# EricSteinberger/PokerRL

Hardware: AMD Instinct MI355X
Metric: CFR+ node-updates/sec on FHP public tree (higher is better)
Workload: dtype f32

## Files before the change

include/pokerrl_hip.h:

```cpp
#ifndef POKERRL_HIP_H
#define POKERRL_HIP_H

#include <stdint.h>

#ifdef __cplusplus
extern "C" {
#endif

#define PRL_MAX_BET_SIZES 96

#define PRL_OK 0
#define PRL_ERR_ARG (-1)
#define PRL_ERR_NO_DEVICE (-2)
#define PRL_ERR_HIP (-3)
#define PRL_ERR_UNSUPPORTED (-4)
#define PRL_ERR_OOM (-5)
#define PRL_ERR_STATE (-6)

typedef struct PrlRules {
    int32_t n_hole_cards;
    int32_t n_ranks;
    int32_t n_suits;
    int32_t n_cards;
    int32_t range_size;
// ... 86 lines not shown
int32_t prl_tree_info(const prl_tree_t* tree, int32_t* out_info );

enum {
    PRL_TF_KIND = 0,
    PRL_TF_ACTOR = 1,
    PRL_TF_PARENT = 2,
    PRL_TF_CHILD_IDX = 3,
    PRL_TF_ACTION = 4,
    PRL_TF_ACTED_LAST = 5,
    PRL_TF_ROUND = 6,
    PRL_TF_BOARD_ID = 7,
    PRL_TF_MAIN_POT = 8,
    PRL_TF_DEPTH = 9,
    PRL_TF_N_CHILDREN = 10,
    PRL_TF_FIRST_COL = 11,
    PRL_TF_SUBTREE_SIZE = 12,
    PRL_TF_CHILD_START = 13,
    PRL_TF_CHILD_LIST = 14,
    PRL_TF_COL_ACTION = 15,
    PRL_TF_COL_NODE = 16,
    PRL_TF_LEVEL_START = 17,
    PRL_TF_LEVEL_NODES = 18
};
int32_t prl_tree_get(const prl_tree_t* tree, int32_t field, int32_t* out);
int32_t prl_tree_get_boards(const prl_tree_t* tree, int8_t* out_rows);

#define PRL_OBS_VANILLA 0
#define PRL_OBS_HISTORY 1
#define PRL_OBS_FLAT_HU_LIMIT 2
int32_t prl_tree_obs_hist_len(const prl_tree_t* tree, const int32_t* node_idx, int32_t n, int32_t* out_hist_len);
int32_t prl_tree_observations_device(const prl_tree_t* tree, int32_t kind, int32_t invert, const int32_t* node_idx, const int64_t* row_offset,
                                     int32_t n, const int32_t* flat_offsets, int32_t row_dim, int64_t n_rows, float* d_out, uint8_t* d_legal,
                                     int32_t n_actions);
int32_t prl_tree_obs_stats(const prl_tree_t* tree, double* out);


int32_t prl_env_reset_host(const PrlGame* game, PrlEnvState* state);
int32_t prl_env_step_host(const PrlGame* game, PrlEnvState* state, int32_t action_int, PrlStepInfo* out_info);
int32_t prl_env_step_processed_host(const PrlGame* game, PrlEnvState* state, int32_t type, int32_t amount, PrlStepInfo* out_info);
int32_t prl_env_apply_action_host(const PrlGame* game, PrlEnvState* state, int32_t action_int, int32_t is_processed, int32_t type, int32_t amount,
                                  PrlStepInfo* out_info);
int32_t prl_env_legal_actions_host(const PrlGame* game, const PrlEnvState* state, int32_t* out_actions, int32_t* out_n);
int32_t prl_env_fraction_of_pot_raise_host(const PrlEnvState* state, double fraction, int32_t seat, int32_t* out_total);

typedef struct prl_envbatch prl_envbatch_t;
#define PRL_EB_N_COLS 13
enum {
    PRL_EB_ROUND = 0, PRL_EB_MAIN_POT = 1, PRL_EB_BET0 = 2, PRL_EB_BET1 = 3, PRL_EB_STACK0 = 4, PRL_EB_STACK1 = 5,
    PRL_EB_FLAGS = 6,
    PRL_EB_SEATS = 7,
    PRL_EB_N_ACTIONS_EP = 8, PRL_EB_N_RAISES_ROUND = 9, PRL_EB_LAST_ACTION_TYPE = 10, PRL_EB_LAST_ACTION_AMOUNT = 11, PRL_EB_LAST_ACTION_SEAT = 12
};
int32_t prl_envbatch_create(const PrlGame* game, int32_t n_envs, prl_envbatch_t** out_batch);
void prl_envbatch_destroy(prl_envbatch_t* batch);
int32_t prl_envbatch_reset(prl_envbatch_t* batch, const uint8_t* mask);
int32_t prl_envbatch_step(prl_envbatch_t* batch, const int32_t* actions, const int32_t* amounts, int32_t* out_info4);
int32_t prl_envbatch_step_device(prl_envbatch_t* batch, const int32_t* d_actions, const int32_t* d_amounts, int32_t* d_info4);
int32_t prl_envbatch_legal_masks(prl_envbatch_t* batch, uint32_t* out_mask4, int32_t* out_count);
int32_t prl_envbatch_active(prl_envbatch_t* batch, int32_t* out_idx, int32_t* out_count);
int32_t prl_envbatch_get_state(prl_envbatch_t* batch, int32_t* out_cols);
int32_t prl_envbatch_state_device(prl_envbatch_t* batch, void** out_d_cols, void** out_hip_stream);
int32_t prl_envbatch_random_rollout(prl_envbatch_t* batch, int32_t n_steps, uint32_t seed, uint64_t* out_stats3, float* out_device_ms);
int32_t prl_envbatch_random_steps(prl_envbatch_t* batch, int32_t n_launches, uint32_t seed, uint64_t* out_stats3, float* out_device_ms);
int32_t prl_env_random_rollout_host(const PrlGame* game, int32_t n_envs, int32_t n_steps, uint32_t seed, uint64_t* out_stats3);
int32_t prl_envbatch_create_with_cards(const PrlGame* game, const PrlRules* rules, int32_t n_envs, uint64_t deck_seed, double reward_scalar,
                                       prl_envbatch_t** out_batch);
int32_t prl_envbatch_obs_dim(prl_envbatch_t* batch, int32_t* out_dim);
int32_t prl_envbatch_reset_full(prl_envbatch_t* batch, const uint8_t* mask, float* out_obs );
int32_t prl_envbatch_set_cards(prl_envbatch_t* batch, const int8_t* cards);
int32_t prl_envbatch_get_cards(prl_envbatch_t* batch, int8_t* out_cards);
int32_t prl_envbatch_observe(prl_envbatch_t* batch, float* out_obs);
int32_t prl_envbatch_step_full(prl_envbatch_t* batch, const int32_t* actions, const int32_t* amounts, float* out_obs, double* out_reward2,
                               uint8_t* out_done, int32_t* out_info4);
int32_t prl_envbatch_step_full_device(prl_envbatch_t* batch, const int32_t* d_actions, const int32_t* d_amounts, float* d_obs, double* d_reward2,
                                      uint8_t* d_done, int32_t* d_info4);
int32_t prl_envbatch_random_rollout_full(prl_envbatch_t* batch, int32_t n_steps, uint32_t seed, uint64_t* out_stats4, float* out_device_ms);
int32_t prl_envbatch_random_steps_full(prl_envbatch_t* batch, int32_t n_launches, uint32_t seed, uint64_t* out_stats3, float* out_device_ms);
int32_t prl_envbatch_last_outputs(prl_envbatch_t* batch, float* out_obs, double* out_reward2, uint8_t* out_done);
int32_t prl_env_random_rollout_full_host(const PrlGame* game, const PrlRules* rules, int32_t n_envs, int32_t n_steps, uint32_t seed, uint64_t deck_seed,
                                         double reward_scalar, uint64_t* out_stats4);

typedef struct prl_solver prl_solver_t;

enum { PRL_VARIANT_VANILLA = 0, PRL_VARIANT_PLUS = 1, PRL_VARIANT_LINEAR = 2 };

int32_t prl_solver_create(const prl_tree_t* tree, int32_t variant, int32_t delay, prl_solver_t** out_solver);
enum { PRL_ENGINE_AUTO = 0, PRL_ENGINE_LEVELS = 1, PRL_ENGINE_FUSED = 2 };
int32_t prl_solver_create_ex(const prl_tree_t* tree, int32_t variant, int32_t delay, int32_t engine, prl_solver_t** out_solver);
enum { PRL_SOLVER_AVG_F32 = 1 };
int32_t prl_solver_create_opts(const prl_tree_t* tree, int32_t variant, int32_t delay, int32_t engine, int32_t flags, prl_solver_t** out_solver);
enum { PRL_SYMMETRIZE_SUBSET = 2 };
int32_t prl_solver_create_weighted(const prl_tree_t* tree, int32_t variant, int32_t delay, int32_t flags, const int32_t* board_mult, int32_t symmetrize,
                                   prl_solver_t** out_solver);
int32_t prl_solver_create_placed(const prl_tree_t* tree, int32_t variant, int32_t delay, int32_t engine, int32_t flags, int32_t n_candidates,
                                 int32_t probe_iters, float* out_ms, int32_t* out_chosen, prl_solver_t** out_solver);
int32_t prl_solver_create_weighted_placed(const prl_tree_t* tree, int32_t variant, int32_t delay, int32_t flags, const int32_t* board_mult, int32_t symmetrize,
                                          int32_t n_candidates, int32_t probe_iters, float* out_ms, int32_t* out_chosen, prl_solver_t** out_solver);
typedef int32_t (*prl_exchange_fn)(void* user, const void* local_dev, void* gathered_dev, uint64_t bytes_per_rank);
int32_t prl_solver_create_sharded(const prl_tree_t* local_tree, int32_t variant, int32_t delay, int32_t world_size, int32_t rank,
                                  prl_exchange_fn exchange, void* user, prl_solver_t** out_solver);
int32_t prl_solver_create_sharded_ragged(const prl_tree_t* local_tree, int32_t variant, int32_t delay, int32_t world_size, int32_t rank,
                                         int64_t shard_boards, int64_t total_boards, prl_exchange_fn exchange, void* user,
                                         prl_solver_t** out_solver);
int32_t prl_rccl_unique_id(void* out_id128);
int32_t prl_rccl_info(char* out, int32_t n);
int32_t prl_solver_create_sharded_rccl(const prl_tree_t* local_tree, int32_t variant, int32_t delay, int32_t world_size, int32_t rank,
                                       const void* unique_id128, int64_t shard_boards, int64_t total_boards, prl_solver_t** out_solver);
int32_t prl_solver_state_size(prl_solver_t* solver, uint64_t* out_bytes);
int32_t prl_solver_save_state(prl_solver_t* solver, void* out_blob, uint64_t bytes);
int32_t prl_solver_load_state(prl_solver_t* solver, const void* blob, uint64_t bytes);
int32_t prl_solver_get_stream(prl_solver_t* solver, void** out_hip_stream);
int32_t prl_solver_set_exchange_async(prl_solver_t* solver, int32_t stream_ordered);
int32_t prl_chance_sum_host(const float* board_values, int32_t n_boards, int32_t R, int32_t world_size, float* out);
int32_t prl_chance_sum_host_ragged(const float* board_values, int32_t n_boards, int32_t R, int32_t world_size, int32_t shard_boards, float* out);
void prl_solver_destroy(prl_solver_t* solver);
int32_t prl_solver_reset(prl_solver_t* solver);
int32_t prl_solver_iteration(prl_solver_t* solver);
int32_t prl_solver_iterations(prl_solver_t* solver, int32_t n);
int32_t prl_solver_iterations_many(prl_solver_t** solvers, int32_t n_solvers, int32_t n);
int32_t prl_solver_eval_avg(prl_solver_t* solver, float* out_expl2);
int32_t prl_solver_fill_uniform(prl_solver_t* solver);
int32_t prl_solver_set_strategy(prl_solver_t* solver, const void* strategy_cols, int32_t is_f64);
int32_t prl_solver_set_strategy_mixed(prl_solver_t* solver, const void* strategy_cols, int32_t is_f64, const uint8_t* node_is_f64);
int32_t prl_solver_update_reach(prl_solver_t* solver);
int32_t prl_solver_compute_ev(prl_solver_t* solver);
int32_t prl_solver_exploitability(prl_solver_t* solver, float* out_expl2);
int32_t prl_solver_sync(prl_solver_t* solver);
int32_t prl_solver_time_iterations(prl_solver_t* solver, int32_t n, float* out_ms);
int32_t prl_solver_time_iterations_ex(prl_solver_t* solver, int32_t n, float* out_ms, float* out_pass_ms, int32_t* out_n_pass);

int32_t prl_solver_time_evaluations(prl_solver_t* solver, int32_t n, float* out_ms, float* out_pass_ms, int32_t* out_n_pass);

enum {
    PRL_SF_REACH = 0,
    PRL_SF_EV = 1,
    PRL_SF_EV_BR = 2,
    PRL_SF_STRATEGY = 3,
    PRL_SF_STRAT_F64 = 4,
    PRL_SF_REGRET = 5,
    PRL_SF_AVG = 6,
    PRL_SF_AVG_F64 = 7,
    PRL_SF_AVG_SUM = 8,
    PRL_SF_BR_IDX = 9,
    PRL_SF_EXPL_HISTORY = 10,
    PRL_SF_ITER = 11,
    PRL_SF_CONSTANTS = 12,
    PRL_SF_BYTES_ALLOCATED = 13,
    PRL_SF_ENGINE = 14,
    PRL_SF_GRAPH_REPLAY = 15,
    PRL_SF_EXCHANGES = 17,
    PRL_SF_VMM_RANGES = 18,
    PRL_SF_AVG_PAIRS = 19,
    PRL_SF_AVG_SPLIT_PAIRS = 20,
    PRL_SF_EXPLICIT_STRATEGY = 16
};
int32_t prl_solver_get(prl_solver_t* solver, int32_t field, void* out);
int32_t prl_solver_set_strategy_device(prl_solver_t* solver, const prl_tree_t* tree, const float* d_probs, int32_t n_actions);
int32_t prl_solver_get_cols(prl_solver_t* solver, int32_t field, int64_t col_begin, int64_t n_cols, void* out);

int32_t prl_lbr_checkdown_equity(const PrlRules* rules, const int8_t* board_dealt, int32_t n_dealt, const int8_t* lbr_hand,
                                 const float* ranges, int32_t n_q, float* out_wp);
int32_t prl_lbr_checkdown_equity_batch(const PrlRules* rules, int32_t n_req, const int8_t* boards_dealt , const int32_t* n_dealt,
                                       const int8_t* lbr_hands , const float* ranges ,
                                       const int32_t* n_q, int32_t q_stride, float* out_wp );

int32_t prl_lbr_batch_run(const PrlGame* lbr_game, const PrlGame* agent_game, const PrlRules* rules, int32_t n_envs, int32_t agent_seat,
                          int32_t check_to_round, int32_t agent_kind, uint32_t agent_seed, uint32_t episode_base, double reward_scalar,
                          double ev_normalizer, const int8_t* cards, float* out_winnings, uint64_t* out_stats4, float* out_device_ms);
int32_t prl_lbr_batch_last_info(double* out8);

int32_t prl_h2h_batch_run(const PrlGame* game, const PrlRules* rules, int32_t n_envs, int32_t ref_seat, int32_t ref_kind, uint32_t ref_seed,
                          int32_t opp_kind, uint32_t opp_seed, uint32_t episode_base, double reward_scalar, double ev_normalizer,
                          const int8_t* cards, float* out_winnings, uint64_t* out_stats2, float* out_device_ms);

typedef struct PrlPolicyTable prl_policy_table_t;
prl_policy_table_t* prl_policy_table_create(const uint64_t* keys, const int32_t* rows, uint32_t capacity, const float* probs, int32_t n_rows,
                                            int32_t n_actions, int32_t range_size, uint32_t key_seed);
void prl_policy_table_destroy(prl_policy_table_t* table);
int32_t prl_policy_table_probe(const prl_policy_table_t* table, int32_t n, const uint32_t* key_lo, const uint32_t* key_hi, const int32_t* action,
                               const int32_t* hand, int32_t* out_row, float* out_prob);

int32_t prl_policy_table_from_solver(prl_solver_t* solver, const prl_tree_t* tree, uint32_t key_seed, prl_policy_table_t** out_table);
int32_t prl_policy_table_info(const prl_policy_table_t* table, int64_t* out6);
int32_t prl_policy_table_export_keys(const prl_policy_table_t* table, uint64_t* out_keys, int32_t* out_rows);
int32_t prl_policy_table_get_rows(const prl_policy_table_t* table, int32_t row_begin, int32_t n_rows, float* out);
int32_t prl_suit_canon_boards(const int8_t* boards, int32_t n, int32_t k, int32_t n_suits, int8_t* out_boards, int32_t* out_perm);

int32_t prl_lbr_batch_run_table(const PrlGame* lbr_game, const PrlGame* agent_game, const PrlRules* rules, int32_t n_envs, int32_t agent_seat,
                                int32_t check_to_round, const prl_policy_table_t* table, uint32_t agent_seed, uint32_t episode_base, double reward_scalar,
                                double ev_normalizer, const int8_t* cards, float* out_winnings, uint64_t* out_stats4, float* out_device_ms);

int32_t prl_h2h_batch_run_tables(const PrlGame* game, const PrlRules* rules, int32_t n_envs, int32_t ref_seat, int32_t ref_kind, uint32_t ref_seed,
                                 const prl_policy_table_t* ref_table, int32_t opp_kind, uint32_t opp_seed, const prl_policy_table_t* opp_table,
                                 uint32_t episode_base, double reward_scalar, double ev_normalizer, const int8_t* cards, float* out_winnings,
                                 uint64_t* out_stats2, float* out_device_ms);

int32_t prl_deal_decks(int32_t n_hands, int32_t n_cards_in_deck, int32_t n_deal, uint64_t seed, uint64_t first_hand, int8_t* out_cards);

#ifdef __cplusplus
}
#endif
#endif
```

pokerrl_amd/_native.py:

```python
import ctypes
import os

import numpy as np

_HERE = os.path.dirname(os.path.abspath(__file__))
EXCHANGE_FN = ctypes.CFUNCTYPE(ctypes.c_int32, ctypes.c_void_p, ctypes.c_void_p, ctypes.c_void_p, ctypes.c_uint64)
LIB_PATH = os.environ.get("POKERRL_AMD_LIB", os.path.join(_HERE, "lib", "libpokerrl_hip.so"))

PRL_MAX_BET_SIZES = 96


class NativeError(RuntimeError):
    status = None


ERR_ARG, ERR_NO_DEVICE, ERR_HIP, ERR_UNSUPPORTED, ERR_OOM, ERR_STATE = -1, -2, -3, -4, -5, -6


class PrlRules(ctypes.Structure):
    _fields_ = [
        ("n_hole_cards", ctypes.c_int32), ("n_ranks", ctypes.c_int32), ("n_suits", ctypes.c_int32),
        ("n_cards", ctypes.c_int32), ("range_size", ctypes.c_int32), ("n_rounds", ctypes.c_int32),
        ("board_cards_in_round", ctypes.c_int32 * 4), ("n_board_cards", ctypes.c_int32),
        ("btn_first_postflop", ctypes.c_int32), ("rank_rule", ctypes.c_int32),
# ... 373 lines not shown
        assert c.shape == (self.n_envs, self.n_deal)
        check(self._L.prl_envbatch_set_cards(self._h, _ptr(c)), self._L)

    def get_cards(self):
        c = np.empty((self.n_envs, self.n_deal), np.int8)
        check(self._L.prl_envbatch_get_cards(self._h, _ptr(c)), self._L)
        return c

    def observe(self):
        o = np.empty((self.n_envs, self.obs_dim), np.float32)
        check(self._L.prl_envbatch_observe(self._h, _ptr(o)), self._L)
        return o

    def step_full(self, actions, amounts=None):
        a = np.ascontiguousarray(actions, dtype=np.int32)
        b = None if amounts is None else np.ascontiguousarray(amounts, dtype=np.int32)
        obs, rew = np.empty((self.n_envs, self.obs_dim), np.float32), np.empty((self.n_envs, 2), np.float64)
        done, info = np.empty(self.n_envs, np.uint8), np.empty((4, self.n_envs), np.int32)
        check(self._L.prl_envbatch_step_full(self._h, _ptr(a), None if b is None else _ptr(b), _ptr(obs), _ptr(rew), _ptr(done), _ptr(info)), self._L)
        return obs, rew, done, info

    def last_outputs(self):
        obs, rew, done = np.empty((self.n_envs, self.obs_dim), np.float32), np.empty((self.n_envs, 2), np.float64), np.empty(self.n_envs, np.uint8)
        self._L.prl_envbatch_last_outputs.argtypes = [ctypes.c_void_p] * 4
        self._L.prl_envbatch_last_outputs.restype = ctypes.c_int32
        check(self._L.prl_envbatch_last_outputs(self._h, _ptr(obs), _ptr(rew), _ptr(done)), self._L)
        return obs, rew, done

    def random_steps_full(self, n_launches, seed):
        st, ms = np.zeros(3, np.uint64), ctypes.c_float()
        self._L.prl_envbatch_random_steps_full.argtypes = [ctypes.c_void_p, ctypes.c_int32, ctypes.c_uint32, ctypes.c_void_p, ctypes.c_void_p]
        self._L.prl_envbatch_random_steps_full.restype = ctypes.c_int32
        check(self._L.prl_envbatch_random_steps_full(self._h, int(n_launches), int(seed) & 0xFFFFFFFF, _ptr(st), ctypes.byref(ms)), self._L)
        return int(st[0]), int(st[1]), int(st[2]), float(ms.value)

    def random_rollout_full(self, n_steps, seed):
        st, ms = np.zeros(4, np.uint64), ctypes.c_float()
        check(self._L.prl_envbatch_random_rollout_full(self._h, int(n_steps), int(seed) & 0xFFFFFFFF, _ptr(st), ctypes.byref(ms)), self._L)
        return int(st[0]), int(st[1]), int(st[2]), int(st[3]), float(ms.value)

    def __del__(self):
        try:
            if self._h:
                self._L.prl_envbatch_destroy(self._h)
                self._h = None
        except Exception:
            pass


def env_random_rollout_full_host(game, rules, n_envs, n_steps, seed, deck_seed=0, reward_scalar=1.0, _lib=None):
    L = _lib or lib()
    st = np.zeros(4, np.uint64)
    L.prl_env_random_rollout_full_host.argtypes = [ctypes.POINTER(PrlGame), ctypes.POINTER(PrlRules), ctypes.c_int32, ctypes.c_int32, ctypes.c_uint32,
                                                   ctypes.c_uint64, ctypes.c_double, ctypes.c_void_p]
    L.prl_env_random_rollout_full_host.restype = ctypes.c_int32
    check(L.prl_env_random_rollout_full_host(ctypes.byref(game), ctypes.byref(rules), int(n_envs), int(n_steps), int(seed) & 0xFFFFFFFF, int(deck_seed),
                                             float(reward_scalar), _ptr(st)), L)
    return tuple(int(x) for x in st)


def env_random_rollout_host(game, n_envs, n_steps, seed, _lib=None):
    L = _lib or lib()
    st = np.zeros(3, np.uint64)
    check(L.prl_env_random_rollout_host(ctypes.byref(game), int(n_envs), int(n_steps), int(seed) & 0xFFFFFFFF, _ptr(st)), L)
    return int(st[0]), int(st[1]), int(st[2])


class NativeTree:

    def __init__(self, game, rules, boards_1d, _lib=None, stop_at_round=None):
        boards = np.ascontiguousarray(boards_1d, dtype=np.int8)
        assert boards.ndim == 2
        self._L = _lib or lib()
        self._h = ctypes.c_void_p()
        self._game, self._rules = game, rules
        self.is_partial = stop_at_round is not None
        self._L.prl_tree_build_partial.argtypes = [ctypes.POINTER(PrlGame), ctypes.POINTER(PrlRules), ctypes.c_void_p, ctypes.c_int32, ctypes.c_int32,
                                                   ctypes.c_int32, ctypes.POINTER(ctypes.c_void_p)]
        self._L.prl_tree_build_partial.restype = ctypes.c_int32
        check(self._L.prl_tree_build_partial(ctypes.byref(game), ctypes.byref(rules), _ptr(boards), boards.shape[0], boards.shape[1],
                                             -1 if stop_at_round is None else int(stop_at_round), ctypes.byref(self._h)), self._L)
        info = np.zeros(TI_COUNT, dtype=np.int32)
        check(self._L.prl_tree_info(self._h, _ptr(info)), self._L)
        self.info = info
        self.n_nodes, self.n_cols = int(info[TI_N_NODES]), int(info[TI_N_COLS])
        self.n_boards, self.board_len = int(info[TI_N_BOARDS]), int(info[TI_BOARD_LEN])
        self.n_levels, self.range_size = int(info[TI_N_LEVELS]), int(info[TI_RANGE_SIZE])
        self.n_decision, self.n_terminal = int(info[TI_N_DECISION]), int(info[TI_N_TERMINAL])
        self.boards = boards
        rows = np.empty((self.n_boards, self.board_len), np.int8)
        self._L.prl_tree_get_boards.argtypes = [ctypes.c_void_p, ctypes.c_void_p]
        self._L.prl_tree_get_boards.restype = ctypes.c_int32
        check(self._L.prl_tree_get_boards(self._h, _ptr(rows)), self._L)
        self.board_rows = rows
        self._cache = {}

    @classmethod
    def for_game(cls, game_cls, stack, bet_sizes, boards_1d, _lib=None):
        args = game_cls.ARGS_CLS(n_seats=2, starting_stack_sizes_list=[stack, stack], bet_sizes_list_as_frac_of_pot=bet_sizes)
        return cls(game_cls.native_game(args), game_cls.native_rules(), boards_1d, _lib=_lib)

    @property
    def handle(self):
        return self._h

    def field(self, name):
        if name not in self._cache:
            n = {"child_start": self.n_nodes + 1, "child_list": max(self.n_nodes - 1, 0), "col_action": self.n_cols,
                 "col_node": self.n_cols, "level_start": self.n_levels + 1}.get(name, self.n_nodes)
            out = np.empty(n, dtype=np.int32)
            check(self._L.prl_tree_get(self._h, TREE_FIELDS[name], _ptr(out)), self._L)
            self._cache[name] = out
        return self._cache[name]

    def obs_hist_len(self, node_idx):
        idx = np.ascontiguousarray(node_idx, dtype=np.int32)
        out = np.empty(len(idx), np.int32)
        self._L.prl_tree_obs_hist_len.argtypes = [ctypes.c_void_p, ctypes.c_void_p, ctypes.c_int32, ctypes.c_void_p]
        self._L.prl_tree_obs_hist_len.restype = ctypes.c_int32
        check(self._L.prl_tree_obs_hist_len(self._h, _ptr(idx), len(idx), _ptr(out)), self._L)
        return out

    def observations_device(self, kind, invert, node_idx, row_offset, flat_offsets, row_dim, n_rows, d_out, d_legal, n_actions):
        idx = np.ascontiguousarray(node_idx, dtype=np.int32)
        off = np.ascontiguousarray(row_offset, dtype=np.int64)
        assert len(off) == len(idx)
        fo = None if flat_offsets is None else np.ascontiguousarray(flat_offsets, dtype=np.int32)
        L = self._L
        L.prl_tree_observations_device.argtypes = [ctypes.c_void_p, ctypes.c_int32, ctypes.c_int32, ctypes.c_void_p, ctypes.c_void_p, ctypes.c_int32,
                                                   ctypes.c_void_p, ctypes.c_int32, ctypes.c_int64, ctypes.c_void_p, ctypes.c_void_p, ctypes.c_int32]
        L.prl_tree_observations_device.restype = ctypes.c_int32
        check(L.prl_tree_observations_device(self._h, int(kind), 1 if invert else 0, _ptr(idx), _ptr(off), len(idx), None if fo is None else _ptr(fo),
                                              int(row_dim), int(n_rows), ctypes.c_void_p(int(d_out)), ctypes.c_void_p(int(d_legal or 0)), int(n_actions)), L)

    def obs_stats(self):
        out = np.zeros(4, np.float64)
        self._L.prl_tree_obs_stats.argtypes = [ctypes.c_void_p, ctypes.c_void_p]
        self._L.prl_tree_obs_stats.restype = ctypes.c_int32
        check(self._L.prl_tree_obs_stats(self._h, _ptr(out)), self._L)
        return dict(state_bytes=int(out[0]), states_ms=float(out[1]), obs_ms=float(out[2]), obs_bytes=int(out[3]))

    def __del__(self):
        try:
            if self._h:
                self._L.prl_tree_destroy(self._h)
                self._h = None
        except Exception:
            pass


OBS_VANILLA, OBS_HISTORY, OBS_FLAT_HU_LIMIT = 0, 1, 2

SF = dict(reach=0, ev=1, ev_br=2, strategy=3, strat_f64=4, regret=5, avg=6, avg_f64=7, avg_sum=8, br_idx=9,
          expl_history=10, iter=11, constants=12, bytes_allocated=13, engine=14, graph_replay=15, explicit_strategy=16, exchanges=17, vmm_ranges=18, avg_pairs=19, avg_split_pairs=20)
VARIANTS = {"vanilla": 0, "plus": 1, "linear": 2}
ENGINES = {"auto": 0, "levels": 1, "fused": 2}


class NativeSolver:

    def __init__(self, tree, variant, delay=0, engine="auto", _lib=None, shard=None, avg_dtype="f64", place=None, probe_iters=4, board_mult=None,
                 symmetrize=False):
        self._L = _lib or tree._L
        self.placement_ms, self.placement_chosen = None, None
        if _lib is None and self._L is lib():
            require_device()
        self.tree = tree
        self._h = ctypes.c_void_p()
        v = VARIANTS[variant] if isinstance(variant, str) else int(variant)
        e = ENGINES[engine] if isinstance(engine, str) else int(engine)
        self._exchange_cb = None
        if board_mult is not None and shard is not None:
            raise ValueError("weighted boards (board_mult=): one GPU -- not with shard=")
        if symmetrize and board_mult is None:
            raise ValueError("symmetrize= goes with board_mult= (suit-class representatives and their orbit sizes)")
        if shard is not None and isinstance(shard[0], str):
            assert shard[0] == "rccl"
            world, rank, uid = shard[1:4]
            uid = (ctypes.c_char * 128).from_buffer_copy(bytes(uid))
            sb, tb = (int(shard[4]), int(shard[5])) if len(shard) == 6 else (0, 0)
            self._L.prl_solver_create_sharded_rccl.argtypes = [ctypes.c_void_p, ctypes.c_int32, ctypes.c_int32, ctypes.c_int32, ctypes.c_int32, ctypes.c_void_p,
                                                               ctypes.c_int64, ctypes.c_int64, ctypes.POINTER(ctypes.c_void_p)]
            self._L.prl_solver_create_sharded_rccl.restype = ctypes.c_int32
            check(self._L.prl_solver_create_sharded_rccl(tree.handle, v, int(delay), int(world), int(rank), ctypes.cast(uid, ctypes.c_void_p), sb, tb,
                                                         ctypes.byref(self._h)), self._L)
            shard = None
        elif shard is not None:
            world, rank, exchange = shard[:3]

            def _cb(_user, local_ptr, gathered_ptr, nbytes):
                try:
                    exchange(int(local_ptr or 0), int(gathered_ptr or 0), int(nbytes))
                    return 0
                except Exception:
                    import traceback
                    traceback.print_exc()
                    return 1

            self._exchange_cb = EXCHANGE_FN(_cb)
            if len(shard) == 5:
                check(self._L.prl_solver_create_sharded_ragged(tree.handle, v, int(delay), int(world), int(rank), int(shard[3]), int(shard[4]),
                                                               self._exchange_cb, None, ctypes.byref(self._h)), self._L)
            else:
                check(self._L.prl_solver_create_sharded(tree.handle, v, int(delay), int(world), int(rank), self._exchange_cb, None,
                                                        ctypes.byref(self._h)), self._L)
        elif board_mult is not None:
            m = np.ascontiguousarray(board_mult, np.int32)
            assert m.shape == (tree.n_boards,), "one multiplicity per listed board"
            sym = 2 if symmetrize == "subset" else (1 if symmetrize else 0)
            if place is not None:
                n = int(place)
                ms, chosen = (ctypes.c_float * n)(), ctypes.c_int32(0)
                self._L.prl_solver_create_weighted_placed.argtypes = [ctypes.c_void_p, ctypes.c_int32, ctypes.c_int32, ctypes.c_int32, ctypes.c_void_p, ctypes.c_int32,
                                                                      ctypes.c_int32, ctypes.c_int32, ctypes.POINTER(ctypes.c_float), ctypes.POINTER(ctypes.c_int32),
                                                                      ctypes.POINTER(ctypes.c_void_p)]
                self._L.prl_solver_create_weighted_placed.restype = ctypes.c_int32
                check(self._L.prl_solver_create_weighted_placed(tree.handle, v, int(delay), 1 if avg_dtype == "f32" else 0, _ptr(m), sym, n, int(probe_iters), ms,
                                                                ctypes.byref(chosen), ctypes.byref(self._h)), self._L)
                self.placement_ms, self.placement_chosen = [float(x) for x in ms], int(chosen.value)
            else:
                check(self._L.prl_solver_create_weighted(tree.handle, v, int(delay), 1 if avg_dtype == "f32" else 0, _ptr(m), sym, ctypes.byref(self._h)), self._L)
        elif not self._h and place is not None:
            n = int(place)
            ms = (ctypes.c_float * n)()
            chosen = ctypes.c_int32(0)
            self._L.prl_solver_create_placed.argtypes = [ctypes.c_void_p, ctypes.c_int32, ctypes.c_int32, ctypes.c_int32, ctypes.c_int32, ctypes.c_int32,
                                                         ctypes.c_int32, ctypes.POINTER(ctypes.c_float), ctypes.POINTER(ctypes.c_int32),
                                                         ctypes.POINTER(ctypes.c_void_p)]
            self._L.prl_solver_create_placed.restype = ctypes.c_int32
            check(self._L.prl_solver_create_placed(tree.handle, v, int(delay), e, 1 if avg_dtype == "f32" else 0, n, int(probe_iters), ms,
                                                   ctypes.byref(chosen), ctypes.byref(self._h)), self._L)
            self.placement_ms = [float(x) for x in ms]
            self.placement_chosen = int(chosen.value)
        elif not self._h:
            if avg_dtype == "f32":
                self._L.prl_solver_create_opts.argtypes = [ctypes.c_void_p, ctypes.c_int32, ctypes.c_int32, ctypes.c_int32, ctypes.c_int32, ctypes.POINTER(ctypes.c_void_p)]
                self._L.prl_solver_create_opts.restype = ctypes.c_int32
                check(self._L.prl_solver_create_opts(tree.handle, v, int(delay), e, 1, ctypes.byref(self._h)), self._L)
            else:
                assert avg_dtype == "f64"
                check(self._L.prl_solver_create_ex(tree.handle, v, int(delay), e, ctypes.byref(self._h)), self._L)
        if shard is not None and hasattr(shard[2], "bind_stream"):
            sp = ctypes.c_void_p()
            check(self._L.prl_solver_get_stream(self._h, ctypes.byref(sp)), self._L)
            if shard[2].bind_stream(sp.value or 0):
                check(self._L.prl_solver_set_exchange_async(self._h, 1), self._L)
        self.n_nodes, self.n_cols, self.R = tree.n_nodes, tree.n_cols, tree.range_size
        eng = np.zeros(1, np.int32)
        self._call("prl_solver_get", SF["engine"], _ptr(eng))
        self.engine = {1: "levels", 2: "fused"}[int(eng[0])]

    def __del__(self):
        try:
            if self._h:
                self._L.prl_solver_destroy(self._h)
                self._h = None
        except Exception:
            pass

    def _call(self, name, *args):
        check(getattr(self._L, name)(self._h, *args), self._L)

    def reset(self):
        self._call("prl_solver_reset")

    def iteration(self):
        self._call("prl_solver_iteration")

    def iterations(self, n):
        self._call("prl_solver_iterations", int(n))

    def fill_uniform(self):
        self._call("prl_solver_fill_uniform")

    def set_strategy(self, strategy_cols):
        a = np.ascontiguousarray(strategy_cols)
        if a.dtype not in (np.float32, np.float64):
            a = a.astype(np.float32)
        assert a.shape == (self.n_cols, self.R), (a.shape, (self.n_cols, self.R))
        self._call("prl_solver_set_strategy", _ptr(a), int(a.dtype == np.float64))

    def set_strategy_device(self, device_ptr, n_actions):
        self._L.prl_solver_set_strategy_device.argtypes = [ctypes.c_void_p, ctypes.c_void_p, ctypes.c_void_p, ctypes.c_int32]
        self._L.prl_solver_set_strategy_device.restype = ctypes.c_int32
        self._call("prl_solver_set_strategy_device", self.tree.handle, ctypes.c_void_p(int(device_ptr)), int(n_actions))

    def set_strategy_mixed(self, strategy_cols_f64, node_is_f64):
        a = np.ascontiguousarray(strategy_cols_f64, dtype=np.float64)
        f = np.ascontiguousarray(node_is_f64, dtype=np.uint8)
        assert a.shape == (self.n_cols, self.R)
        self._L.prl_solver_set_strategy_mixed.argtypes = [ctypes.c_void_p, ctypes.c_void_p, ctypes.c_int32, ctypes.c_void_p]
        self._L.prl_solver_set_strategy_mixed.restype = ctypes.c_int32
        self._call("prl_solver_set_strategy_mixed", _ptr(a), 1, _ptr(f))

    def update_reach(self):
        self._call("prl_solver_update_reach")

    def compute_ev(self):
        self._call("prl_solver_compute_ev")

    def sync(self):
        self._call("prl_solver_sync")

    def time_iterations(self, n):
        ms = ctypes.c_float()
        self._call("prl_solver_time_iterations", int(n), ctypes.byref(ms))
        return float(ms.value)

    def save_state(self):
        n = ctypes.c_uint64()
        self._call("prl_solver_state_size", ctypes.byref(n))
        blob = np.zeros(int(n.value), np.uint8)
        self._call("prl_solver_save_state", _ptr(blob), int(n.value))
        return blob

    def load_state(self, blob):
        blob = np.ascontiguousarray(blob, dtype=np.uint8)
        self._call("prl_solver_load_state", _ptr(blob), int(blob.shape[0]))

    @property
    def graph_replay(self):
        v = np.zeros(1, np.int32)
        self._call("prl_solver_get", SF["graph_replay"], _ptr(v))
        return bool(v[0])

    def time_iterations_ex(self, n):
        ms, pms, cnt = ctypes.c_float(), ctypes.c_float(), ctypes.c_int32()
        self._call("prl_solver_time_iterations_ex", int(n), ctypes.byref(ms), ctypes.byref(pms), ctypes.byref(cnt))
        return float(ms.value), float(pms.value), int(cnt.value)

    def time_evaluations(self, n):
        ms, pms, cnt = ctypes.c_float(), ctypes.c_float(), ctypes.c_int32()
        self._call("prl_solver_time_evaluations", int(n), ctypes.byref(ms), ctypes.byref(pms), ctypes.byref(cnt))
        return float(ms.value), float(pms.value), int(cnt.value)

    @staticmethod
    def iterations_many(solvers, n):
        if not solvers:
            return
        L = solvers[0]._L
        arr = (ctypes.c_void_p * len(solvers))(*[s._h for s in solvers])
        check(L.prl_solver_iterations_many(arr, len(solvers), int(n)), L)

    def exploitability(self):
        out = np.zeros(2, np.float32)
        self._call("prl_solver_exploitability", _ptr(out))
        return out

    def eval_avg(self):
        out = np.zeros(2, np.float32)
        self._call("prl_solver_eval_avg", _ptr(out))
        return out

    @property
    def iter(self):
        out = np.zeros(1, np.int32)
        self._call("prl_solver_get", SF["iter"], _ptr(out))
        return int(out[0])

    def get_cols(self, name, col_begin, n_cols):
        out = np.zeros((int(n_cols), self.R), np.float64 if name == "avg" else np.float32)
        self._L.prl_solver_get_cols.argtypes = [ctypes.c_void_p, ctypes.c_int32, ctypes.c_int64, ctypes.c_int64, ctypes.c_void_p]
        self._L.prl_solver_get_cols.restype = ctypes.c_int32
        self._call("prl_solver_get_cols", SF[name], int(col_begin), int(n_cols), _ptr(out))
        return out

    def sha256_of(self, name, cols_per_piece=65536):
        import hashlib
        h = hashlib.sha256()
        for c0 in range(0, self.n_cols, cols_per_piece):
            a = self.get_cols(name, c0, min(cols_per_piece, self.n_cols - c0))
            h.update(np.ascontiguousarray(a + a.dtype.type(0)).tobytes())
        return h.hexdigest()

    def sha256_of_many(self, names, cols_per_piece=32768):
        import hashlib
        import queue
        import threading
        hs = {n: hashlib.sha256() for n in names}
        qs = {n: queue.Queue(maxsize=3) for n in names}

        def work(n):
            while True:
                a = qs[n].get()
                if a is None:
                    return
                hs[n].update(np.ascontiguousarray(a + a.dtype.type(0)).tobytes())

        th = [threading.Thread(target=work, args=(n,), daemon=True) for n in names]
        for t in th:
            t.start()
        try:
            for c0 in range(0, self.n_cols, cols_per_piece):
                for n in names:
                    qs[n].put(self.get_cols(n, c0, min(cols_per_piece, self.n_cols - c0)))
        finally:
            for n in names:
                qs[n].put(None)
            for t in th:
                t.join()
        return {n: h.hexdigest() for n, h in hs.items()}

    def get(self, name):
        n, c, R = self.n_nodes, self.n_cols, self.R
        shape, dtype = {
            "reach": ((n, 2, R), np.float32), "ev": ((n, 2, R), np.float32), "ev_br": ((n, 2, R), np.float32),
            "strategy": ((c, R), np.float64), "strat_f64": ((n,), np.uint8), "regret": ((c, R), np.float32),
            "avg": ((c, R), np.float64), "avg_f64": ((n,), np.uint8), "avg_sum": ((c, R), np.float32),
            "br_idx": ((n, R), np.int32), "constants": ((2,), np.float32), "bytes_allocated": ((1,), np.int64),
            "explicit_strategy": ((1,), np.int32), "exchanges": ((1,), np.int64), "vmm_ranges": ((2,), np.int64),
            "avg_pairs": ((1,), np.int64), "avg_split_pairs": ((1,), np.int64),
        }.get(name, (None, None))
        if name == "expl_history":
            shape, dtype = (self.iter + 1, 2), np.float32
        out = np.zeros(shape, dtype)
        self._call("prl_solver_get", SF[name], _ptr(out))
        return out
```

pokerrl_amd/csrc/prl_fhp.h:

```cpp
#pragma once
#include "prl_defs.h"
#include "prl_solver_types.h"
#include "prl_tree.h"

enum { PRL_SRC_REGRET = 0, PRL_SRC_UNIFORM64 = 1, PRL_SRC_ARR64 = 2, PRL_SRC_ARR32 = 3,
       PRL_SRC_STRAT32 = 4 ,
       PRL_SRC_AVGF32 = 5  };
enum { PRL_FHP_UPDATE0 = 0, PRL_FHP_UPDATE1 = 1, PRL_FHP_EVAL = 2, PRL_FHP_UPDATE0_EVAL = 3, PRL_FHP_UPDATE0_BR = 4, PRL_FHP_UPDATE1_EVAL1 = 5,
       PRL_FHP_EVAL0 = 6 };
constexpr bool prl_fhp_runs_seat(int mode, int p) {
    return mode == PRL_FHP_EVAL || mode == PRL_FHP_UPDATE0_EVAL ? true
         : (mode == PRL_FHP_UPDATE1 || mode == PRL_FHP_UPDATE1_EVAL1) ? p == 1 : p == 0;
}
constexpr bool prl_fhp_updates(int mode, int p) {
    return p == 0 ? (mode == PRL_FHP_UPDATE0 || mode == PRL_FHP_UPDATE0_EVAL || mode == PRL_FHP_UPDATE0_BR)
                  : (mode == PRL_FHP_UPDATE1 || mode == PRL_FHP_UPDATE1_EVAL1);
}
constexpr bool prl_fhp_with_br(int mode) { return mode >= PRL_FHP_EVAL; }
constexpr int prl_fhp_out_width(int mode) {
    return mode == PRL_FHP_UPDATE1_EVAL1 ? 3
         : (prl_fhp_runs_seat(mode, 0) && prl_fhp_runs_seat(mode, 1) ? 2 : 1) * (prl_fhp_with_br(mode) ? 2 : 1);
}

#define PRL_FHP_MAX_NODES 40
// ... 12 lines not shown
    static constexpr int K(int n) { constexpr int t[N_NODES] = {0, 0, 3, 0, 2, 3, 0, 2, 3}; return t[n]; }
    static constexpr int A(int n) { constexpr int t[N_NODES] = {1, 0, -1, 1, -1, -1, 0, -1, -1}; return t[n]; }
    static constexpr int C(int n) { constexpr int t[N_NODES] = {2, 2, 0, 2, 0, 0, 2, 0, 0}; return t[n]; }
};
struct PrlFhpSpec21 {
    static constexpr int N_NODES = 21;
    static constexpr int K(int n) { constexpr int t[N_NODES] = {0, 0, 3, 0, 2, 3, 0, 2, 3, 0, 2, 3, 0, 2, 3, 0, 2, 3, 0, 2, 3}; return t[n]; }
    static constexpr int A(int n) { constexpr int t[N_NODES] = {1, 0, -1, 1, -1, -1, 0, -1, -1, 1, -1, -1, 0, -1, -1, 1, -1, -1, 0, -1, -1}; return t[n]; }
    static constexpr int C(int n) { constexpr int t[N_NODES] = {2, 2, 0, 3, 0, 0, 3, 0, 0, 2, 0, 0, 3, 0, 0, 3, 0, 0, 2, 0, 0}; return t[n]; }
};

struct PrlFhpSpec27 {
    static constexpr int N_NODES = 27;
    static constexpr int K(int n) { constexpr int t[N_NODES] = {0, 0, 3, 0, 2, 3, 0, 2, 3, 0, 2, 3, 0, 2, 3, 0, 2, 3, 0, 2, 3, 0, 2, 3, 0, 2, 3}; return t[n]; }
    static constexpr int A(int n) { constexpr int t[N_NODES] = {1, 0, -1, 1, -1, -1, 0, -1, -1, 1, -1, -1, 0, -1, -1, 0, -1, -1, 1, -1, -1, 0, -1, -1, 1, -1, -1}; return t[n]; }
    static constexpr int C(int n) { constexpr int t[N_NODES] = {2, 2, 0, 3, 0, 0, 3, 0, 0, 3, 0, 0, 2, 0, 0, 3, 0, 0, 3, 0, 0, 3, 0, 0, 2, 0, 0}; return t[n]; }
};
struct PrlFhpSpec33 {
    static constexpr int N_NODES = 33;
    static constexpr int K(int n) { constexpr int t[N_NODES] = {0, 0, 3, 0, 2, 3, 0, 2, 3, 0, 2, 3, 0, 2, 3, 0, 2, 3, 0, 2, 3, 0, 2, 3, 0, 2, 3, 0, 2, 3, 0, 2, 3}; return t[n]; }
    static constexpr int A(int n) { constexpr int t[N_NODES] = {1, 0, -1, 1, -1, -1, 0, -1, -1, 1, -1, -1, 0, -1, -1, 1, -1, -1, 0, -1, -1, 1, -1, -1, 0, -1, -1, 1, -1, -1, 0, -1, -1}; return t[n]; }
    static constexpr int C(int n) { constexpr int t[N_NODES] = {2, 2, 0, 3, 0, 0, 3, 0, 0, 3, 0, 0, 3, 0, 0, 2, 0, 0, 3, 0, 0, 3, 0, 0, 3, 0, 0, 3, 0, 0, 2, 0, 0}; return t[n]; }
};
struct PrlFhpSpec15B2 {
    static constexpr int N_NODES = 15;
    static constexpr int K(int n) { constexpr int t[N_NODES] = {0, 0, 3, 0, 2, 3, 0, 2, 3, 0, 2, 3, 0, 2, 3}; return t[n]; }
    static constexpr int A(int n) { constexpr int t[N_NODES] = {1, 0, -1, 1, -1, -1, 1, -1, -1, 0, -1, -1, 0, -1, -1}; return t[n]; }
    static constexpr int C(int n) { constexpr int t[N_NODES] = {3, 3, 0, 2, 0, 0, 2, 0, 0, 2, 0, 0, 2, 0, 0}; return t[n]; }
};
struct PrlFhpSpec21B2 {
    static constexpr int N_NODES = 21;
    static constexpr int K(int n) { constexpr int t[N_NODES] = {0, 0, 3, 0, 2, 3, 0, 2, 3, 0, 2, 3, 0, 2, 3, 0, 2, 3, 0, 2, 3}; return t[n]; }
    static constexpr int A(int n) { constexpr int t[N_NODES] = {1, 0, -1, 1, -1, -1, 0, -1, -1, 1, -1, -1, 0, -1, -1, 1, -1, -1, 0, -1, -1}; return t[n]; }
    static constexpr int C(int n) { constexpr int t[N_NODES] = {3, 3, 0, 3, 0, 0, 2, 0, 0, 2, 0, 0, 3, 0, 0, 2, 0, 0, 2, 0, 0}; return t[n]; }
};
struct PrlFhpSpec33B2 {
    static constexpr int N_NODES = 33;
    static constexpr int K(int n) { constexpr int t[N_NODES] = {0, 0, 3, 0, 2, 3, 0, 2, 3, 0, 2, 3, 0, 2, 3, 0, 2, 3, 0, 2, 3, 0, 2, 3, 0, 2, 3, 0, 2, 3, 0, 2, 3}; return t[n]; }
    static constexpr int A(int n) { constexpr int t[N_NODES] = {1, 0, -1, 1, -1, -1, 0, -1, -1, 1, -1, -1, 0, -1, -1, 1, -1, -1, 0, -1, -1, 1, -1, -1, 0, -1, -1, 1, -1, -1, 0, -1, -1}; return t[n]; }
    static constexpr int C(int n) { constexpr int t[N_NODES] = {3, 3, 0, 4, 0, 0, 3, 0, 0, 2, 0, 0, 2, 0, 0, 2, 0, 0, 4, 0, 0, 3, 0, 0, 2, 0, 0, 2, 0, 0, 2, 0, 0}; return t[n]; }
};
template <class S>
struct PrlFhpDerive {
    static constexpr int N_NODES = S::N_NODES;
    static constexpr int kind(int n) { return S::K(n); }
    static constexpr int actor(int n) { return S::A(n); }
    static constexpr int nch(int n) { return S::C(n); }
    static constexpr int subtree_size(int n) {
        int size = 1;
        for (int i = 0, c = n + 1; i < nch(n); ++i) { const int t = subtree_size(c); size += t; c += t; }
        return size;
    }
    static constexpr int child(int n, int i) {
        if (i >= nch(n)) return -1;
        int c = n + 1;
        for (int k = 0; k < i; ++k) c += subtree_size(c);
        return c;
    }
    static constexpr int parent(int n) {
        for (int p = n - 1; p >= 0; --p)
            for (int i = 0; i < nch(p); ++i)
                if (child(p, i) == n) return p;
        return -1;
    }
    static constexpr int count_kind(int k, int below) { int c = 0; for (int m = 0; m < below; ++m) c += kind(m) == k; return c; }
    static constexpr int N_DEC = count_kind(PRL_NODE_DECISION, N_NODES);
    static constexpr int N_SHOW = count_kind(PRL_NODE_TERM_SHOWDOWN, N_NODES);
    static constexpr int N_FOLD = count_kind(PRL_NODE_TERM_FOLD, N_NODES);
    static constexpr int col0(int n) {
        if (kind(n) != PRL_NODE_DECISION) return -1;
        int c = 0;
        for (int m = 0; m < n; ++m) c += kind(m) == PRL_NODE_DECISION ? nch(m) : 0;
        return c;
    }
    static constexpr int n_cols_() { int c = 0; for (int m = 0; m < N_NODES; ++m) c += kind(m) == PRL_NODE_DECISION ? nch(m) : 0; return c; }
    static constexpr int N_COLS = n_cols_();
    static constexpr int max_a_() { int a = 0; for (int m = 0; m < N_NODES; ++m) a = kind(m) == PRL_NODE_DECISION && nch(m) > a ? nch(m) : a; return a; }
    static constexpr int MAX_A = max_a_();
    static constexpr int folder(int n) { return kind(n) == PRL_NODE_TERM_FOLD ? actor(parent(n)) : -1; }
    static constexpr int term_slot(int n) {
        return kind(n) == PRL_NODE_TERM_SHOWDOWN ? count_kind(PRL_NODE_TERM_SHOWDOWN, n)
             : kind(n) == PRL_NODE_TERM_FOLD ? N_SHOW + count_kind(PRL_NODE_TERM_FOLD, n) : -1;
    }
    static constexpr int col_node(int col) {
        for (int m = 0; m < N_NODES; ++m)
            if (kind(m) == PRL_NODE_DECISION && col0(m) <= col && col < col0(m) + nch(m)) return m;
        return -1;
    }
    static constexpr int col_actor(int col) { return actor(col_node(col)); }
    static constexpr int dec_node(int j) {
        for (int m = 0, k = 0; m < N_NODES; ++m)
            if (kind(m) == PRL_NODE_DECISION && k++ == j) return m;
        return -1;
    }
};

struct PrlFhpShapeDesc {
    int32_t n_nodes, n_cols, n_dec;
    int32_t kind[PRL_FHP_MAX_NODES], actor[PRL_FHP_MAX_NODES], nch[PRL_FHP_MAX_NODES], parent[PRL_FHP_MAX_NODES], col0[PRL_FHP_MAX_NODES],
        folder[PRL_FHP_MAX_NODES];
    int32_t dec_nch[PRL_FHP_MAX_DEC], dec_col0[PRL_FHP_MAX_DEC];
};
template <class D>
inline PrlFhpShapeDesc prl_fhp_describe() {
    PrlFhpShapeDesc d = {};
    d.n_nodes = D::N_NODES; d.n_cols = D::N_COLS; d.n_dec = D::N_DEC;
    static_assert(D::N_NODES <= PRL_FHP_MAX_NODES && D::N_DEC <= PRL_FHP_MAX_DEC, "enlarge PRL_FHP_MAX_*");
    static_assert(D::MAX_A <= PRL_FHP_MAX_ACTIONS, "a decision node with more actions than the readers of dec_nch hold (PRL_FHP_MAX_ACTIONS)");
    for (int n = 0; n < D::N_NODES; ++n) {
        d.kind[n] = D::kind(n); d.actor[n] = D::actor(n); d.nch[n] = D::nch(n); d.parent[n] = D::parent(n); d.col0[n] = D::col0(n);
        d.folder[n] = D::folder(n);
    }
    for (int j = 0; j < D::N_DEC; ++j) { d.dec_nch[j] = D::nch(D::dec_node(j)); d.dec_col0[j] = D::col0(D::dec_node(j)); }
    return d;
}
enum { PRL_FHP_SHAPE_15 = 0, PRL_FHP_SHAPE_9 = 1, PRL_FHP_SHAPE_21 = 2, PRL_FHP_N_SHAPES = 3 };
const PrlFhpShapeDesc& prl_fhp_shape_desc(int shape_id);

#define PRL_FHP_NP 1088
enum { PRL_FHP_AVG_NORMAL = 0, PRL_FHP_AVG_DEFERRED = 1, PRL_FHP_AVG_CATCH_UP = 2 };
struct PrlFhpParams {
    int32_t n_boards, R;
    int32_t np;
    int32_t variant, iter;
    int32_t max_grid;
    int32_t shape;
    int32_t n_cols_board, n_dec;
    int32_t dec_nch[PRL_FHP_MAX_DEC], dec_col0[PRL_FHP_MAX_DEC];
    float chance_prob, eq_const;
    float pot[PRL_FHP_MAX_NODES];
    const float* chance_reach;
    const float* board_w;
    float* regret;
    double* avg;
    float* avg32;
    int32_t avg_mode;
    double m_old, m_new;
    int32_t avg_pair, avg_pair_b;
    double m_old_prev, m_new_prev;
    float* avg_sum;
    int32_t avgsum_mask, avgsum_iter[2];
    int32_t block_sum;
    int32_t exp;
    int32_t no_steady;
    const double* strat_arr;
    float* board_out;
    const int16_t* plan_pp;
    const uint32_t* plan_clx;
    unsigned long long* timing;
};

int prl_fhp_match_shape(const PrlFlatTree& t, int* chance_node, int* first_board_node, int* col_base, float* pots );

int prl_launch_fhp_pass(const PrlFhpParams& prm, int mode, int src0, int src1, void* stream);
bool prl_fhp_avg_split_supported(int shape_id);
void prl_launch_fhp_strategy_from_regret(const PrlFhpParams& prm, double* out_region, void* stream);
void prl_launch_fhp_avg_from_sum(const PrlFhpParams& prm, void* stream);
void prl_launch_fhp_symmetrize(const float* in, int n_vec, int R, const int32_t* class_of, const int32_t* class_start, const int32_t* class_hands, float* out, void* stream);
void prl_launch_fhp_expand(const PrlFhpParams& prm, const void* region, int elem, int b0, int nb, const void* fill_by_col, const void* blocked_src,
                           void* dst, void* stream);
void prl_launch_fhp_compact(const PrlFhpParams& prm, const void* src, int elem, int b0, int nb, void* region, void* blocked_dst, void* stream);
#define PRL_FHP_NBLOCKED (1326 - 1081)
void prl_launch_fhp_chance_sum(const float* d_board_vals, int n_boards, int W, float* d_scratch, float* d_dest, void* stream);
int prl_fhp_units_at_level(int n_boards, int level);
void prl_launch_fhp_chance_partial(const float* d_board_vals, int n_boards, int level, int W, float* d_scratch, float* d_units, void* stream);
void prl_launch_fhp_chance_partial_from_blocks(const float* d_blocks, int n_blk, int level, int W, float* d_units, void* stream);
void prl_launch_fhp_chance_finish(const float* d_units, int n_units, int level, int W, float* d_scratch, float* d_dest, void* stream);
void prl_launch_fhp_compact_gathered(const float* d_in, int world, int n_which, int n_units, int W, float* d_out, void* stream);
```

pokerrl_amd/csrc/prl_fhp_kernels.hip:

```cpp
#include <type_traits>

#include "prl_device.h"
#include "prl_fhp.h"
#include "prl_kernels.h"


#if defined(PRL_EMU)
#define FHP_LB(t, w)
#else
#define FHP_LB(t, w) __launch_bounds__(t, w)
#endif

#define FHP_THREADS 768
#define FHP_SLOTS 2
#define FHP_LAUNCH_BOUNDS FHP_LB(768, 3)
#define FHP_AVG_SPLIT 1
#define FHP_SPEC PrlFhpSpec15
namespace fhp_shape15 {
#include "prl_fhp_pass.inc"
}
#undef FHP_SPEC
#define FHP_SPEC PrlFhpSpec9
namespace fhp_shape9 {
#include "prl_fhp_pass.inc"
}
#undef FHP_SPEC
#if !defined(PRL_FHP_NO_SHAPE21)
#undef FHP_AVG_SPLIT
#define FHP_AVG_SPLIT 0
#define FHP_SPEC PrlFhpSpec21
namespace fhp_shape21 {
#include "prl_fhp_pass.inc"
}
#undef FHP_SPEC
#endif
#undef FHP_THREADS
#undef FHP_SLOTS
#undef FHP_LAUNCH_BOUNDS
#undef FHP_AVG_SPLIT

bool prl_fhp_avg_split_supported(int shape_id) { return shape_id == PRL_FHP_SHAPE_15 || shape_id == PRL_FHP_SHAPE_9; }

const PrlFhpShapeDesc& prl_fhp_shape_desc(int shape_id) {
    static_assert(PrlFhpDerive<PrlFhpSpec15>::MAX_A <= PRL_FHP_BOARD_MAX_ACTIONS && PrlFhpDerive<PrlFhpSpec9>::MAX_A <= PRL_FHP_BOARD_MAX_ACTIONS &&
                      PrlFhpDerive<PrlFhpSpec21>::MAX_A <= PRL_FHP_BOARD_MAX_ACTIONS,
                  "the board pass and the readers of PrlFhpParams::dec_nch hold PRL_FHP_BOARD_MAX_ACTIONS actions per node");
    static const PrlFhpShapeDesc d[PRL_FHP_N_SHAPES] = {prl_fhp_describe<PrlFhpDerive<PrlFhpSpec15>>(), prl_fhp_describe<PrlFhpDerive<PrlFhpSpec9>>(),
                                                        prl_fhp_describe<PrlFhpDerive<PrlFhpSpec21>>()};
    return d[shape_id];
}

bool prl_fhp_shape_compiled(int shape_id) {
#if !defined(PRL_FHP_NO_SHAPE21)
    return shape_id >= 0 && shape_id < PRL_FHP_N_SHAPES;
#else
    return shape_id == PRL_FHP_SHAPE_15 || shape_id == PRL_FHP_SHAPE_9;
#endif
}

PRL_GLOBAL void prl_k_fhp_symmetrize(const float* in, int n_vec, int R, const int32_t* class_of, const int32_t* class_start, const int32_t* class_hands, float* out) {
    const int i = (int)(prl_bid() * prl_nthreads() + prl_tid());
    if (i >= n_vec * R) return;
    const int v = i / R, h = i - v * R, k = class_of[h];
    const int a = class_start[k], b = class_start[k + 1];
    float s = in[(size_t)v * R + class_hands[a]];
    for (int j = a + 1; j < b; ++j) s = s + in[(size_t)v * R + class_hands[j]];
    out[i] = s / (float)(b - a);
}
void prl_launch_fhp_symmetrize(const float* in, int n_vec, int R, const int32_t* class_of, const int32_t* class_start, const int32_t* class_hands, float* out, void* stream) {
    const int n = n_vec * R;
    PRL_LAUNCH(prl_k_fhp_symmetrize, (n + 255) / 256, 256, 0, stream, in, n_vec, R, class_of, class_start, class_hands, out);
}

int prl_launch_fhp_pass(const PrlFhpParams& prm, int mode, int src0, int src1, void* stream) {
    switch (prm.shape) {
        case PRL_FHP_SHAPE_15: return fhp_shape15::launch_pass(prm, mode, src0, src1, stream);
        case PRL_FHP_SHAPE_9: return fhp_shape9::launch_pass(prm, mode, src0, src1, stream);
#if !defined(PRL_FHP_NO_SHAPE21)
        case PRL_FHP_SHAPE_21: return fhp_shape21::launch_pass(prm, mode, src0, src1, stream);
#endif
        default: return PRL_ERR_UNSUPPORTED;
    }
}

PRL_GLOBAL void prl_k_fhp_strategy_from_regret(PrlFhpParams prm, double* out_region) {
    const size_t per_board = (size_t)prm.n_dec * prm.np;
    const size_t total = (size_t)prm.n_boards * per_board;
    for (size_t t = (size_t)prl_bid() * prl_nthreads() + prl_tid(); t < total; t += (size_t)prl_nblocks() * prl_nthreads()) {
        const size_t b = t / per_board;
        const int j = (int)((t % per_board) / prm.np);
        const size_t q = t % prm.np;
        const int A = prm.dec_nch[j], col0 = prm.dec_col0[j];
        const size_t base = (b * prm.n_cols_board + col0) * (size_t)prm.np + q;
        float tt[PRL_FHP_BOARD_MAX_ACTIONS];
        float sum = 0.f;
        for (int i = 0; i < A; ++i) {
            float r = prm.regret[base + (size_t)i * prm.np];
            tt[i] = prm.variant == PRL_CFR_PLUS ? r : (r > 0.f ? r : 0.f);
            sum = sum + tt[i];
        }
        const float unif = (float)(1.0 / (double)A);
        for (int i = 0; i < A; ++i) out_region[base + (size_t)i * prm.np] = (double)(sum > 0.f ? tt[i] / sum : unif);
    }
}

PRL_GLOBAL void prl_k_fhp_avg_from_sum(PrlFhpParams prm) {
    const size_t per_board = (size_t)prm.n_dec * prm.np;
    const size_t total = (size_t)prm.n_boards * per_board;
    for (size_t t = (size_t)prl_bid() * prl_nthreads() + prl_tid(); t < total; t += (size_t)prl_nblocks() * prl_nthreads()) {
        const size_t b = t / per_board;
        const int j = (int)((t % per_board) / prm.np);
        const size_t q = t % prm.np;
        const int A = prm.dec_nch[j], col0 = prm.dec_col0[j];
        const size_t base = (b * prm.n_cols_board + col0) * (size_t)prm.np + q;
        float as[PRL_FHP_BOARD_MAX_ACTIONS];
        for (int i = 0; i < A; ++i) as[i] = prm.avg_sum[base + (size_t)i * prm.np];
        float sum = as[0];
        for (int i = 1; i < A; ++i) sum = sum + as[i];
        for (int i = 0; i < A; ++i) prm.avg[base + (size_t)i * prm.np] = sum == 0.f ? 1.0 / (double)A : (double)(as[i] / sum);
    }
}

template <class E>
PRL_GLOBAL void prl_k_fhp_expand(PrlFhpParams prm, const E* region, int b0, int nb, const E* fill_by_col, const E* blocked_src, E* dst) {
    const int ncb = prm.n_cols_board, R = prm.R, NL = R - PRL_FHP_NBLOCKED;
    const size_t total = (size_t)nb * ncb * R;
    for (size_t t = (size_t)prl_bid() * prl_nthreads() + prl_tid(); t < total; t += (size_t)prl_nblocks() * prl_nthreads()) {
        const int q = (int)(t % R);
        const size_t bj = t / R;
        const int j = (int)(bj % ncb);
        const size_t b = (size_t)b0 + bj / ncb;
        const int h = prm.plan_pp[b * PRL_PP_STRIDE + q];
        E v;
        if (q < NL) v = region[(b * ncb + j) * (size_t)prm.np + q];
        else if (blocked_src) v = blocked_src[(b * ncb + j) * (size_t)PRL_FHP_NBLOCKED + (q - NL)];
        else v = fill_by_col ? fill_by_col[j] : (E)0;
        dst[bj * R + h] = v;
    }
}
template <class E>
PRL_GLOBAL void prl_k_fhp_compact(PrlFhpParams prm, const E* src, int b0, int nb, E* region, E* blocked_dst) {
    const int ncb = prm.n_cols_board, R = prm.R, NL = R - PRL_FHP_NBLOCKED, NPX = prm.np + PRL_FHP_NBLOCKED;
    const size_t total = (size_t)nb * ncb * NPX;
    for (size_t t = (size_t)prl_bid() * prl_nthreads() + prl_tid(); t < total; t += (size_t)prl_nblocks() * prl_nthreads()) {
        const int q = (int)(t % NPX);
        const size_t bj = t / NPX;
        const int j = (int)(bj % ncb);
        const size_t b = (size_t)b0 + bj / ncb;
        const int16_t* sh = prm.plan_pp + b * PRL_PP_STRIDE;
        if (q < prm.np) region[(b * ncb + j) * (size_t)prm.np + q] = q < NL ? src[bj * R + sh[q]] : (E)0;
        else if (blocked_dst) blocked_dst[(b * ncb + j) * (size_t)PRL_FHP_NBLOCKED + (q - prm.np)] = src[bj * R + sh[NL + (q - prm.np)]];
    }
}

struct alignas(8) PrlF2 { float x, y; };
PRL_GLOBAL void prl_k_fhp_sum_level(const float* __restrict__ in, int n_in, int fan, int R2, float* __restrict__ out) {
    const int n_out = (n_in + fan - 1) / fan;
    const int R2h = R2 / 2;
    const size_t total = (size_t)n_out * R2h;
    for (size_t t = (size_t)prl_bid() * prl_nthreads() + prl_tid(); t < total; t += (size_t)prl_nblocks() * prl_nthreads()) {
        const int o = (int)(t / R2h);
        const int x = 2 * (int)(t % R2h);
        const int lo = o * fan, hi = lo + fan < n_in ? lo + fan : n_in;
        PrlF2 s = *(const PrlF2*)(in + (size_t)lo * R2 + x);
        for (int i = lo + 1; i < hi; ++i) {
            const PrlF2 v = *(const PrlF2*)(in + (size_t)i * R2 + x);
            s.x = s.x + v.x;
            s.y = s.y + v.y;
        }
        *(PrlF2*)(out + (size_t)o * R2 + x) = s;
    }
}

static inline int fhp_grid_for(size_t items, int block) {
    size_t g = (items + block - 1) / block;
    if (g < 1) g = 1;
    if (g > 16384) g = 16384;
    return (int)g;
}

void prl_launch_fhp_strategy_from_regret(const PrlFhpParams& prm, double* out_region, void* stream) {
    if (prm.n_boards <= 0) return;
    size_t items = (size_t)prm.n_boards * prm.n_dec * prm.np;
    PRL_LAUNCH(prl_k_fhp_strategy_from_regret, fhp_grid_for(items, 256), 256, 0, stream, prm, out_region);
}

void prl_launch_fhp_avg_from_sum(const PrlFhpParams& prm, void* stream) {
    if (prm.n_boards <= 0) return;
    size_t items = (size_t)prm.n_boards * prm.n_dec * prm.np;
    PRL_LAUNCH(prl_k_fhp_avg_from_sum, fhp_grid_for(items, 256), 256, 0, stream, prm);
}

void prl_launch_fhp_expand(const PrlFhpParams& prm, const void* region, int elem, int b0, int nb, const void* fill_by_col, const void* blocked_src,
                           void* dst, void* stream) {
    if (nb <= 0) return;
    const size_t items = (size_t)nb * prm.n_cols_board * prm.R;
    if (elem == 4) PRL_LAUNCH(prl_k_fhp_expand<float>, fhp_grid_for(items, 256), 256, 0, stream, prm, (const float*)region, b0, nb, (const float*)fill_by_col, (const float*)blocked_src, (float*)dst);
    else PRL_LAUNCH(prl_k_fhp_expand<double>, fhp_grid_for(items, 256), 256, 0, stream, prm, (const double*)region, b0, nb, (const double*)fill_by_col, (const double*)blocked_src, (double*)dst);
}

void prl_launch_fhp_compact(const PrlFhpParams& prm, const void* src, int elem, int b0, int nb, void* region, void* blocked_dst, void* stream) {
    if (nb <= 0) return;
    const size_t items = (size_t)nb * prm.n_cols_board * (prm.np + PRL_FHP_NBLOCKED);
    if (elem == 4) PRL_LAUNCH(prl_k_fhp_compact<float>, fhp_grid_for(items, 256), 256, 0, stream, prm, (const float*)src, b0, nb, (float*)region, (float*)blocked_dst);
    else PRL_LAUNCH(prl_k_fhp_compact<double>, fhp_grid_for(items, 256), 256, 0, stream, prm, (const double*)src, b0, nb, (double*)region, (double*)blocked_dst);
}

void prl_launch_fhp_chance_sum(const float* d_board_vals, int n_boards, int W, float* d_scratch, float* d_dest, void* stream) {
    prl_launch_fhp_chance_finish(d_board_vals, n_boards, 0, W, d_scratch, d_dest, stream);
}

int prl_fhp_units_at_level(int n_boards, int level) {
    int n = n_boards;
    for (int l = 0; l < level; ++l) n = (n + PRL_CHANCE_BLOCK - 1) / PRL_CHANCE_BLOCK;
    return n;
}

void prl_launch_fhp_chance_partial(const float* d_board_vals, int n_boards, int level, int W, float* d_scratch, float* d_units, void* stream) {
    const int R2 = W;
    if (level == 0) {
        PRL_LAUNCH(prl_k_fhp_sum_level, fhp_grid_for((size_t)n_boards * R2 / 2, 256), 256, 0, stream, d_board_vals, n_boards, 1, R2, d_units);
        return;
    }
    const int n_blk = (n_boards + PRL_CHANCE_BLOCK - 1) / PRL_CHANCE_BLOCK;
    float* blk = level == 1 ? d_units : d_scratch;
    PRL_LAUNCH(prl_k_fhp_sum_level, fhp_grid_for((size_t)n_blk * R2 / 2, 256), 256, 0, stream, d_board_vals, n_boards, PRL_CHANCE_BLOCK, R2, blk);
    if (level == 1) return;
    const int n_grp = (n_blk + PRL_CHANCE_BLOCK - 1) / PRL_CHANCE_BLOCK;
    PRL_LAUNCH(prl_k_fhp_sum_level, fhp_grid_for((size_t)n_grp * R2 / 2, 256), 256, 0, stream, (const float*)blk, n_blk, PRL_CHANCE_BLOCK, R2, d_units);
}

void prl_launch_fhp_chance_partial_from_blocks(const float* d_blocks, int n_blk, int level, int W, float* d_units, void* stream) {
// ... 39 lines not shown
```

pokerrl_amd/csrc/prl_fhp_pass.inc:

```
#ifndef FHP_NPAD
#define FHP_NPAD 1088
#define FHP_NLIVE 1081
#define FHP_NCARDS 52
#define FHP_R 1326
#define FHP_NP PRL_FHP_NP
#define FHP_NSHOW (PrlFhpShape::N_SHOW)
#define FHP_NFOLD (PrlFhpShape::N_FOLD)
#define FHP_NVEC (PrlFhpShape::N_SHOW + PrlFhpShape::N_FOLD)
#endif
typedef PrlFhpDerive<FHP_SPEC> PrlFhpShape;
#if defined(FHP_EXPERIMENT)
#define FHP_EXP(c, bit) (((c).prm->exp & (bit)) != 0)
#define FHP_AVG_PIPELINED(c) true
#define FHP_TERMINAL_CACHE(c) true
#else
#define FHP_EXP(c, bit) false
#define FHP_AVG_PIPELINED(c) true
#define FHP_TERMINAL_CACHE(c) true
#endif
static_assert(PrlFhpShape::subtree_size(0) == PrlFhpShape::N_NODES, "the spec is one DFS pre-order tree");
static_assert(FHP_NP == FHP_NPAD && FHP_NP == PRL_PP_NPAD && FHP_R == PRL_PP_R && FHP_SLOTS == 2, "sorted storage: a column holds the padded sorted domain, a lane two positions");

#include "prl_fhp_div.inc"
struct FhpV { FhpF v; };
// ... 31 lines not shown
#else
    if constexpr (FHP_SLOTS == 2 && sizeof(T) == 4) {
        typedef float v2 __attribute__((ext_vector_type(2)));
        v2 v; v.x = in[0]; v.y = in[1];
        __builtin_nontemporal_store(v, (v2*)p);
    } else if constexpr (FHP_SLOTS == 2 && sizeof(T) == 8) {
        typedef double d2 __attribute__((ext_vector_type(2)));
        d2 v; v.x = in[0]; v.y = in[1];
        __builtin_nontemporal_store(v, (d2*)p);
    } else { for (int k = 0; k < FHP_SLOTS; ++k) __builtin_nontemporal_store(in[k], p + k); }
#endif
}
template <class T>
PRL_DEV PRL_INLINE void fhp_gload_nt(const T* p, T (&out)[FHP_SLOTS]) {
#if defined(PRL_EMU)
    fhp_gload(p, out);
#else
    if constexpr (FHP_SLOTS == 2 && sizeof(T) == 8) {
        typedef double d2 __attribute__((ext_vector_type(2)));
        const d2 v = __builtin_nontemporal_load((const d2*)p);
        out[0] = v.x; out[1] = v.y;
    } else if constexpr (FHP_SLOTS == 2 && sizeof(T) == 4) {
        typedef float v2 __attribute__((ext_vector_type(2)));
        const v2 v = __builtin_nontemporal_load((const v2*)p);
        out[0] = v.x; out[1] = v.y;
    } else { for (int k = 0; k < FHP_SLOTS; ++k) out[k] = __builtin_nontemporal_load(p + k); }
#endif
}
PRL_DEV PRL_INLINE void fhp_gstore(float* p, const FhpF& in) {
    float t[FHP_SLOTS];
    for (int k = 0; k < FHP_SLOTS; ++k) t[k] = in[k];
    fhp_gstore(p, t);
}

PRL_DEV PRL_INLINE FhpF fhp_lds_load2(const float* v, int p0) { return *(const FhpF*)(v + p0); }
PRL_DEV PRL_INLINE void fhp_lds_store2(float* v, int p0, const FhpF& x) { *(FhpF*)(v + p0) = x; }

#define FHP_NPAIRS (FHP_NVEC / 2)
constexpr int fhp_y_base(int u) { return u < 2 * FHP_NPAIRS ? (u >> 1) * (2 * FHP_NPAD) + (u & 1) : 2 * FHP_NPAIRS * FHP_NPAD; }
constexpr int fhp_y_step(int u) { return u < 2 * FHP_NPAIRS ? 2 : 1; }
constexpr int fhp_term_node(int slot) {
    for (int n = 0; n < PrlFhpShape::N_NODES; ++n)
        if (PrlFhpShape::kind(n) != PRL_NODE_DECISION && PrlFhpShape::term_slot(n) == slot) return n;
    return -1;
}
constexpr int fhp_yord(int slot) {
    int u = 0;
    for (int n = 0; n < fhp_term_node(slot); ++n) u += PrlFhpShape::kind(n) != PRL_NODE_DECISION;
    return u;
}
constexpr unsigned fhp_show_mask() {
    unsigned m = 0;
    for (int s = 0; s < PrlFhpShape::N_SHOW; ++s) m |= 1u << fhp_yord(s);
    return m;
}
#if defined(PRL_EMU)
struct FhpQ { float e[4]; float& operator[](int k) { return e[k]; } const float& operator[](int k) const { return e[k]; } };
#else
typedef float FhpQ __attribute__((ext_vector_type(4)));
#endif

#ifdef PRL_FHP_TIMING
#define FHP_TICK(c, i) do { const long long t_ = __builtin_readcyclecounter(); (c).t_acc[i] += t_ - (c).t_prev; (c).t_prev = t_; } while (0)
#ifdef PRL_FHP_TIMING_BARRIERS
#define FHP_SYNC(c, id) do { const long long a_ = clock64(); prl_sync_lds(); if ((prl_tid() & 63) == 0) atomicAdd((c).prm->timing + 8 + 12 * (id) + (prl_tid() >> 6), (unsigned long long)(clock64() - a_)); } while (0)
#else
#define FHP_SYNC(c, id) prl_sync_lds()
#endif
#else
#define FHP_TICK(c, i) do { } while (0)
#define FHP_SYNC(c, id) prl_sync_lds()
#endif

struct FhpLds {
    float* y;
    float* K;
    float* Tc;
    float* Tt;
    float* pf_rg;
    uint32_t* pf_clx;
    uint32_t* pf_pp;
    float* acc;
};
PRL_DEV PRL_INLINE int fhp_lead(const void* p) { return (int)(((size_t)p >> 2) & 3); }
#define FHP_PF_ROWS(words) ((((words) + 3 + 3) / 4 + 63) / 64)
#define FHP_PF_AREA(words) (FHP_PF_ROWS(words) * 256)
#define FHP_PP_WORDS (PRL_PP_STRIDE / 2)
#define FHP_ACC_WORDS (4 * FHP_R)
constexpr bool fhp_run_starts(int seat, int j) { return PrlFhpShape::col_actor(j) == seat && (j == 0 || PrlFhpShape::col_actor(j - 1) != seat); }
constexpr int fhp_n_runs(int seat) { int n = 0; for (int j = 0; j < PrlFhpShape::N_COLS; ++j) n += fhp_run_starts(seat, j); return n; }
constexpr int fhp_run_col0(int seat, int r) {
    for (int j = 0, n = 0; j < PrlFhpShape::N_COLS; ++j)
        if (fhp_run_starts(seat, j) && n++ == r) return j;
    return PrlFhpShape::N_COLS;
}
constexpr int fhp_run_cols(int seat, int r) {
    int n = 0;
    for (int j = fhp_run_col0(seat, r); j < PrlFhpShape::N_COLS && PrlFhpShape::col_actor(j) == seat; ++j) ++n;
    return n;
}
constexpr int fhp_run_rows(int seat, int r) { return FHP_PF_ROWS(fhp_run_cols(seat, r) * FHP_NP); }
constexpr int fhp_run_row0(int seat, int r) { int s = 0; for (int i = 0; i < r; ++i) s += fhp_run_rows(seat, i); return s; }
constexpr int fhp_seat_rows(int seat) { return fhp_run_row0(seat, fhp_n_runs(seat)); }
constexpr int fhp_col_run(int j) {
    const int seat = PrlFhpShape::col_actor(j);
    for (int r = 0; r < fhp_n_runs(seat); ++r)
        if (fhp_run_col0(seat, r) <= j && j < fhp_run_col0(seat, r) + fhp_run_cols(seat, r)) return r;
    return -1;
}
constexpr int FHP_PF_RG_ROWS = fhp_seat_rows(0) > fhp_seat_rows(1) ? fhp_seat_rows(0) : fhp_seat_rows(1);
#define FHP_PF_RG_WORDS (FHP_PF_RG_ROWS * 256)
#define FHP_LDS_WORK_BYTES ((FHP_NVEC * FHP_NPAD + 2 * FHP_NSHOW * FHP_NPAD + FHP_NFOLD * 64 + 16 + FHP_ACC_WORDS) * 4)
#define FHP_LDS_BYTES_WITH_RG (FHP_LDS_WORK_BYTES + (FHP_PF_RG_WORDS + FHP_PF_AREA(PRL_CLX_WORDS) + FHP_PF_AREA(FHP_PP_WORDS)) * 4)
#define FHP_RG_IN_LDS (FHP_LDS_BYTES_WITH_RG <= 160 * 1024)
#define FHP_LDS_BYTES (FHP_RG_IN_LDS ? FHP_LDS_BYTES_WITH_RG : FHP_LDS_BYTES_WITH_RG - FHP_PF_RG_WORDS * 4)

PRL_DEV PRL_INLINE FhpLds fhp_lds() {
    FhpLds L;
    float* f = (float*)prl_smem();
    L.y = f; f += FHP_NVEC * FHP_NPAD;
    L.K = f; f += 2 * FHP_NSHOW * FHP_NPAD;
    L.Tc = f; f += FHP_NFOLD * 64;
    L.Tt = f; f += 16;
    L.acc = f; f += FHP_ACC_WORDS;
    L.pf_rg = f; f += FHP_RG_IN_LDS ? FHP_PF_RG_WORDS : 0;
    L.pf_clx = (uint32_t*)f; f += FHP_PF_AREA(PRL_CLX_WORDS);
    L.pf_pp = (uint32_t*)f; f += FHP_PF_AREA(FHP_PP_WORDS);
    return L;
}

constexpr int FHP_STEADY_PAIR0 = 16;
constexpr int fhp_kind_code(int k) { return k == 1 ? 0 : k == 5 ? 1 : 2; }
constexpr int fhp_steady_pair(int ka, int kb) { return ka == kb ? ka : FHP_STEADY_PAIR0 + 4 * fhp_kind_code(ka) + fhp_kind_code(kb); }
constexpr int fhp_code_kind(int c) { return c == 0 ? 1 : c == 1 ? 5 : 6; }
constexpr int fhp_set_kind(int steady, int set) {
    return steady < FHP_STEADY_PAIR0 ? steady : fhp_code_kind(set == 0 ? (steady - FHP_STEADY_PAIR0) / 4 : (steady - FHP_STEADY_PAIR0) % 4);
}
constexpr bool fhp_steady_plus(int steady) { return steady == 1 || steady == 4 || steady == 5 || steady == 6 || steady >= FHP_STEADY_PAIR0; }
constexpr int fhp_avg_set(int n) {
    int cols[2] = {0, 0};
    for (int a = PrlFhpShape::MAX_A; a >= 1; --a)
        for (int m = 0; m < PrlFhpShape::N_NODES; ++m)
            if (PrlFhpShape::kind(m) == PRL_NODE_DECISION && PrlFhpShape::actor(m) == PrlFhpShape::actor(n) && PrlFhpShape::nch(m) == a) {
                const int set = cols[1] <= cols[0] ? 1 : 0;
                if (m == n) return set;
                cols[set] += a;
            }
    return 0;
}
constexpr bool fhp_may_load_avg(int steady, int n) {
    if (steady == 0) return true;
    const int k = fhp_set_kind(steady, fhp_avg_set(n));
    return k == 1 || k == 4 || k == 6;
}
template <int STEADY>
struct FhpCtxT {
    static constexpr int steady = STEADY;
    static constexpr bool own_after_b(int src_opp) { return src_opp == PRL_SRC_REGRET && !fhp_steady_plus(STEADY); }
    PRL_DEV PRL_INLINE int variant() const {
        if constexpr (fhp_steady_plus(STEADY)) return PRL_CFR_PLUS;
        else if constexpr (STEADY == 2) return PRL_CFR_LINEAR;
        else if constexpr (STEADY == 3) return PRL_CFR_VANILLA;
        else return variant_;
    }
    PRL_DEV PRL_INLINE bool first_iteration() const { if constexpr (STEADY != 0) return false; else return iter == 0; }
    template <int NODE>
    PRL_DEV PRL_INLINE int avg_mode() const {
        constexpr int set = fhp_avg_set(NODE);
        if constexpr (STEADY == 0) return (set == 0 ? prm->avg_pair : prm->avg_pair_b) == PRL_FHP_AVG_DEFERRED ? 0 : prm->avg_mode;
        else return fhp_may_load_avg(STEADY, NODE) ? 2 : 0;
    }
    template <int NODE>
    PRL_DEV PRL_INLINE bool avg_catch_up() const {
        constexpr int set = fhp_avg_set(NODE);
        if constexpr (STEADY == 0) return (set == 0 ? prm->avg_pair : prm->avg_pair_b) == PRL_FHP_AVG_CATCH_UP;
        else return fhp_set_kind(STEADY, set) == 6;
    }
    PRL_DEV PRL_INLINE int avgsum_mask() const { if constexpr (fhp_steady_plus(STEADY)) return 0; else return prm->avgsum_mask; }
    PRL_DEV PRL_INLINE bool avg32() const { if constexpr (STEADY == 4) return true; else if constexpr (STEADY != 0) return false; else return prm->avg32 != nullptr; }
    FhpLds L;
    int wave;
    uint32_t pf_lds;
    uint32_t rec0, rec1;
    int p0;
    int gsm1[FHP_SLOTS];
    int gem1[FHP_SLOTS];
    bool live[FHP_SLOTS];
    int c1[FHP_SLOTS], c2[FHP_SLOTS];
    int sh[FHP_SLOTS];
    bool active;
    bool valid;
    float eq_const;
    int variant_, iter;
    const PrlFhpParams* prm;
    size_t cofs;
    FhpF nr0, nr1;
    float nw;
    double av_old[PrlFhpShape::N_COLS][FHP_SLOTS];
    bool fast;
#ifdef PRL_FHP_TIMING
    long long t_prev, t_acc[6];
#endif
};

constexpr bool fhp_src_f32_block(int src) { return src == PRL_SRC_REGRET || src == PRL_SRC_STRAT32; }
constexpr bool fhp_src_in_lds(int src) { return FHP_RG_IN_LDS && fhp_src_f32_block(src); }
template <int SRC> struct FhpScalar { typedef float type; };
template <> struct FhpScalar<PRL_SRC_UNIFORM64> { typedef double type; };
template <> struct FhpScalar<PRL_SRC_ARR64> { typedef double type; };
template <> struct FhpScalar<PRL_SRC_AVGF32> { typedef double type; };

PRL_DEV PRL_INLINE float fhp_mul_reach(float s, float r) { return s * r; }
PRL_DEV PRL_INLINE float fhp_mul_reach(double s, float r) { return (float)(s * (double)r); }

struct FhpRegs {
    float rg[PrlFhpShape::N_COLS][FHP_SLOTS];
    double sa[PrlFhpShape::N_COLS][FHP_SLOTS];
};

template <int SRC, int A, class S, class C>
PRL_DEV PRL_INLINE void fhp_node_strategy(const C& c, const FhpRegs& R, int col0, S (&s)[3][FHP_SLOTS]) {
    if constexpr (SRC == PRL_SRC_REGRET) {
        float t[3][FHP_SLOTS], sum[FHP_SLOTS], q[3][FHP_SLOTS];
        for (int k = 0; k < FHP_SLOTS; ++k) {
            for (int i = 0; i < A; ++i) {
                float r = R.rg[col0 + i][k];
                t[i][k] = c.variant() == PRL_CFR_PLUS ? r : (r > 0.f ? r : 0.f);
            }
            sum[k] = 0.f;
            for (int i = 0; i < A; ++i) sum[k] = sum[k] + t[i][k];
        }
        fhp_regret_match<A>(t, sum, q, c.fast);
        for (int i = 0; i < A; ++i)
            for (int k = 0; k < FHP_SLOTS; ++k) s[i][k] = (S)q[i][k];
        return;
    }
    for (int k = 0; k < FHP_SLOTS; ++k) {
        if (SRC == PRL_SRC_UNIFORM64) {
            for (int i = 0; i < A; ++i) s[i][k] = (S)(1.0 / (double)A);
        } else if (SRC == PRL_SRC_STRAT32) {
            for (int i = 0; i < A; ++i) s[i][k] = (S)R.rg[col0 + i][k];
        } else if (SRC == PRL_SRC_ARR64 || SRC == PRL_SRC_AVGF32) {
            for (int i = 0; i < A; ++i) s[i][k] = (S)R.sa[col0 + i][k];
        } else {
            for (int i = 0; i < A; ++i) s[i][k] = (S)(float)R.sa[col0 + i][k];
        }
    }
}

struct FhpAvgPre { float v[PrlFhpShape::N_COLS][FHP_SLOTS]; };

template <int Q, int S0, int S1, int NODE>
struct FhpDown {
    template <class C>
    static PRL_DEV PRL_INLINE void run(C& c, const FhpRegs& R, const FhpAvgPre& AP, const FhpV& rq, FhpF& yv) {
        constexpr int kind = PrlFhpShape::kind(NODE);
        if constexpr (kind != PRL_NODE_DECISION) {
            constexpr int u = fhp_yord(PrlFhpShape::term_slot(NODE)), ub = fhp_y_base(u);
            if constexpr (fhp_y_step(u) == 1) fhp_lds_store2(c.L.y + ub, c.p0, rq.v);
            else if constexpr ((u & 1) == 0) yv = rq.v;
            else {
                FhpQ q;
                q[0] = yv[0]; q[1] = rq.v[0]; q[2] = yv[1]; q[3] = rq.v[1];
                *(FhpQ*)(c.L.y + (u >> 1) * (2 * FHP_NPAD) + 2 * c.p0) = q;
            }
        } else {
            constexpr int a = PrlFhpShape::actor(NODE);
            constexpr int A = PrlFhpShape::nch(NODE);
            if constexpr (a == Q) {
                constexpr int SRC = Q == 0 ? S0 : S1;
                constexpr int col0_q = PrlFhpShape::col0(NODE);
                typedef typename FhpScalar<SRC>::type S;
                S s[3][FHP_SLOTS];
                fhp_node_strategy<SRC, A, S>(c, R, col0_q, s);
                if (SRC == PRL_SRC_REGRET && (c.avgsum_mask() & (1 << Q))) {
                    constexpr int col0 = PrlFhpShape::col0(NODE);
                    const int it = c.prm->avgsum_iter[Q];
                    for (int i = 0; i < A; ++i) {
                        float as[FHP_SLOTS];
                        for (int k = 0; k < FHP_SLOTS; ++k) {
                            float contrib = (float)s[i][k] * rq.v[k];
                            if (c.variant() == PRL_CFR_LINEAR) contrib = contrib * (float)(it + 1);
                            as[k] = it > 0 ? AP.v[col0 + i][k] + contrib : contrib;
                        }
                        fhp_gstore(c.prm->avg_sum + c.cofs + (size_t)(col0 + i) * FHP_NP, as);
                    }
                }
                FhpV cr;
                for (int k = 0; k < FHP_SLOTS; ++k) cr.v[k] = fhp_mul_reach(s[0][k], rq.v[k]);
                FhpDown<Q, S0, S1, PrlFhpShape::child(NODE, 0)>::run(c, R, AP, cr, yv);
                for (int k = 0; k < FHP_SLOTS; ++k) cr.v[k] = fhp_mul_reach(s[1][k], rq.v[k]);
                FhpDown<Q, S0, S1, PrlFhpShape::child(NODE, 1)>::run(c, R, AP, cr, yv);
                if constexpr (A > 2) {
                    for (int k = 0; k < FHP_SLOTS; ++k) cr.v[k] = fhp_mul_reach(s[2][k], rq.v[k]);
                    FhpDown<Q, S0, S1, PrlFhpShape::child(NODE, 2)>::run(c, R, AP, cr, yv);
                }
            } else {
                FhpDown<Q, S0, S1, PrlFhpShape::child(NODE, 0)>::run(c, R, AP, rq, yv);
                FhpDown<Q, S0, S1, PrlFhpShape::child(NODE, 1)>::run(c, R, AP, rq, yv);
                if constexpr (A > 2) FhpDown<Q, S0, S1, PrlFhpShape::child(NODE, 2)>::run(c, R, AP, rq, yv);
            }
        }
    }
};

template <class C, class F>
PRL_DEV PRL_INLINE void fhp_scan_phases(C& c, F&& between_c_and_d) {
    const FhpLds& L = c.L;
    const int tid = (int)prl_tid(), wave = tid >> 6, lane = tid & 63, n_waves = FHP_THREADS / 64;
    static_assert(FHP_THREADS == PRL_CLX_SLOTS * 16, "one lane per record");
    {
        float kc[3][FHP_NSHOW];
        int qpos[3];
        const uint32_t ent[3] = {c.rec0 & 0xFFFFu, c.rec0 >> 16, c.rec1 & 0xFFFFu};
        const int lane_a = (int)((c.rec1 >> 16) & 15u), lane_b = (int)((c.rec1 >> 20) & 15u), card = (int)(c.rec1 >> 24);
        const int row_base = lane & 48;
        bool head[3], tail[3], lower[3], ok[3];
#pragma unroll
        for (int k = 0; k < 3; ++k) {
            qpos[k] = (int)(ent[k] & 0x7FFu);
            head[k] = (ent[k] & PRL_CLX_HEAD) != 0;
            tail[k] = (ent[k] & PRL_CLX_TAIL) != 0;
            lower[k] = (ent[k] & PRL_CLX_LOWER) != 0;
            ok[k] = (ent[k] & PRL_CLX_VALID) != 0;
        }
        float l[3][FHP_NVEC];
#pragma unroll
        for (int j = 0; j < FHP_NPAIRS; ++j)
#pragma unroll
            for (int k = 0; k < 3; ++k) {
                const FhpF t = *(const FhpF*)(L.y + j * (2 * FHP_NPAD) + 2 * qpos[k]);
                l[k][2 * j] = t[0];
                l[k][2 * j + 1] = t[1];
            }
        if constexpr (FHP_NVEC % 2 == 1) {
#pragma unroll
            for (int k = 0; k < 3; ++k) l[k][FHP_NVEC - 1] = L.y[2 * FHP_NPAIRS * FHP_NPAD + qpos[k]];
        }
        float carry[FHP_NVEC];
#pragma unroll
        for (int v = 0; v < FHP_NVEC; ++v) {
            l[1][v] = l[0][v] + l[1][v];
            l[2][v] = l[1][v] + l[2][v];
            carry[v] = l[2][v];
        }
#pragma unroll
        for (int v = 0; v < FHP_NVEC; ++v) carry[v] = prl_row16_scan(carry[v]);
#pragma unroll
        for (int v = 0; v < FHP_NVEC; ++v) carry[v] = prl_dpp_row_shr<1>(carry[v]);
        if ((lane & 15) == 15 && card < 64) {
            fhp_static_for<0, FHP_NFOLD>([&](auto V) __attribute__((always_inline)) {
                constexpr int v = decltype(V)::value, u = fhp_yord(FHP_NSHOW + v);
                L.Tc[v * 64 + card] = carry[u] + l[0][u];
            });
        }
        fhp_static_for<0, FHP_NSHOW>([&](auto V) __attribute__((always_inline)) {
            constexpr int v = decltype(V)::value, u = fhp_yord(v);
            const float qi0 = carry[u] + l[0][u], qi1 = carry[u] + l[1][u], qi2 = carry[u] + l[2][u];
            const float qe0 = prl_dpp_row_shr<1>(qi2);
            const float tot = prl_dpp_row_share<15>(qi0);
            const float out_a = head[2] ? qi1 : (head[1] ? qi0 : qe0);
            const float out_b = tail[0] ? qi0 : (tail[1] ? qi1 : qi2);
            const float ra = prl_shfl(out_a, row_base + lane_a);
            const float rb = prl_shfl(out_b, row_base + lane_b);
            const float a0 = head[0] ? qe0 : ra, a1 = head[1] ? qi0 : a0, a2 = head[2] ? qi1 : a1;
            const float b2 = tail[2] ? qi2 : rb, b1 = tail[1] ? qi1 : b2, b0 = tail[0] ? qi0 : b1;
            kc[0][v] = a0 - (tot - b0);
            kc[1][v] = a1 - (tot - b1);
            kc[2][v] = a2 - (tot - b2);
        });
#pragma unroll
        for (int k = 0; k < 3; ++k) {
            const int kp = ok[k] ? qpos[k] + (lower[k] ? 0 : FHP_NSHOW * FHP_NPAD) : FHP_NPAD - 2 - (lane & 3);
#pragma unroll
            for (int v = 0; v < FHP_NSHOW; ++v) L.K[v * FHP_NPAD + kp] = kc[k][v];
        }
    }
    FHP_SYNC(c, 2);
    FHP_TICK(c, 2);
    between_c_and_d();
    constexpr int NCH = FHP_NPAD / 64, LAST = NCH - 1, LAST_LANES = FHP_NLIVE - 64 * LAST;
    static_assert(LAST_LANES > 0 && LAST_LANES <= 64 - 7, "the last chunk ends with the unused / trash / zero slots");
    auto range_prefix = [&](auto ST, const int v) __attribute__((always_inline)) {
        constexpr int st = decltype(ST)::value;
        float* y = L.y + (st == 2 ? (v >> 1) * (2 * FHP_NPAD) + (v & 1) : 2 * FHP_NPAIRS * FHP_NPAD) + st * lane;
        float incl[NCH];
#pragma unroll
        for (int k = 0; k < NCH; ++k) incl[k] = y[st * 64 * k];
        incl[LAST] = lane < LAST_LANES ? incl[LAST] : 0.f;
        prl_wave_scan_canonical_n(incl);
        float carry = 0.f;
        constexpr unsigned SHOW = fhp_show_mask();
        const bool show = ((SHOW >> v) & 1u) != 0u;
        if (show) {
#pragma unroll
            for (int k = 0; k < LAST; ++k) {
                y[st * 64 * k] = carry + incl[k];
                carry = carry + prl_readlane(incl[k], 63);
            }
        } else {
#pragma unroll
            for (int k = 0; k < LAST; ++k) carry = carry + prl_readlane(incl[k], 63);
        }
        const float pj = carry + incl[LAST];
        if (show && lane < LAST_LANES) y[st * 64 * LAST] = pj;
        if (lane == LAST_LANES - 1) L.Tt[v] = pj;
    };
    for (int v = wave; v < FHP_NVEC; v += n_waves) {
        if (v < 2 * FHP_NPAIRS) range_prefix(std::integral_constant<int, 2>(), v);
        else range_prefix(std::integral_constant<int, 1>(), v);
    }
    prl_dma_wait();
    FHP_SYNC(c, 3);
}

constexpr bool fhp_is_dec_of(int P, int n) { return PrlFhpShape::kind(n) == PRL_NODE_DECISION && PrlFhpShape::actor(n) == P; }
constexpr bool fhp_completes_before(int a, int b) {
    if (a > b) return a < b + PrlFhpShape::subtree_size(b);
    return !(b < a + PrlFhpShape::subtree_size(a));
}
constexpr int fhp_completion_rank(int steady, int P, int n) {
    int r = 0;
    for (int m = 0; m < PrlFhpShape::N_NODES; ++m)
        if (m != n && fhp_is_dec_of(P, m) && fhp_may_load_avg(steady, m) && fhp_completes_before(m, n)) ++r;
    return r;
}
constexpr int fhp_node_of_rank(int steady, int P, int r) {
    for (int m = 0; m < PrlFhpShape::N_NODES; ++m)
        if (fhp_is_dec_of(P, m) && fhp_may_load_avg(steady, m) && fhp_completion_rank(steady, P, m) == r) return m;
    return -1;
}
template <int NODE, class C>
PRL_DEV PRL_INLINE void fhp_request_old_average(C& c) {
    if constexpr (NODE >= 0) {
        constexpr int col0 = PrlFhpShape::col0(NODE);
        if (c.template avg_mode<NODE>() == 2)
#pragma unroll
        for (int i = 0; i < PrlFhpShape::nch(NODE); ++i)
        {
            if (c.avg32()) {
                float f[FHP_SLOTS];
                fhp_gload_nt(c.prm->avg32 + c.cofs + (size_t)(col0 + i) * FHP_NP, f);
                for (int k = 0; k < FHP_SLOTS; ++k) c.av_old[col0 + i][k] = (double)f[k];
            } else fhp_gload_nt(c.prm->avg + c.cofs + (size_t)(col0 + i) * FHP_NP, c.av_old[col0 + i]);
        }
    }
}

template <int MODE, int P, int S0, int S1, int NODE, int TC = 0>
struct FhpUp {
    template <class C>
    static PRL_DEV PRL_INLINE void run(C& c, FhpRegs& R, FhpV& ev, FhpV& br) {
        constexpr int kind = PrlFhpShape::kind(NODE);
        const FhpLds& L = c.L;
        if constexpr (kind != PRL_NODE_DECISION) {
            constexpr int slot = PrlFhpShape::term_slot(NODE);
            constexpr int yu = fhp_yord(slot), yb = fhp_y_base(yu), ys = fhp_y_step(yu);
            if constexpr (TC == 2) {
                FhpF ek;
                if constexpr (kind == PRL_NODE_TERM_SHOWDOWN) ek = fhp_lds_load2(L.K + slot * FHP_NPAD, c.p0);
                else { ek[0] = L.y[yb + ys * c.p0]; ek[1] = L.y[yb + ys * (c.p0 + 1)]; }
                ev.v = ek;
                br.v = ek;
                return;
            }
            const float pot = c.prm->pot[NODE];
            const float T = L.Tt[yu];
            FhpF e;
            if constexpr (kind == PRL_NODE_TERM_SHOWDOWN) {
                const float* Pm = L.y + yb;
                FhpF p_gs, p_ge;
                for (int k = 0; k < FHP_SLOTS; ++k) {
                    p_gs[k] = Pm[ys * c.gsm1[k]];
                    p_ge[k] = Pm[ys * c.gem1[k]];
                }
                const FhpF kk = fhp_lds_load2(L.K + slot * FHP_NPAD, c.p0) + fhp_lds_load2(L.K + (FHP_NSHOW + slot) * FHP_NPAD, c.p0);
                const FhpF G = p_gs - (T - p_ge);
                e = G - kk;
            } else {
                const float* Tc = L.Tc + (slot - FHP_NSHOW) * 64;
                FhpF t1, t2;
                for (int k = 0; k < FHP_SLOTS; ++k) {
                    t1[k] = Tc[c.c1[k]];
                    t2[k] = Tc[c.c2[k]];
                }
                FhpF yv;
                if constexpr (ys == 2) {
                    const FhpQ q = *(const FhpQ*)(L.y + (yb & ~1) + 2 * c.p0);
                    yv[0] = q[yb & 1]; yv[1] = q[2 + (yb & 1)];
                } else { yv[0] = L.y[yb + ys * c.p0]; yv[1] = L.y[yb + ys * (c.p0 + 1)]; }
                const FhpF m = t1 + t2;
                e = T - (m - yv);
            }
            e = e * c.eq_const;
            constexpr bool p_folded = kind == PRL_NODE_TERM_FOLD && PrlFhpShape::folder(NODE) == P;
            if constexpr (p_folded) e = -e;
            e = (e * pot) * 0.5f;
            for (int k = 0; k < FHP_SLOTS; ++k) {
                const float ek = c.live[k] ? e[k] : 0.f;
                ev.v[k] = ek;
                br.v[k] = ek;
            }
            if constexpr (TC == 1) {
                if constexpr (kind == PRL_NODE_TERM_SHOWDOWN) fhp_lds_store2(L.K + slot * FHP_NPAD, c.p0, ev.v);
                else { L.y[yb + ys * c.p0] = ev.v[0]; L.y[yb + ys * (c.p0 + 1)] = ev.v[1]; }
            }
        } else {
            constexpr int a = PrlFhpShape::actor(NODE);
            constexpr int A = PrlFhpShape::nch(NODE);
            constexpr int col0 = PrlFhpShape::col0(NODE);
            constexpr bool UPD = a == P && prl_fhp_updates(MODE, P);
            if constexpr (UPD) {
                if (!FHP_AVG_PIPELINED(c)) fhp_request_old_average<NODE>(c);
            }
            FhpV ce[3], cb[3];
            FhpUp<MODE, P, S0, S1, PrlFhpShape::child(NODE, 0), TC>::run(c, R, ce[0], cb[0]);
            FhpUp<MODE, P, S0, S1, PrlFhpShape::child(NODE, 1), TC>::run(c, R, ce[1], cb[1]);
            if constexpr (A > 2) FhpUp<MODE, P, S0, S1, PrlFhpShape::child(NODE, 2), TC>::run(c, R, ce[2], cb[2]);
            if constexpr (a == P) {
                constexpr int SRC = P == 0 ? S0 : S1;
                typedef typename FhpScalar<SRC>::type S;
                S s[3][FHP_SLOTS];
                fhp_node_strategy<SRC, A, S>(c, R, col0, s);
                if constexpr (sizeof(S) == sizeof(float)) {
                    FhpF sv[3];
                    for (int i = 0; i < A; ++i)
                        for (int k = 0; k < FHP_SLOTS; ++k) sv[i][k] = (float)s[i][k];
                    FhpF acc = sv[0] * ce[0].v;
                    for (int i = 1; i < A; ++i) acc = acc + sv[i] * ce[i].v;
                    ev.v = acc;
                } else {
                    for (int k = 0; k < FHP_SLOTS; ++k) {
                        S acc = s[0][k] * (S)ce[0].v[k];
                        for (int i = 1; i < A; ++i) acc = acc + s[i][k] * (S)ce[i].v[k];
                        ev.v[k] = (float)acc;
                    }
                }
                for (int k = 0; k < FHP_SLOTS; ++k) {
                    float mx = cb[0].v[k];
                    for (int i = 1; i < A; ++i) mx = cb[i].v[k] > mx ? cb[i].v[k] : mx;
                    br.v[k] = mx;
                }
                if constexpr (UPD) {
                    float rn[3][FHP_SLOTS];
                    for (int i = 0; i < A; ++i) {
                        const FhpF d = ce[i].v - ev.v;
                        FhpF rv = d;
                        if (!c.first_iteration()) {
                            FhpF old;
                            for (int k = 0; k < FHP_SLOTS; ++k) old[k] = SRC == PRL_SRC_REGRET ? R.rg[col0 + i][k] : 0.f;
                            rv = c.variant() == PRL_CFR_LINEAR ? ((float)(c.iter + 1) * d) + old : d + old;
                        }
                        for (int k = 0; k < FHP_SLOTS; ++k) {
                            float r = rv[k];
                            if (c.variant() == PRL_CFR_PLUS) r = r > 0.f ? r : 0.f;
                            rn[i][k] = r;
                        }
                        fhp_gstore_nt(c.prm->regret + c.cofs + (size_t)(col0 + i) * FHP_NP, rn[i]);
                    }
                    constexpr bool KEEP = MODE == PRL_FHP_UPDATE1_EVAL1;
                    const int avg_mode = c.template avg_mode<NODE>();
                    if (KEEP || avg_mode) {
                        float t[3][FHP_SLOTS], sum[FHP_SLOTS];
                        for (int k = 0; k < FHP_SLOTS; ++k) {
                            sum[k] = 0.f;
                            for (int i = 0; i < A; ++i) {
                                t[i][k] = c.variant() == PRL_CFR_PLUS ? rn[i][k] : (rn[i][k] > 0.f ? rn[i][k] : 0.f);
                                sum[k] = sum[k] + t[i][k];
                            }
                        }
                        float qn[3][FHP_SLOTS];
#if !defined(FHP_DIV_FAST) || defined(FHP_NEWSTRAT_GENERIC)
                        fhp_regret_match<A>(t, sum, qn, false);
#else
                        fhp_regret_match<A>(t, sum, qn, prl_ballot(!fhp_node_in_box<A>(t, sum)) == 0ull);
#endif
                        for (int i = 0; i < A; ++i) {
                            double an[FHP_SLOTS];
                            for (int k = 0; k < FHP_SLOTS; ++k) {
                                const float sn = qn[i][k];
                                if (KEEP) R.rg[col0 + i][k] = sn;
                                double ao = c.av_old[col0 + i][k];
                                if constexpr (SRC == PRL_SRC_REGRET) {
                                    if (c.template avg_catch_up<NODE>()) ao = c.prm->m_old_prev * ao + c.prm->m_new_prev * (double)s[i][k];
                                }
                                an[k] = avg_mode == 2 ? c.prm->m_old * ao + c.prm->m_new * (double)sn : (double)sn;
                            }
                            if (avg_mode) {
                                if (c.avg32()) {
                                    float af[FHP_SLOTS];
                                    for (int k = 0; k < FHP_SLOTS; ++k) af[k] = (float)an[k];
                                    fhp_gstore_nt(c.prm->avg32 + c.cofs + (size_t)(col0 + i) * FHP_NP, af);
                                } else fhp_gstore_nt(c.prm->avg + c.cofs + (size_t)(col0 + i) * FHP_NP, an);
                            }
                        }
                    }
                    if constexpr (fhp_may_load_avg(C::steady, NODE)) {
                        if (FHP_AVG_PIPELINED(c)) fhp_request_old_average<fhp_node_of_rank(C::steady, P, fhp_completion_rank(C::steady, P, NODE) + 2)>(c);
                    }
                }
            } else {
                FhpF acc = ce[0].v, accb = cb[0].v;
                for (int i = 1; i < A; ++i) { acc = acc + ce[i].v; accb = accb + cb[i].v; }
                ev.v = acc;
                br.v = accb;
            }
        }
    }
};

struct FhpSrc { const float* rg; const uint32_t* clx; const int16_t* pp; };
PRL_DEV PRL_INLINE FhpSrc fhp_sources(const PrlFhpParams& prm, int b) {
    FhpSrc s;
    s.rg = prm.regret + (size_t)b * PrlFhpShape::N_COLS * FHP_NP;
    s.clx = prm.plan_clx + (size_t)b * PRL_CLX_WORDS;
    s.pp = prm.plan_pp + (size_t)b * PRL_PP_STRIDE;
    return s;
}

template <int ROWS, int START>
PRL_DEV PRL_INLINE void fhp_prefetch_segment(const void* g, uint32_t lds_addr, int wave, uint32_t lane_off) {
    constexpr int n_waves = FHP_THREADS / 64;
    const int lead = fhp_lead(g);
    int r = wave - START;
    if (r < 0) r += n_waves;
    const char* gw = (const char*)g - 4 * lead + r * 1024;
    const uint32_t lw = lds_addr + (uint32_t)r * 1024u;
#pragma unroll
    for (int i = 0; i * n_waves < ROWS; ++i)
        if ((i + 1) * n_waves <= ROWS || r + i * n_waves < ROWS) prl_lds_dma_x4_a(gw + i * n_waves * 1024, lane_off, lw + (uint32_t)(i * n_waves * 1024));
}

template <bool RG, int SEAT, class C>
PRL_DEV PRL_INLINE void fhp_prefetch(const C& c, int b) {
    const PrlFhpParams& prm = *c.prm;
    constexpr int n_waves = FHP_THREADS / 64;
    const uint32_t lane_off = ((uint32_t)prl_tid() & 63u) * 16u;
    const int wave = c.wave;
    const FhpSrc src = fhp_sources(prm, b);
    constexpr int R_RG = RG ? fhp_seat_rows(SEAT) : 0, R_CLX = FHP_PF_ROWS(PRL_CLX_WORDS), R_PP = FHP_PF_ROWS(FHP_PP_WORDS);
    const uint32_t a0 = c.pf_lds;
    constexpr uint32_t O_CLX = (FHP_RG_IN_LDS ? FHP_PF_RG_WORDS : 0) * 4u, O_PP = O_CLX + FHP_PF_AREA(PRL_CLX_WORDS) * 4u;
    if constexpr (RG) {
        fhp_static_for<0, fhp_n_runs(SEAT)>([&](auto Rn) __attribute__((always_inline)) {
            constexpr int r = decltype(Rn)::value, rows = fhp_run_rows(SEAT, r), row0 = fhp_run_row0(SEAT, r), col0 = fhp_run_col0(SEAT, r);
            fhp_prefetch_segment<rows, row0 % n_waves>(src.rg + (size_t)col0 * FHP_NP, a0 + (uint32_t)row0 * 1024u, wave, lane_off);
        });
    }
    fhp_prefetch_segment<R_CLX, R_RG % n_waves>(src.clx, a0 + O_CLX, wave, lane_off);
    fhp_prefetch_segment<R_PP, (R_RG + R_CLX) % n_waves>(src.pp, a0 + O_PP, wave, lane_off);
}

template <int MODE, int P, int S0, int S1, bool FIRST, class C>
PRL_DEV PRL_INLINE void fhp_seat(C& c, FhpRegs& R, const FhpV& r_opp, FhpV& ev, FhpV& br, int next_b) {
    if (c.active) {
        FhpAvgPre AP;
        if ((P == 0 ? S1 : S0) == PRL_SRC_REGRET && (c.avgsum_mask() & (1 << (1 - P))) && c.prm->avgsum_iter[1 - P] > 0) {
            fhp_for_cols<0>([&](auto J) __attribute__((always_inline)) {
                constexpr int j = decltype(J)::value;
                if constexpr (PrlFhpShape::col_actor(j) == 1 - P) fhp_gload(c.prm->avg_sum + c.cofs + (size_t)j * FHP_NP, AP.v[j]);
            });
        }
        FhpF yv;
        FhpDown<1 - P, S0, S1, 0>::run(c, R, AP, r_opp, yv);
    }
    FHP_SYNC(c, 1);
    if (FIRST && next_b >= 0) fhp_prefetch<fhp_src_in_lds(P == 0 ? S1 : S0), 1 - P>(c, next_b);
    if constexpr (FIRST && fhp_src_f32_block(P == 0 ? S0 : S1) && C::own_after_b(P == 0 ? S1 : S0)) {
        if (c.active) {
            fhp_for_cols<0>([&](auto J) __attribute__((always_inline)) {
                constexpr int j = decltype(J)::value;
                if constexpr (PrlFhpShape::col_actor(j) == P) fhp_gload(c.prm->regret + c.cofs + (size_t)j * FHP_NP, R.rg[j]);
            });
        }
    }
    FHP_TICK(c, 1);
    fhp_scan_phases(c, [&]() {});
    if (FIRST && next_b >= 0 && c.active) {
        const FhpSrc nsrc = fhp_sources(*c.prm, next_b);
        const uint32_t s2 = (c.L.pf_pp + fhp_lead(nsrc.pp))[prl_tid()];
#pragma unroll
        for (int k = 0; k < FHP_SLOTS; ++k) {
            const int sh = (int)((s2 >> (16 * k)) & 0xFFFFu);
            c.nr0[k] = c.prm->chance_reach[sh];
            c.nr1[k] = c.prm->chance_reach[c.prm->R + sh];
        }
    }
    if (FIRST && next_b >= 0) c.nw = c.prm->board_w[next_b];
    FHP_TICK(c, 3);
    if (c.active) {
        if constexpr (prl_fhp_updates(MODE, P)) {
            if (FHP_AVG_PIPELINED(c)) {
                fhp_request_old_average<fhp_node_of_rank(C::steady, P, 0)>(c);
                fhp_request_old_average<fhp_node_of_rank(C::steady, P, 1)>(c);
            }
        }
        if constexpr (MODE == PRL_FHP_UPDATE1_EVAL1) {
            if (FHP_TERMINAL_CACHE(c)) FhpUp<MODE, P, S0, S1, 0, 1>::run(c, R, ev, br);
            else FhpUp<MODE, P, S0, S1, 0>::run(c, R, ev, br);
        } else {
            FhpUp<MODE, P, S0, S1, 0>::run(c, R, ev, br);
        }
    }
    FHP_TICK(c, 4);
}

template <int MODE, int S0, int S1, int STEADY>
FHP_LAUNCH_BOUNDS PRL_GLOBAL void prl_k_fhp_pass(PrlFhpParams prm) {
    constexpr int PF_SEAT = prl_fhp_runs_seat(MODE, 0) ? 1 : 0;
    constexpr bool RG = fhp_src_in_lds(PF_SEAT == 0 ? S0 : S1);
    constexpr bool OWN_AFTER_B = FhpCtxT<STEADY>::own_after_b(PF_SEAT == 0 ? S0 : S1);
    FhpCtxT<STEADY> c;
    c.L = fhp_lds();
    c.prm = &prm;
    c.eq_const = prm.eq_const;
    for (int k = 0; k < FHP_SLOTS; ++k) { c.nr0[k] = 0.f; c.nr1[k] = 0.f; }
    c.nw = 0.f;
    c.variant_ = prm.variant;
    c.iter = prm.iter;
    const int tid = (int)prl_tid();
    c.wave = prl_wave_uniform(tid >> 6);
    c.pf_lds = prl_lds_addr(c.L.pf_rg);
    int per_wg = (prm.n_boards + (int)prl_nblocks() - 1) / (int)prl_nblocks();
    if (prm.block_sum) per_wg = (per_wg + PRL_CHANCE_BLOCK - 1) / PRL_CHANCE_BLOCK * PRL_CHANCE_BLOCK;
    int b = (int)prl_bid() * per_wg;
    const int b_begin = b, b_end = b + per_wg < prm.n_boards ? b + per_wg : prm.n_boards, b_step = 1;
    if (b < b_end) fhp_prefetch<RG, PF_SEAT>(c, b);
    static_assert(PRL_CLX_ZERO_POS == FHP_NPAD - 1, "entries past the end of a card list read the always-zero slot");
    if (tid < FHP_NVEC) c.L.y[fhp_y_base(tid) + fhp_y_step(tid) * (FHP_NPAD - 1)] = 0.f;
    if (tid < FHP_NFOLD * 64) c.L.Tc[tid] = 0.f;
    static_assert(FHP_THREADS * FHP_SLOTS >= FHP_R && FHP_NLIVE < FHP_NPAD - 6, "a lane owns two adjacent positions; trash and zero slots follow the live ones");
    c.p0 = tid * FHP_SLOTS;
    c.active = c.p0 < FHP_NLIVE;
    c.valid = c.p0 < prm.R;
    constexpr int NV = prl_fhp_out_width(MODE);
    auto flush_block = [&](int blk) __attribute__((always_inline)) {
        if (c.valid) {
            float* o = (prm.board_out + (size_t)blk * NV * prm.R) + c.p0;
#pragma unroll
            for (int v = 0; v < NV; ++v) fhp_gstore(o + (size_t)v * prm.R, fhp_lds_load2(c.L.acc + v * FHP_R, c.p0));
        }
    };
#ifdef PRL_FHP_TIMING
    for (int i = 0; i < 6; ++i) c.t_acc[i] = 0;
    c.t_prev = __builtin_readcyclecounter();
#endif
    prl_dma_wait();
    if (b < b_end) {
        prl_sync_lds();
        if (c.active) {
            const uint32_t s2 = (c.L.pf_pp + fhp_lead(fhp_sources(prm, prl_opaque_scalar(b)).pp))[tid];
#pragma unroll
            for (int k = 0; k < FHP_SLOTS; ++k) {
                const int sh = (int)((s2 >> (16 * k)) & 0xFFFFu);
                c.nr0[k] = prm.chance_reach[sh];
                c.nr1[k] = prm.chance_reach[prm.R + sh];
            }
        }
        c.nw = prm.board_w[b];
        for (int k = 0; k < FHP_SLOTS; ++k) {
            float a = c.nr0[k], b2 = c.nr1[k];
            prl_use(a); prl_use(b2);
            c.nr0[k] = a; c.nr1[k] = b2;
        }
        prl_use(c.nw);
    }
    for (int b_iv = b; b_iv < b_end; b_iv += b_step) {
        const int b = prl_opaque_scalar(b_iv);
        c.cofs = (size_t)b * (PrlFhpShape::N_COLS * FHP_NP) + (size_t)c.p0;
        FHP_SYNC(c, 0);
        if (prm.block_sum && b_iv > b_begin && b % PRL_CHANCE_BLOCK == 0) flush_block(b / PRL_CHANCE_BLOCK - 1);
        FhpRegs R;
        FhpV r0, r1;
        const FhpSrc src = fhp_sources(prm, b);
        {
            const uint32_t* lclx = c.L.pf_clx + fhp_lead(src.clx);
            c.rec0 = lclx[2 * tid];
            c.rec1 = lclx[2 * tid + 1];
        }
        const uint32_t* lpp = c.L.pf_pp + fhp_lead(src.pp);
        if (c.valid) {
            const uint32_t s2 = lpp[tid];
            c.sh[0] = (int)(s2 & 0xFFFFu);
            c.sh[1] = (int)(s2 >> 16);
        }
        for (int k = 0; k < FHP_SLOTS; ++k) { r0.v[k] = 0.f; r1.v[k] = 0.f; c.live[k] = false; }
        if (c.active) {
            const uint32_t g2 = lpp[PRL_PP_OFF_GM1 / 2 + tid], e2 = lpp[PRL_PP_OFF_EM1 / 2 + tid], c2 = lpp[PRL_PP_OFF_CC / 2 + tid];
            const float* lrg = c.L.pf_rg + fhp_lead(src.rg);
#pragma unroll
            for (int k = 0; k < FHP_SLOTS; ++k) {
                const bool live = c.p0 + k < FHP_NLIVE;
                c.live[k] = live;
                c.gsm1[k] = (int)((g2 >> (16 * k)) & 0xFFFFu);
                c.gem1[k] = (int)((e2 >> (16 * k)) & 0xFFFFu);
                const uint32_t cc = (c2 >> (16 * k)) & 0xFFFFu;
                c.c1[k] = (int)(cc & 0xFFu);
                c.c2[k] = (int)(cc >> 8);
                const float w = live ? c.nw : 0.f;
                r0.v[k] = c.nr0[k] * w;
                r1.v[k] = c.nr1[k] * w;
            }
            auto request = [&](auto J) __attribute__((always_inline)) {
                constexpr int j = decltype(J)::value;
                constexpr int sj = PrlFhpShape::col_actor(j) == 0 ? S0 : S1;
                constexpr bool from_pf = fhp_src_in_lds(sj) && PrlFhpShape::col_actor(j) == PF_SEAT;
                const size_t col = c.cofs + (size_t)j * FHP_NP;
                if constexpr (sj == PRL_SRC_ARR64 || sj == PRL_SRC_ARR32) fhp_gload(prm.strat_arr + col, R.sa[j]);
                if constexpr (sj == PRL_SRC_AVGF32) {
                    float f[FHP_SLOTS];
                    fhp_gload(prm.avg32 + col, f);
                    for (int k = 0; k < FHP_SLOTS; ++k) R.sa[j][k] = (double)f[k];
                }
                if constexpr (fhp_src_f32_block(sj) && !from_pf && (PrlFhpShape::col_actor(j) == PF_SEAT || !OWN_AFTER_B)) fhp_gload(prm.regret + col, R.rg[j]);
            };
            fhp_for_cols<0>([&](auto J) __attribute__((always_inline)) { if constexpr (PrlFhpShape::col_actor(decltype(J)::value) == PF_SEAT) request(J); });
            fhp_for_cols<0>([&](auto J) __attribute__((always_inline)) { if constexpr (PrlFhpShape::col_actor(decltype(J)::value) != PF_SEAT) request(J); });
            fhp_for_cols<0>([&](auto J) __attribute__((always_inline)) {
                constexpr int j = decltype(J)::value;
                constexpr int sj = PrlFhpShape::col_actor(j) == 0 ? S0 : S1;
                constexpr bool from_pf = fhp_src_in_lds(sj) && PrlFhpShape::col_actor(j) == PF_SEAT;
                if constexpr (from_pf) {
                    constexpr int r = fhp_col_run(j), word0 = fhp_run_row0(PF_SEAT, r) * 256 + (j - fhp_run_col0(PF_SEAT, r)) * FHP_NP;
                    const FhpF v = fhp_lds_load2(lrg + word0, c.p0);
#pragma unroll
                    for (int k = 0; k < FHP_SLOTS; ++k) R.rg[j][k] = v[k];
                }
            });
#if !defined(FHP_DIV_FAST)
            c.fast = false;
#else
#error "FHP_DIV_FAST (measured and rejected in round 2): its board-start box looks at every regret column, and since round 5 the own columns are requested after phase B"
            {
                FhpBox box = fhp_box_empty();
                fhp_for_cols<0>([&](auto J) __attribute__((always_inline)) {
                    constexpr int j = decltype(J)::value;
                    constexpr int sj = PrlFhpShape::col_actor(j) == 0 ? S0 : S1;
                    if constexpr (sj == PRL_SRC_REGRET)
                        for (int k = 0; k < FHP_SLOTS; ++k) {
                            const float r = R.rg[j][k];
                            fhp_box_add(box, c.variant() == PRL_CFR_PLUS ? r : (r > 0.f ? r : 0.f));
                        }
                });
                c.fast = prl_ballot(!fhp_box_ok(box)) == 0ull;
#if defined(FHP_EXPERIMENT)
                c.fast = c.fast && FHP_EXP(c, 2);
#endif
#ifdef PRL_FHP_TIMING
                if (b % 64 == 0 && (tid & 63) == 0) { atomicAdd(c.prm->timing + 6, (unsigned long long)(c.fast ? 1 : 0)); atomicAdd(c.prm->timing + 7, 1ull); }
#endif
            }
#endif
        }
        FHP_TICK(c, 0);
        const int next_b = b_iv + b_step < b_end ? prl_opaque_scalar(b_iv + b_step) : -1;
        FhpV ev0, ev1, br0, br1;
        for (int k = 0; k < FHP_SLOTS; ++k) { ev0.v[k] = 0.f; ev1.v[k] = 0.f; br0.v[k] = 0.f; br1.v[k] = 0.f; }
        if constexpr (!prl_fhp_runs_seat(MODE, 0)) {
            fhp_seat<MODE, 1, S0, S1, true>(c, R, r0, ev1, br1, next_b);
            if constexpr (MODE == PRL_FHP_UPDATE1_EVAL1) {
                if (c.active) {
                    if (FHP_TERMINAL_CACHE(c)) FhpUp<PRL_FHP_EVAL, 1, S0, PRL_SRC_STRAT32, 0, 2>::run(c, R, br0, br1);
                    else FhpUp<PRL_FHP_EVAL, 1, S0, PRL_SRC_STRAT32, 0>::run(c, R, br0, br1);
                }
            }
        } else {
            fhp_seat<MODE, 0, S0, S1, true>(c, R, r1, ev0, br0, next_b);
            if constexpr (prl_fhp_runs_seat(MODE, 1)) {
                FHP_SYNC(c, 4);
                fhp_seat<MODE, 1, S0, S1, false>(c, R, r0, ev1, br1, -1);
            }
        }
        if (c.valid) {
            constexpr bool BOTH = prl_fhp_runs_seat(MODE, 0) && prl_fhp_runs_seat(MODE, 1);
            constexpr int SEAT = prl_fhp_runs_seat(MODE, 0) ? 0 : 1;
            FhpF row[NV];
            if constexpr (BOTH) {
                row[0] = ev0.v; row[1] = ev1.v;
                if constexpr (prl_fhp_with_br(MODE)) { row[2] = br0.v; row[3] = br1.v; }
            } else if constexpr (MODE == PRL_FHP_UPDATE1_EVAL1) {
                row[0] = ev1.v; row[1] = br0.v; row[2] = br1.v;
            } else {
                row[0] = SEAT == 0 ? ev0.v : ev1.v;
                if constexpr (prl_fhp_with_br(MODE)) row[1] = SEAT == 0 ? br0.v : br1.v;
            }
            if (prm.block_sum) {
                const bool first = b % PRL_CHANCE_BLOCK == 0;
#pragma unroll
                for (int k = 0; k < FHP_SLOTS; ++k) {
                    float* a = c.L.acc + c.sh[k];
#pragma unroll
                    for (int v = 0; v < NV; ++v) {
                        const float x = c.live[k] ? row[v][k] : 0.f;
                        a[v * FHP_R] = first ? x : a[v * FHP_R] + x;
                    }
                }
            } else {
                float* o = prm.board_out + (size_t)b * NV * prm.R;
#pragma unroll
                for (int k = 0; k < FHP_SLOTS; ++k)
#pragma unroll
                    for (int v = 0; v < NV; ++v) o[(size_t)v * prm.R + c.sh[k]] = c.live[k] ? row[v][k] : 0.f;
            }
        }
        FHP_TICK(c, 5);
    }
    if (prm.block_sum && b_begin < b_end) {
        prl_sync_lds();
        flush_block((b_end - 1) / PRL_CHANCE_BLOCK);
    }
#ifdef PRL_FHP_TIMING
    if (tid == 0) for (int i = 0; i < 6; ++i) atomicAdd(prm.timing + i, (unsigned long long)c.t_acc[i]);
#endif
}

template <int MODE, int S0, int S1, int STEADY = 0>
static void fhp_launch_t(const PrlFhpParams& prm, int grid, void* stream) {
    PRL_LAUNCH((prl_k_fhp_pass<MODE, S0, S1, STEADY>), grid, FHP_THREADS, FHP_LDS_BYTES, stream, prm);
}

template <int MODE, int STEADY>
static void fhp_launch_split_t(const PrlFhpParams& prm, int grid, void* stream) {
    if constexpr (FHP_AVG_SPLIT) fhp_launch_t<MODE, PRL_SRC_REGRET, PRL_SRC_REGRET, STEADY>(prm, grid, stream);
    else fhp_launch_t<MODE, PRL_SRC_REGRET, PRL_SRC_REGRET>(prm, grid, stream);
}

int launch_pass(const PrlFhpParams& prm, int mode, int src0, int src1, void* stream) {
    if (prm.n_boards <= 0) return PRL_OK;
    if (prm.R != FHP_R) return PRL_ERR_UNSUPPORTED;
    if (((prm.avgsum_mask & 1) && src0 != PRL_SRC_REGRET) || ((prm.avgsum_mask & 2) && src1 != PRL_SRC_REGRET)) return PRL_ERR_UNSUPPORTED;
    static_assert(FHP_NVEC <= 16 && FHP_LDS_BYTES <= 160 * 1024, "terminal vectors + prefetch area of this shape must fit the CU's LDS");
    int grid = prm.n_boards < prm.max_grid ? prm.n_boards : prm.max_grid;
    const int key = mode * 100 + src0 * 10 + src1;
    auto kind_of = [](int pair) { return pair == PRL_FHP_AVG_DEFERRED ? 5 : pair == PRL_FHP_AVG_CATCH_UP ? 6 : 1; };
    const int steady = prm.no_steady || prm.iter == 0 ? 0
                       : (prm.variant == PRL_CFR_PLUS && prm.avg_mode == 2 && prm.avgsum_mask == 0)
                           ? (prm.avg32 ? 4 : fhp_steady_pair(kind_of(prm.avg_pair), kind_of(prm.avg_pair_b)))
                       : (prm.variant == PRL_CFR_LINEAR && prm.avg_mode == 0) ? 2
                       : (prm.variant == PRL_CFR_VANILLA && prm.avg_mode == 0) ? 3 : 0;
    switch (key) {
        case PRL_FHP_UPDATE0 * 100 + PRL_SRC_UNIFORM64 * 10 + PRL_SRC_UNIFORM64: fhp_launch_t<PRL_FHP_UPDATE0, PRL_SRC_UNIFORM64, PRL_SRC_UNIFORM64>(prm, grid, stream); break;
        case PRL_FHP_UPDATE1 * 100 + PRL_SRC_REGRET * 10 + PRL_SRC_UNIFORM64: fhp_launch_t<PRL_FHP_UPDATE1, PRL_SRC_REGRET, PRL_SRC_UNIFORM64>(prm, grid, stream); break;
        case PRL_FHP_UPDATE0 * 100 + PRL_SRC_REGRET * 10 + PRL_SRC_REGRET: fhp_launch_t<PRL_FHP_UPDATE0, PRL_SRC_REGRET, PRL_SRC_REGRET>(prm, grid, stream); break;
        case PRL_FHP_UPDATE1 * 100 + PRL_SRC_REGRET * 10 + PRL_SRC_REGRET: fhp_launch_t<PRL_FHP_UPDATE1, PRL_SRC_REGRET, PRL_SRC_REGRET>(prm, grid, stream); break;
        case PRL_FHP_UPDATE0_EVAL * 100 + PRL_SRC_REGRET * 10 + PRL_SRC_REGRET: fhp_launch_t<PRL_FHP_UPDATE0_EVAL, PRL_SRC_REGRET, PRL_SRC_REGRET>(prm, grid, stream); break;
        case PRL_FHP_UPDATE0_BR * 100 + PRL_SRC_REGRET * 10 + PRL_SRC_REGRET:
            if (steady == 1) fhp_launch_t<PRL_FHP_UPDATE0_BR, PRL_SRC_REGRET, PRL_SRC_REGRET, 1>(prm, grid, stream);
            else if (steady == 4) fhp_launch_t<PRL_FHP_UPDATE0_BR, PRL_SRC_REGRET, PRL_SRC_REGRET, 4>(prm, grid, stream);
            else if (steady == 5) fhp_launch_t<PRL_FHP_UPDATE0_BR, PRL_SRC_REGRET, PRL_SRC_REGRET, 5>(prm, grid, stream);
            else if (steady == 6) fhp_launch_t<PRL_FHP_UPDATE0_BR, PRL_SRC_REGRET, PRL_SRC_REGRET, 6>(prm, grid, stream);
            else if (steady == fhp_steady_pair(5, 1)) fhp_launch_split_t<PRL_FHP_UPDATE0_BR, fhp_steady_pair(5, 1)>(prm, grid, stream);
            else if (steady == fhp_steady_pair(6, 5)) fhp_launch_split_t<PRL_FHP_UPDATE0_BR, fhp_steady_pair(6, 5)>(prm, grid, stream);
            else if (steady == fhp_steady_pair(5, 6)) fhp_launch_split_t<PRL_FHP_UPDATE0_BR, fhp_steady_pair(5, 6)>(prm, grid, stream);
            else if (steady == fhp_steady_pair(6, 1)) fhp_launch_split_t<PRL_FHP_UPDATE0_BR, fhp_steady_pair(6, 1)>(prm, grid, stream);
            else if (steady == fhp_steady_pair(1, 6)) fhp_launch_split_t<PRL_FHP_UPDATE0_BR, fhp_steady_pair(1, 6)>(prm, grid, stream);
            else if (steady == 2) fhp_launch_t<PRL_FHP_UPDATE0_BR, PRL_SRC_REGRET, PRL_SRC_REGRET, 2>(prm, grid, stream);
            else if (steady == 3) fhp_launch_t<PRL_FHP_UPDATE0_BR, PRL_SRC_REGRET, PRL_SRC_REGRET, 3>(prm, grid, stream);
            else fhp_launch_t<PRL_FHP_UPDATE0_BR, PRL_SRC_REGRET, PRL_SRC_REGRET>(prm, grid, stream);
            break;
        case PRL_FHP_UPDATE1_EVAL1 * 100 + PRL_SRC_REGRET * 10 + PRL_SRC_REGRET:
            if (steady == 1) fhp_launch_t<PRL_FHP_UPDATE1_EVAL1, PRL_SRC_REGRET, PRL_SRC_REGRET, 1>(prm, grid, stream);
            else if (steady == 4) fhp_launch_t<PRL_FHP_UPDATE1_EVAL1, PRL_SRC_REGRET, PRL_SRC_REGRET, 4>(prm, grid, stream);
            else if (steady == 5) fhp_launch_t<PRL_FHP_UPDATE1_EVAL1, PRL_SRC_REGRET, PRL_SRC_REGRET, 5>(prm, grid, stream);
            else if (steady == 6) fhp_launch_t<PRL_FHP_UPDATE1_EVAL1, PRL_SRC_REGRET, PRL_SRC_REGRET, 6>(prm, grid, stream);
            else if (steady == fhp_steady_pair(5, 1)) fhp_launch_split_t<PRL_FHP_UPDATE1_EVAL1, fhp_steady_pair(5, 1)>(prm, grid, stream);
            else if (steady == fhp_steady_pair(6, 5)) fhp_launch_split_t<PRL_FHP_UPDATE1_EVAL1, fhp_steady_pair(6, 5)>(prm, grid, stream);
            else if (steady == fhp_steady_pair(5, 6)) fhp_launch_split_t<PRL_FHP_UPDATE1_EVAL1, fhp_steady_pair(5, 6)>(prm, grid, stream);
            else if (steady == fhp_steady_pair(6, 1)) fhp_launch_split_t<PRL_FHP_UPDATE1_EVAL1, fhp_steady_pair(6, 1)>(prm, grid, stream);
            else if (steady == fhp_steady_pair(1, 6)) fhp_launch_split_t<PRL_FHP_UPDATE1_EVAL1, fhp_steady_pair(1, 6)>(prm, grid, stream);
            else if (steady == 2) fhp_launch_t<PRL_FHP_UPDATE1_EVAL1, PRL_SRC_REGRET, PRL_SRC_REGRET, 2>(prm, grid, stream);
            else if (steady == 3) fhp_launch_t<PRL_FHP_UPDATE1_EVAL1, PRL_SRC_REGRET, PRL_SRC_REGRET, 3>(prm, grid, stream);
            else fhp_launch_t<PRL_FHP_UPDATE1_EVAL1, PRL_SRC_REGRET, PRL_SRC_REGRET>(prm, grid, stream);
            break;
        case PRL_FHP_EVAL0 * 100 + PRL_SRC_REGRET * 10 + PRL_SRC_REGRET: fhp_launch_t<PRL_FHP_EVAL0, PRL_SRC_REGRET, PRL_SRC_REGRET>(prm, grid, stream); break;
        case PRL_FHP_EVAL * 100 + PRL_SRC_UNIFORM64 * 10 + PRL_SRC_UNIFORM64: fhp_launch_t<PRL_FHP_EVAL, PRL_SRC_UNIFORM64, PRL_SRC_UNIFORM64>(prm, grid, stream); break;
        case PRL_FHP_EVAL * 100 + PRL_SRC_REGRET * 10 + PRL_SRC_REGRET: fhp_launch_t<PRL_FHP_EVAL, PRL_SRC_REGRET, PRL_SRC_REGRET>(prm, grid, stream); break;
        case PRL_FHP_EVAL * 100 + PRL_SRC_ARR64 * 10 + PRL_SRC_ARR64: fhp_launch_t<PRL_FHP_EVAL, PRL_SRC_ARR64, PRL_SRC_ARR64>(prm, grid, stream); break;
        case PRL_FHP_EVAL * 100 + PRL_SRC_STRAT32 * 10 + PRL_SRC_STRAT32: fhp_launch_t<PRL_FHP_EVAL, PRL_SRC_STRAT32, PRL_SRC_STRAT32>(prm, grid, stream); break;
        case PRL_FHP_EVAL * 100 + PRL_SRC_AVGF32 * 10 + PRL_SRC_AVGF32: fhp_launch_t<PRL_FHP_EVAL, PRL_SRC_AVGF32, PRL_SRC_AVGF32>(prm, grid, stream); break;
        case PRL_FHP_EVAL * 100 + PRL_SRC_ARR32 * 10 + PRL_SRC_ARR32: fhp_launch_t<PRL_FHP_EVAL, PRL_SRC_ARR32, PRL_SRC_ARR32>(prm, grid, stream); break;
        default: return PRL_ERR_UNSUPPORTED;
    }
    return PRL_OK;
}
```

pokerrl_amd/csrc/prl_solver.hip:

```cpp
#include <math.h>
#include <stdlib.h>
#include <string.h>
#if !defined(PRL_EMU)
#include <dlfcn.h>
#include <rccl/rccl.h>
#endif

#include <algorithm>
#include <string>
#include <unordered_map>
#include <vector>

#include "prl_cards.h"
#include "prl_device.h"
#include "prl_fhp.h"
#include "prl_host.h"
#include "prl_kernels.h"
#include "prl_policy.h"
#include "prl_rt.h"
#include "prl_solver_types.h"
#include "prl_st.h"

#define PRL_NODE_LEAF 4

struct prl_solver {
    PrlFlatTree ft;
    PrlDevTree T{};
    PrlDevState S{};
    PrlDevState Seval{};
    bool eval_ready = false;
    hipStream_t stream = nullptr;
    std::vector<void*> allocs;
    std::vector<void*> vmm;
    int32_t* d_term_nodes = nullptr;
    int n_term = 0;
    int32_t* d_nodes_p[2] = {nullptr, nullptr};
    int n_nodes_p[2] = {0, 0};
    int32_t* d_col_node = nullptr;
    int variant = PRL_CFR_PLUS, delay = 0, iter = 0;
    bool ev_valid = false;
    bool root_reach_set[2] = {false, false};
    float* expl_copy_dst = nullptr;
    float* d_expl_hist = nullptr;
    int hist_cap = 0;
    size_t bytes_allocated = 0;
    int full_nodes = 0, full_cols = 0, R = 0;
    bool fused = false;
    int world = 1, rank = 0, xlevel = 0, n_units = 0;
    int n_units_all = 0;
    uint64_t fingerprint = 0;
    prl_exchange_fn exchange = nullptr;
    bool exchange_async = false;
    bool block_sum = true;
    void* exchange_user = nullptr;
    float *d_xlocal = nullptr, *d_xgather = nullptr;
    bool have_half = false;
    float* d_board_out = nullptr;
    float* d_row_sum = nullptr;
    const float* d_board_w = nullptr;
    bool symmetrize = false;
    float* d_row_sym = nullptr;
    const int32_t *d_sym_class_of = nullptr, *d_sym_class_start = nullptr, *d_sym_class_hands = nullptr;
    float* d_half = nullptr;
    PrlIterDev* d_ip = nullptr;
    const int32_t* d_level_start = nullptr;
    bool small_tree = false;
    void* levels_graph_exec = nullptr;
    bool graphs_off = false;
    int avg_pending[2] = {-1, -1};
    bool time_passes = false;
    std::vector<hipEvent_t> pass_events;
    bool expl_pending = false;
    PrlFhpParams fp{};
    int chance_trunk = -1;
    float* d_sum_scratch = nullptr;
    double* d_user_strategy = nullptr;
    float* d_user_strategy32 = nullptr;
    int user_strategy_f64 = -1;
    int src[2] = {PRL_SRC_UNIFORM64, PRL_SRC_UNIFORM64};
    bool board_avg_f64 = false;
    bool board_avg_stale = false;
    bool avg_deferred = false;
    float* d_regret = nullptr;
    double* d_avg = nullptr;
    float* d_avg32 = nullptr;
    bool avg_f32 = false;
    long long n_exchanges = 0;
    long long n_avg_pairs = 0;
    long long n_avg_split_pairs = 0;
    void* rccl_comm = nullptr;
    bool streets = false;
    PrlStPlanHost st;
    PrlStParams sp{};
    struct StLevelDev { PrlStInst* inst = nullptr; } st_dev[PRL_ST_MAX_GROUPS];
    struct StStreetDev { float* leaf_reach = nullptr; float* val = nullptr; } st_str[PRL_ST_MAX_LEVELS + 1];
    PrlFlatTree chain_ft;
    PrlDevTree Tc{};
    float* d_chain_ev = nullptr;
    PrlStChainTerm* d_chain_terms = nullptr;
    PrlStChainBundle* d_chain_bundles = nullptr;
    hipStream_t chain_stream = nullptr;
    hipEvent_t chain_fork = nullptr, chain_join = nullptr;
    std::vector<int32_t> chain_level_start;
    int n_chain_term = 0, n_chain_bundles = 0, n_chain = 0;
    PrlStChainDev chain_dev{};
    int32_t* d_trunk_leaves = nullptr;
    int n_trunk_leaves = 1;
    std::vector<int32_t> col_dfs;
    std::vector<int32_t> col_int;
    bool sorted = false;
    int col_base = 0, ncb = 0;
    size_t board_ofs = 0, col_elems = 0;
    double blk_avg[PRL_FHP_BOARD_MAX_ACTIONS + 1] = {};
    float* d_user_blocked32 = nullptr;
    double* d_user_blocked64 = nullptr;
    char* d_stage = nullptr;
    int stage_boards = 0;
    double* d_fill = nullptr;
};

namespace {

#if !defined(PRL_EMU)
struct PrlVmmRange { void* va; size_t size, chunk; std::vector<hipMemGenericAllocationHandle_t> handles; };
static void* vmm_alloc_shuffled(size_t bytes, size_t chunk, PrlVmmRange* out) {
    int dev = 0;
    if (hipGetDevice(&dev) != hipSuccess) return nullptr;
    hipMemAllocationProp prop = {};
    prop.type = hipMemAllocationTypePinned;
    prop.location.type = hipMemLocationTypeDevice;
    prop.location.id = dev;
    size_t gran = 0;
    if (hipMemGetAllocationGranularity(&gran, &prop, hipMemAllocationGranularityRecommended) != hipSuccess || gran == 0) return nullptr;
    chunk = (chunk + gran - 1) / gran * gran;
    const size_t n = (bytes + chunk - 1) / chunk, size = n * chunk;
    void* va = nullptr;
    if (hipMemAddressReserve(&va, size, chunk, nullptr, 0) != hipSuccess) return nullptr;
    out->va = va; out->size = size; out->chunk = chunk;
    std::vector<size_t> slot(n);
    for (size_t i = 0; i < n; ++i) slot[i] = i;
    unsigned long long x = 0x9E3779B97F4A7C15ull;
    for (size_t i = n; i > 1; --i) { x = x * 6364136223846793005ull + 1442695040888963407ull; std::swap(slot[i - 1], slot[(size_t)((x >> 33) % i)]); }
    bool ok = true;
    for (size_t i = 0; i < n && ok; ++i) {
        hipMemGenericAllocationHandle_t h;
        if (hipMemCreate(&h, chunk, &prop, 0) != hipSuccess) { ok = false; break; }
        out->handles.push_back(h);
        if (hipMemMap((char*)va + slot[i] * chunk, chunk, 0, h, 0) != hipSuccess) ok = false;
    }
    hipMemAccessDesc acc = {};
    acc.location = prop.location;
    acc.flags = hipMemAccessFlagsProtReadWrite;
    if (ok && hipMemSetAccess(va, size, &acc, 1) != hipSuccess) ok = false;
    if (!ok) {
        (void)hipGetLastError();
        (void)hipMemUnmap(va, size);
        for (auto h : out->handles) (void)hipMemRelease(h);
        (void)hipMemAddressFree(va, size);
        out->handles.clear();
        return nullptr;
    }
    return va;
}
static void vmm_free(PrlVmmRange& r) {
    (void)hipMemUnmap(r.va, r.size);
    for (auto h : r.handles) (void)hipMemRelease(h);
    (void)hipMemAddressFree(r.va, r.size);
}
#endif

#if !defined(PRL_EMU)
struct PrlRcclApi {
    ncclResult_t (*GetUniqueId)(ncclUniqueId*) = nullptr;
    ncclResult_t (*CommInitRank)(ncclComm_t*, int, ncclUniqueId, int) = nullptr;
    ncclResult_t (*AllGather)(const void*, void*, size_t, ncclDataType_t, ncclComm_t, hipStream_t) = nullptr;
    ncclResult_t (*CommDestroy)(ncclComm_t) = nullptr;
    const char* (*GetErrorString)(ncclResult_t) = nullptr;
    bool ok = false;
    std::string why, path;
};
static const PrlRcclApi& prl_rccl_api() {
    static PrlRcclApi api = [] {
        PrlRcclApi a;
        void* h = nullptr;
        const char* forced = getenv("PRL_RCCL_LIB");
        if (forced && *forced) {
            h = dlopen(forced, RTLD_NOW | RTLD_GLOBAL);
            if (!h) {
                const char* de = dlerror();
                a.why = std::string("PRL_RCCL_LIB=") + forced + ": " + (de ? de : "dlopen failed");
                return a;
            }
        }
        if (!h) h = dlopen("librccl.so", RTLD_NOW | RTLD_NOLOAD);
        if (!h) h = dlopen("librccl.so.1", RTLD_NOW | RTLD_NOLOAD);
        if (!h) h = dlopen("librccl.so.1", RTLD_NOW | RTLD_GLOBAL);
        if (!h) h = dlopen("/opt/rocm/lib/librccl.so.1", RTLD_NOW | RTLD_GLOBAL);
        if (!h) { a.why = "librccl.so / librccl.so.1 not found (already loaded, on the loader's path, or /opt/rocm/lib); set PRL_RCCL_LIB=<path to librccl.so>"; return a; }
        a.GetUniqueId = (decltype(a.GetUniqueId))dlsym(h, "ncclGetUniqueId");
        a.CommInitRank = (decltype(a.CommInitRank))dlsym(h, "ncclCommInitRank");
        a.AllGather = (decltype(a.AllGather))dlsym(h, "ncclAllGather");
        a.CommDestroy = (decltype(a.CommDestroy))dlsym(h, "ncclCommDestroy");
        a.GetErrorString = (decltype(a.GetErrorString))dlsym(h, "ncclGetErrorString");
        a.ok = a.GetUniqueId && a.CommInitRank && a.AllGather && a.CommDestroy && a.GetErrorString;
        if (!a.ok) a.why = "the RCCL library bound lacks ncclGetUniqueId / ncclCommInitRank / ncclAllGather / ncclCommDestroy / ncclGetErrorString";
        {
            Dl_info di;
            if (a.GetUniqueId && dladdr((void*)a.GetUniqueId, &di) && di.dli_fname) a.path = di.dli_fname;
        }
        return a;
    }();
    return api;
}
static int32_t prl_rccl_exchange(void* user, const void* local_dev, void* gathered_dev, uint64_t bytes_per_rank) {
    prl_solver* s = (prl_solver*)user;
    const ncclResult_t r = prl_rccl_api().AllGather(local_dev, gathered_dev, (size_t)bytes_per_rank, ncclInt8, (ncclComm_t)s->rccl_comm, s->stream);
    if (r != ncclSuccess) { prl_set_error(std::string("ncclAllGather: ") + prl_rccl_api().GetErrorString(r)); return 1; }
    return 0;
}
#endif

template <class T>
int dev_alloc(prl_solver* s, T** p, size_t count, bool plain = false) {
    void* q = nullptr;
    size_t bytes = (count ? count : 1) * sizeof(T);
#if !defined(PRL_EMU)
    static const long vmm_env = getenv("PRL_VMM_SHUFFLE_MB") ? atol(getenv("PRL_VMM_SHUFFLE_MB")) : -1;
    const long vmm_mb = vmm_env >= 0 ? vmm_env : (s->world > 1 ? 2 : 0);
    if (!plain && vmm_mb > 0 && bytes >= ((size_t)32 << 20)) {
        PrlVmmRange* r = new PrlVmmRange();
        q = vmm_alloc_shuffled(bytes + 4096, (size_t)vmm_mb << 20, r);
        if (q) {
            s->vmm.push_back(r);
            s->bytes_allocated += bytes;
            *p = (T*)q;
            return PRL_OK;
        }
        delete r;
    }
#endif
    hipError_t e = hipMalloc(&q, bytes + 4096);
    if (e != hipSuccess) {
// ... 186 lines not shown
                p.avgsum_iter[q] = s->avg_pending[q];
                s->avg_pending[q] = -1;
                s->board_avg_f64 = true;
                s->board_avg_stale = true;
            }
    }
    const int NG = s->st.n_groups, R = p.R, NL0 = s->n_trunk_leaves;
    const int width = prl_fhp_out_width(mode);
    auto level_params = [&](int g) {
        PrlStParams q = p;
        const PrlStLevelHost& H = s->st.group[g];
        q.n_inst = H.n_inst; q.col_base = H.col_base; q.inst = s->st_dev[g].inst;
        q.parent_reach = H.street == 0 ? st.reach : s->st_str[H.street - 1].leaf_reach;
        q.leaf_reach = s->st_str[H.street].leaf_reach;
        q.child_val = s->st_str[H.street + 1].val;
        q.child_w = width;
        q.val = s->st_str[H.street].val;
#ifdef PRL_ST_TIMING
        if (H.last == (getenv("PRL_ST_TIMING_INNER") != nullptr)) q.timing = nullptr;
#else
        q.timing = nullptr;
#endif
        return q;
    };
    auto side_by_side = [&](int g0, int g1, auto&& launch) -> int {
        for (int g = g0; g < g1; ++g) {
            const int e = launch(g, s->stream);
            if (e) return e;
        }
        return PRL_OK;
    };
    auto street_end = [&](int g0) { int g1 = g0; while (g1 < NG && s->st.group[g1].street == s->st.group[g0].street) ++g1; return g1; };
    for (int g0 = 0; g0 < NG;) {
        const int g1 = street_end(g0);
        if (!s->st.group[g0].last) {
            const int e = side_by_side(g0, g1, [&](int g, hipStream_t on) { return prl_launch_st_down(s->st.group[g].spec, level_params(g), src0, src1, on); });
            if (e) { if (e != PRL_ERR_HIP) prl_set_error("street engine: unsupported strategy-source combination"); return e; }
        }
        g0 = g1;
    }
    if (s->n_chain) {
        PrlStChainIo io = {};
        for (int v = 0; v <= PRL_ST_MAX_LEVELS; ++v) {
            io.src[v] = v == 0 ? st.reach : s->st_str[v - 1].leaf_reach;
            io.val[v] = s->st_str[v].val;
        }
        if (s->chain_stream) {
            PRL_HIP_TRY(hipEventRecord(s->chain_fork, s->stream));
            PRL_HIP_TRY(hipStreamWaitEvent(s->chain_stream, s->chain_fork, 0));
        }
        prl_launch_st_chain_eval(s->Tc, s->d_chain_terms, s->d_chain_bundles, s->n_chain_bundles, io, s->chain_dev, s->d_chain_ev, s->chain_level_start.data(), mode,
                                 s->chain_stream ? s->chain_stream : s->stream);
        if (s->chain_stream) PRL_HIP_TRY(hipEventRecord(s->chain_join, s->chain_stream));
    }
    bool chain_joined = !(s->n_chain && s->chain_stream);
    for (int g1 = NG; g1 > 0;) {
        int g0 = g1 - 1;
        while (g0 > 0 && s->st.group[g0 - 1].street == s->st.group[g1 - 1].street) --g0;
        if (s->st.group[g0].last) {
            for (int g = g1 - 1; g >= g0; --g) {
                hipEvent_t ev0 = nullptr, ev1 = nullptr;
                const bool timed = s->time_passes;
                if (timed) {
                    PRL_HIP_TRY(hipEventCreate(&ev0));
                    PRL_HIP_TRY(hipEventCreate(&ev1));
                    PRL_HIP_TRY(hipEventRecord(ev0, s->stream));
                }
                const int e = prl_launch_st_pass(s->st.group[g].spec, true, level_params(g), mode, src0, src1, s->stream);
                if (e) { prl_set_error("street engine: unsupported pass mode / strategy-source combination"); return e; }
                if (timed) {
                    PRL_HIP_TRY(hipEventRecord(ev1, s->stream));
                    s->pass_events.push_back(ev0);
                    s->pass_events.push_back(ev1);
                }
            }
        } else {
            if (!chain_joined) {
                PRL_HIP_TRY(hipStreamWaitEvent(s->stream, s->chain_join, 0));
                chain_joined = true;
            }
            const int e = side_by_side(g0, g1, [&](int g, hipStream_t on) { return prl_launch_st_pass(s->st.group[g].spec, false, level_params(g), mode, src0, src1, on); });
            if (e) { if (e != PRL_ERR_HIP) prl_set_error("street engine: unsupported pass mode / strategy-source combination"); return e; }
        }
        g1 = g0;
    }
    if (!chain_joined) PRL_HIP_TRY(hipStreamWaitEvent(s->stream, s->chain_join, 0));
    const int W = NL0 * width * R, n_top = s->st.n_top;
    float* summed = s->d_row_sum;
    const float* rows = s->st_str[0].val;
    if (!s->exchange) prl_launch_fhp_chance_sum(rows, n_top, W, s->d_sum_scratch, summed, s->stream);
    else {
        const size_t per_rank = (size_t)s->n_units * W;
        prl_launch_fhp_chance_partial(rows, n_top, s->xlevel, W, s->d_sum_scratch, s->d_xlocal, s->stream);
        if (!s->exchange_async) PRL_HIP_TRY(hipStreamSynchronize(s->stream));
        ++s->n_exchanges;
        if (s->exchange(s->exchange_user, s->d_xlocal, s->d_xgather, (uint64_t)(per_rank * sizeof(float))) != 0) {
            prl_set_error("sharded solve: the exchange callback failed");
            return PRL_ERR_STATE;
        }
        prl_launch_fhp_chance_finish(s->d_xgather, s->n_units_all, s->xlevel, W, s->d_sum_scratch, summed, s->stream);
    }
    const bool both = prl_fhp_runs_seat(mode, 0) && prl_fhp_runs_seat(mode, 1);
    const int seat = prl_fhp_runs_seat(mode, 0) ? 0 : 1;
    const bool with_br = prl_fhp_with_br(mode);
    PrlStScatter sc = {};
    sc.n_vec = width;
    auto add = [&](int src, int arr, int dst_seat) { sc.src_vec[sc.n_dst] = src; sc.dst_arr[sc.n_dst] = arr; sc.dst_seat[sc.n_dst] = dst_seat; ++sc.n_dst; };
    if (both) {
        add(0, 0, 0); add(1, 0, 1);
        add(with_br ? 2 : 0, 1, 0); add(with_br ? 3 : 1, 1, 1);
    } else if (mode == PRL_FHP_UPDATE1_EVAL1) {
        add(0, 0, 1); add(0, 1, 1);
        add(1, 2, 0); add(2, 2, 1);
    } else {
        add(0, 0, seat); add(with_br ? 1 : 0, 1, seat);
    }
    prl_launch_st_scatter_trunk(summed, s->d_trunk_leaves, NL0, R, sc, st.ev, st.ev_br, s->d_half, s->stream);
    if (!both && mode != PRL_FHP_UPDATE1_EVAL1 && seat == 0 && with_br && s->have_half && &st == &s->S)
        prl_launch_st_half_to_trunk(s->d_half, s->d_trunk_leaves, NL0, R, st.ev, st.ev_br, s->stream);
    PRL_HIP_TRY(hipGetLastError());
    return PRL_OK;
}

int fused_board_pass(prl_solver* s, const PrlDevState& st, int mode, int src0, int src1, const double* strat_arr, const float* strat32 = nullptr) {
    if (s->streets) return street_sweep(s, st, mode, src0, src1, strat_arr, strat32);
    PrlFhpParams p = s->fp;
    p.regret = (strat32 ? const_cast<float*>(strat32) : s->d_regret) + s->board_ofs;
    p.iter = s->iter;
    p.variant = s->variant;
    p.chance_reach = st.reach + prl_vidx(s->T, s->chance_trunk, 0);
    p.strat_arr = strat_arr ? strat_arr + s->board_ofs : nullptr;
    p.avg_sum = s->S.avg_sum ? s->S.avg_sum + s->board_ofs : nullptr;
    p.avg = s->avg_f32 ? nullptr : s->d_avg + s->board_ofs;
    p.avg32 = s->d_avg32 ? s->d_avg32 + s->board_ofs : nullptr;
    p.avgsum_mask = 0;
    p.block_sum = (s->block_sum && (!s->exchange || s->xlevel >= 1)) ? 1 : 0;
    if (&st == &s->S && strat_arr == nullptr) {
        const bool walks[2] = {prl_fhp_runs_seat(mode, 1), prl_fhp_runs_seat(mode, 0)};
        for (int q = 0; q < 2; ++q)
            if (walks[q] && s->avg_pending[q] >= 0) {
                p.avgsum_mask |= 1 << q;
                p.avgsum_iter[q] = s->avg_pending[q];
                s->avg_pending[q] = -1;
                s->board_avg_f64 = true;
                s->board_avg_stale = true;
            }
    }
    hipEvent_t ev0 = nullptr, ev1 = nullptr;
    if (s->time_passes) {
        PRL_HIP_TRY(hipEventCreate(&ev0));
        PRL_HIP_TRY(hipEventCreate(&ev1));
        PRL_HIP_TRY(hipEventRecord(ev0, s->stream));
    }
    int e = prl_launch_fhp_pass(p, mode, src0, src1, s->stream);
    if (e) { prl_set_error("fused engine: unsupported strategy-source combination"); return e; }
    if (s->time_passes) {
        PRL_HIP_TRY(hipEventRecord(ev1, s->stream));
        s->pass_events.push_back(ev0);
        s->pass_events.push_back(ev1);
    }
    const bool both = prl_fhp_runs_seat(mode, 0) && prl_fhp_runs_seat(mode, 1);
    const int seat = prl_fhp_runs_seat(mode, 0) ? 0 : 1;
    const bool with_br = prl_fhp_with_br(mode);
    const int W = prl_fhp_out_width(mode) * p.R;
    float* summed = s->d_row_sum;
    const int n_blk = (p.n_boards + PRL_CHANCE_BLOCK - 1) / PRL_CHANCE_BLOCK;
    if (!s->exchange) {
        if (p.block_sum) prl_launch_fhp_chance_finish(s->d_board_out, n_blk, 1, W, s->d_sum_scratch, summed, s->stream);
        else prl_launch_fhp_chance_sum(s->d_board_out, p.n_boards, W, s->d_sum_scratch, summed, s->stream);
    } else {
        const size_t per_rank = (size_t)s->n_units * W;
        if (p.block_sum) prl_launch_fhp_chance_partial_from_blocks(s->d_board_out, n_blk, s->xlevel, W, s->d_xlocal, s->stream);
        else prl_launch_fhp_chance_partial(s->d_board_out, p.n_boards, s->xlevel, W, s->d_sum_scratch, s->d_xlocal, s->stream);
        if (!s->exchange_async) PRL_HIP_TRY(hipStreamSynchronize(s->stream));
        ++s->n_exchanges;
        if (s->exchange(s->exchange_user, s->d_xlocal, s->d_xgather, (uint64_t)(per_rank * sizeof(float))) != 0) {
            prl_set_error("sharded solve: the exchange callback failed");
            return PRL_ERR_STATE;
        }
        prl_launch_fhp_chance_finish(s->d_xgather, s->n_units_all, s->xlevel, W, s->d_sum_scratch, summed, s->stream);
    }
    if (s->symmetrize) {
        prl_launch_fhp_symmetrize(summed, prl_fhp_out_width(mode), p.R, s->d_sym_class_of, s->d_sym_class_start, s->d_sym_class_hands, s->d_row_sym, s->stream);
        summed = s->d_row_sym;
    }
    const size_t vec = (size_t)p.R * sizeof(float);
    float* ch_ev = st.ev + prl_vidx(s->T, s->chance_trunk, 0);
    float* ch_br = st.ev_br + prl_vidx(s->T, s->chance_trunk, 0);
    auto put = [&](float* dst, int k, int n_vec) { return hipMemcpyAsync(dst, summed + (size_t)k * p.R, n_vec * vec, hipMemcpyDeviceToDevice, s->stream); };
    if (both) {
        PRL_HIP_TRY(put(ch_ev, 0, 2));
        PRL_HIP_TRY(put(ch_br, with_br ? 2 : 0, 2));
    } else if (mode == PRL_FHP_UPDATE1_EVAL1) {
        PRL_HIP_TRY(put(ch_ev + p.R, 0, 1));
        PRL_HIP_TRY(put(ch_br + p.R, 0, 1));
        PRL_HIP_TRY(put(s->d_half, 1, 2));
    } else {
        PRL_HIP_TRY(put(ch_ev + (size_t)seat * p.R, 0, 1));
        PRL_HIP_TRY(put(ch_br + (size_t)seat * p.R, with_br ? 1 : 0, 1));
        if (seat == 0 && with_br && s->have_half && &st == &s->S) {
            PRL_HIP_TRY(hipMemcpyAsync(ch_ev + p.R, s->d_half, vec, hipMemcpyDeviceToDevice, s->stream));
            PRL_HIP_TRY(hipMemcpyAsync(ch_br + p.R, s->d_half + p.R, vec, hipMemcpyDeviceToDevice, s->stream));
        }
    }
    PRL_HIP_TRY(hipGetLastError());
    return PRL_OK;
}

int do_compute_ev(prl_solver* s, const PrlDevState& st, int fused_mode = PRL_FHP_EVAL) {
    float* const expl_dst = &st == &s->S ? s->expl_copy_dst : nullptr;
    if (&st == &s->S) s->expl_copy_dst = nullptr;
    if (s->fused) {
        const double* arr = nullptr;
        int s0 = s->src[0], s1 = s->src[1];
        const float* arr32 = nullptr;
        if (s->user_strategy_f64 == 1) {
            arr = s->d_user_strategy;
            s0 = s1 = PRL_SRC_ARR64;
        } else if (s->user_strategy_f64 == 0) {
            arr32 = s->d_user_strategy32;
            s0 = s1 = PRL_SRC_STRAT32;
        }
        TRY(fused_board_pass(s, st, fused_mode, s0, s1, arr, arr32));
    }
    prl_launch_ev(s->T, st, s->ft.level_start.data(), s->d_term_nodes, s->n_term, s->stream, expl_dst);
    PRL_HIP_TRY(hipGetLastError());
    return PRL_OK;
}

int ensure_ev(prl_solver* s) {
    if (s->ev_valid) return PRL_OK;
    TRY(do_compute_ev(s, s->S));
    s->ev_valid = true;
    return PRL_OK;
}

int ensure_hist(prl_solver* s, int need) {
    if (need <= s->hist_cap) return PRL_OK;
    int cap = s->hist_cap ? s->hist_cap : 1024;
    while (cap < need) cap *= 2;
    float* q = nullptr;
    TRY(dev_alloc(s, &q, (size_t)cap * 2));
    if (s->d_expl_hist && s->hist_cap) PRL_HIP_TRY(hipMemcpyAsync(q, s->d_expl_hist, (size_t)s->hist_cap * 2 * sizeof(float), hipMemcpyDeviceToDevice, s->stream));
    s->d_expl_hist = q;
    s->hist_cap = cap;
    return PRL_OK;
}

int expl_to_history(prl_solver* s) {
    TRY(ensure_hist(s, s->iter + 1));
    s->expl_copy_dst = s->d_expl_hist + (size_t)s->iter * 2;
    return PRL_OK;
}

int record_expl(prl_solver* s) {
    TRY(ensure_hist(s, s->iter + 1));
    PRL_HIP_TRY(hipMemcpyAsync(s->d_expl_hist + (size_t)s->iter * 2, s->S.expl, 2 * sizeof(float), hipMemcpyDeviceToDevice, s->stream));
    return PRL_OK;
}

void make_trunk(const PrlFlatTree& t, int chance_node, int first_board_node, int board_nodes_total, PrlFlatTree* out, int* chance_trunk) {
    PrlFlatTree& u = *out;
    u = PrlFlatTree();
    u.rules = t.rules;
    u.game = t.game;
    std::vector<int> map(t.n_nodes, -1);
    for (int i = 0; i < t.n_nodes; ++i) {
        if (i >= first_board_node && i < first_board_node + board_nodes_total) continue;
        map[i] = u.n_nodes++;
        const bool is_ch = i == chance_node;
        u.kind.push_back(is_ch ? PRL_NODE_LEAF : t.kind[i]);
        u.actor.push_back(t.actor[i]);
        u.parent.push_back(t.parent[i] < 0 ? -1 : map[t.parent[i]]);
        u.child_idx.push_back(t.child_idx[i]);
        u.action.push_back(t.action[i]);
        u.acted_last.push_back(t.acted_last[i]);
        u.round.push_back(t.round[i]);
        u.board_id.push_back(-1);
        u.main_pot.push_back(t.main_pot[i]);
        u.depth.push_back(t.depth[i]);
        u.n_children.push_back(is_ch ? 0 : t.n_children[i]);
        u.first_col.push_back(t.first_col[i]);
        u.subtree_size.push_back(1);
    }
    *chance_trunk = map[chance_node];
    u.n_cols = 0;
    for (int i = 0; i < u.n_nodes; ++i)
        if (u.kind[i] == PRL_NODE_DECISION) u.n_cols += u.n_children[i];
    for (int c = 0; c < u.n_cols; ++c) { u.col_action.push_back(t.col_action[c]); u.col_node.push_back(map[t.col_node[c]]); }
    u.n_boards = 0;
    u.board_len = t.board_len;
    u.child_start.assign(u.n_nodes + 1, 0);
    for (int i = 0; i < u.n_nodes; ++i) u.child_start[i + 1] = u.child_start[i] + u.n_children[i];
    u.child_list.assign(u.child_start[u.n_nodes], -1);
    int max_depth = 0;
    for (int i = 1; i < u.n_nodes; ++i) {
        u.child_list[u.child_start[u.parent[i]] + u.child_idx[i]] = i;
        max_depth = max_depth > u.depth[i] ? max_depth : u.depth[i];
    }
    u.n_levels = max_depth + 1;
    u.level_start.assign(u.n_levels + 1, 0);
    for (int i = 0; i < u.n_nodes; ++i) u.level_start[u.depth[i] + 1]++;
    for (int d = 0; d < u.n_levels; ++d) u.level_start[d + 1] += u.level_start[d];
    u.level_nodes.assign(u.n_nodes, 0);
    std::vector<int32_t> fill(u.level_start.begin(), u.level_start.end() - 1);
    for (int i = 0; i < u.n_nodes; ++i) u.level_nodes[fill[u.depth[i]]++] = i;
}

// ... 1465 lines not shown
        PRL_HIP_TRY(hipMemcpyAsync(o, src + (size_t)c * cb, (size_t)n * cb, hipMemcpyDeviceToHost, s->stream));
        o += (size_t)n * cb; c += n;
    }
    if (c < c_end) {
        const int b_first = (int)((c - s->col_base) / s->ncb), b_last = (int)((c_end - 1 - s->col_base) / s->ncb);
        const bool whole = (c - s->col_base) % s->ncb == 0 && (c_end - s->col_base) % s->ncb == 0;
        const char* region = src + s->board_ofs * elem;
        if (whole) TRY(sorted_get_boards(s, region, (int)elem, fill, nullptr, o, (int)elem, b_first, b_last - b_first + 1));
        else {
            std::vector<char> tmp((size_t)(b_last - b_first + 1) * s->ncb * cb);
            TRY(sorted_get_boards(s, region, (int)elem, fill, nullptr, tmp.data(), (int)elem, b_first, b_last - b_first + 1));
            memcpy(o, tmp.data() + (size_t)(c - s->col_base - (int64_t)b_first * s->ncb) * cb, (size_t)(c_end - c) * cb);
        }
    }
    return prl_solver_sync(s);
}

int32_t prl_solver_get(prl_solver_t* s, int32_t field, void* out) {
    if (!s || !out) { prl_set_error("NULL argument"); return PRL_ERR_ARG; }
    const size_t nv = (size_t)s->T.n_nodes * 2 * s->T.R, nc = (size_t)s->full_cols * s->R;
    const void* src = nullptr;
    size_t bytes = 0;
    const bool node_vectors = field == PRL_SF_REACH || field == PRL_SF_EV || field == PRL_SF_EV_BR || field == PRL_SF_BR_IDX ||
                              field == PRL_SF_STRAT_F64 || field == PRL_SF_AVG_F64;
    if (s->fused && node_vectors) {
        prl_set_error("the fused engine keeps per-node vectors on chip; create the solver with PRL_ENGINE_LEVELS to read them");
        return PRL_ERR_UNSUPPORTED;
    }
    switch (field) {
        case PRL_SF_REACH: src = s->S.reach; bytes = nv * 4; break;
        case PRL_SF_EV: TRY(ensure_ev(s)); src = s->S.ev; bytes = nv * 4; break;
        case PRL_SF_EV_BR: TRY(ensure_ev(s)); src = s->S.ev_br; bytes = nv * 4; break;
        case PRL_SF_STRATEGY:
            if (s->sorted) {
                const size_t tcb = (size_t)s->T.n_cols * s->R;
                double* o = (double*)out;
                double fill[PRL_FHP_MAX_NODES * 3];
                if (s->user_strategy_f64 == 1) {
                    PRL_HIP_TRY(hipMemcpyAsync(o, s->d_user_strategy, tcb * 8, hipMemcpyDeviceToHost, s->stream));
                    TRY(sorted_get_boards(s, s->d_user_strategy + s->board_ofs, 8, nullptr, s->d_user_blocked64, o + tcb, 8, 0, s->fp.n_boards));
                    return prl_solver_sync(s);
                }
                if (s->user_strategy_f64 == 0) {
                    std::vector<float> f(tcb);
                    PRL_HIP_TRY(hipStreamSynchronize(s->stream));
                    PRL_HIP_TRY(hipMemcpy(f.data(), s->d_user_strategy32, tcb * 4, hipMemcpyDeviceToHost));
                    for (size_t i = 0; i < tcb; ++i) o[i] = (double)f[i];
                    TRY(sorted_get_boards(s, s->d_user_strategy32 + s->board_ofs, 4, nullptr, s->d_user_blocked32, o + tcb, 8, 0, s->fp.n_boards));
                    return prl_solver_sync(s);
                }
                if (s->src[0] != PRL_SRC_REGRET || s->src[1] != PRL_SRC_REGRET) {
                    prl_set_error("fused engine: strategy is the implicit uniform fill until both seats have been updated");
                    return PRL_ERR_STATE;
                }
                if (!s->d_user_strategy) TRY(dev_alloc(s, &s->d_user_strategy, col_array_elems(s)));
                PrlFhpParams fp = s->fp;
                fp.variant = s->variant;
                fp.regret = s->d_regret + s->board_ofs;
                prl_launch_fhp_strategy_from_regret(fp, s->d_user_strategy + s->board_ofs, s->stream);
                PRL_HIP_TRY(hipMemcpyAsync(o, s->S.strategy, tcb * 8, hipMemcpyDeviceToHost, s->stream));
                for (int j = 0; j < s->ncb; ++j) fill[j] = (double)(float)(1.0 / (double)board_col_actions(s, j));
                TRY(sorted_get_boards(s, s->d_user_strategy + s->board_ofs, 8, fill, nullptr, o + tcb, 8, 0, s->fp.n_boards));
                return prl_solver_sync(s);
            }
            if (s->fused) {
                if (s->user_strategy_f64 == 1) { src = s->d_user_strategy; bytes = nc * 8; break; }
                if (s->user_strategy_f64 == 0) {
                    std::vector<float> f(nc);
                    PRL_HIP_TRY(hipStreamSynchronize(s->stream));
                    PRL_HIP_TRY(hipMemcpy(f.data(), s->d_user_strategy32, nc * 4, hipMemcpyDeviceToHost));
                    double* o = (double*)out;
                    if (s->col_dfs.empty()) for (size_t i = 0; i < nc; ++i) o[i] = (double)f[i];
                    else
                        for (int c = 0; c < s->full_cols; ++c)
                            for (int h = 0; h < s->R; ++h) o[(size_t)s->col_dfs[c] * s->R + h] = (double)f[(size_t)c * s->R + h];
                    return PRL_OK;
                }
                if (s->src[0] != PRL_SRC_REGRET || s->src[1] != PRL_SRC_REGRET) {
                    prl_set_error("fused engine: strategy is the implicit uniform fill until both seats have been updated");
                    return PRL_ERR_STATE;
                }
                if (!s->d_user_strategy) TRY(dev_alloc(s, &s->d_user_strategy, nc));
                PRL_HIP_TRY(hipMemcpyAsync(s->d_user_strategy, s->S.strategy, (size_t)s->T.n_cols * s->R * 8, hipMemcpyDeviceToDevice, s->stream));
                if (s->streets) {
                    for (int lv = 0; lv < s->st.n_groups; ++lv) {
                        PrlStParams q = s->sp;
                        q.n_inst = s->st.group[lv].n_inst; q.col_base = s->st.group[lv].col_base; q.regret = s->d_regret; q.variant = s->variant;
                        prl_launch_st_strategy_from_regret(q, s->st.group[lv].spec, s->d_user_strategy, s->stream);
                    }
                } else {
                    PrlFhpParams fp = s->fp;
                    fp.variant = s->variant;
                    prl_launch_fhp_strategy_from_regret(fp, s->d_user_strategy, s->stream);
                }
                src = s->d_user_strategy; bytes = nc * 8;
                break;
            }
            src = s->S.strategy; bytes = nc * 8; break;
        case PRL_SF_STRAT_F64: src = s->S.strat_f64; bytes = (size_t)s->T.n_nodes; break;
        case PRL_SF_REGRET:
            if (s->sorted) {
                const size_t tcb = (size_t)s->T.n_cols * s->R;
                PRL_HIP_TRY(hipMemcpyAsync(out, s->d_regret, tcb * 4, hipMemcpyDeviceToHost, s->stream));
                TRY(sorted_get_boards(s, s->d_regret + s->board_ofs, 4, nullptr, nullptr, (float*)out + tcb, 4, 0, s->fp.n_boards));
                return prl_solver_sync(s);
            }
            src = s->d_regret; bytes = nc * 4; break;
        case PRL_SF_AVG:
            if (s->sorted) {
                const size_t tcb = (size_t)s->T.n_cols * s->R;
                double fill[PRL_FHP_MAX_NODES * 3];
                TRY(ensure_board_avg(s));
                blocked_avg_fill(s, fill);
                PRL_HIP_TRY(hipMemcpyAsync(out, s->d_avg, tcb * 8, hipMemcpyDeviceToHost, s->stream));
                if (s->avg_f32) TRY(sorted_get_boards(s, s->d_avg32 + s->board_ofs, 4, fill, nullptr, (double*)out + tcb, 8, 0, s->fp.n_boards));
                else TRY(sorted_get_boards(s, s->d_avg + s->board_ofs, 8, fill, nullptr, (double*)out + tcb, 8, 0, s->fp.n_boards));
                return prl_solver_sync(s);
            }
            if (s->avg_f32 && s->streets) {
                const size_t tcb = (size_t)s->T.n_cols * s->R;
                std::vector<float> f(nc);
                std::vector<double> tr(tcb);
                PRL_HIP_TRY(hipStreamSynchronize(s->stream));
                PRL_HIP_TRY(hipMemcpy(f.data(), s->d_avg32, nc * 4, hipMemcpyDeviceToHost));
                PRL_HIP_TRY(hipMemcpy(tr.data(), s->d_avg, tcb * 8, hipMemcpyDeviceToHost));
                double* o = (double*)out;
                for (int c = 0; c < s->full_cols; ++c) {
                    double* dst = o + (size_t)(s->col_dfs.empty() ? c : s->col_dfs[c]) * s->R;
                    if (c < s->T.n_cols) memcpy(dst, tr.data() + (size_t)c * s->R, (size_t)s->R * 8);
                    else for (int h = 0; h < s->R; ++h) dst[h] = (double)f[(size_t)c * s->R + h];
                }
                return PRL_OK;
            }
            TRY(ensure_board_avg(s)); src = s->d_avg; bytes = nc * 8; break;
        case PRL_SF_AVG_F64: src = s->S.avg_f64; bytes = (size_t)s->T.n_nodes; break;
        case PRL_SF_AVG_SUM:
            if (s->sorted && s->S.avg_sum) {
                const size_t tcb = (size_t)s->T.n_cols * s->R;
                PRL_HIP_TRY(hipMemcpyAsync(out, s->S.avg_sum, tcb * 4, hipMemcpyDeviceToHost, s->stream));
                TRY(sorted_get_boards(s, s->S.avg_sum + s->board_ofs, 4, nullptr, nullptr, (float*)out + tcb, 4, 0, s->fp.n_boards));
                return prl_solver_sync(s);
            }
            src = s->S.avg_sum; bytes = nc * 4; break;
        case PRL_SF_BR_IDX: TRY(ensure_ev(s)); src = s->S.br_idx; bytes = (size_t)s->T.n_nodes * s->T.R * 4; break;
        case PRL_SF_EXPL_HISTORY: src = s->d_expl_hist; bytes = (size_t)(s->iter + 1) * 2 * 4; break;
        case PRL_SF_ITER: *(int32_t*)out = s->iter; return PRL_OK;
        case PRL_SF_CONSTANTS: ((float*)out)[0] = s->T.chance_prob; ((float*)out)[1] = s->T.eq_const; return PRL_OK;
        case PRL_SF_BYTES_ALLOCATED: *(int64_t*)out = (int64_t)s->bytes_allocated; return PRL_OK;
        case PRL_SF_ENGINE: *(int32_t*)out = s->fused ? PRL_ENGINE_FUSED : PRL_ENGINE_LEVELS; return PRL_OK;
        case PRL_SF_GRAPH_REPLAY: *(int32_t*)out = s->levels_graph_exec != nullptr; return PRL_OK;
        case PRL_SF_EXCHANGES: *(int64_t*)out = (int64_t)s->n_exchanges; return PRL_OK;
        case PRL_SF_AVG_PAIRS: *(int64_t*)out = (int64_t)s->n_avg_pairs; return PRL_OK;
        case PRL_SF_AVG_SPLIT_PAIRS: *(int64_t*)out = (int64_t)s->n_avg_split_pairs; return PRL_OK;
        case PRL_SF_VMM_RANGES: {
            int64_t bytes = 0;
#if !defined(PRL_EMU)
            for (void* r : s->vmm) bytes += (int64_t)((PrlVmmRange*)r)->size;
#endif
            ((int64_t*)out)[0] = (int64_t)s->vmm.size(); ((int64_t*)out)[1] = bytes; return PRL_OK;
        }
        case PRL_SF_EXPLICIT_STRATEGY: *(int32_t*)out = s->fused ? s->user_strategy_f64 : -1; return PRL_OK;
        default: prl_set_error("unknown solver field"); return PRL_ERR_ARG;
    }
    if (!src) { prl_set_error("field not available for this variant"); return PRL_ERR_STATE; }
    const bool col_field = field == PRL_SF_STRATEGY || field == PRL_SF_REGRET || field == PRL_SF_AVG || field == PRL_SF_AVG_SUM;
    if (col_field && !s->col_dfs.empty()) {
        std::vector<char> tmp(bytes);
        PRL_HIP_TRY(hipMemcpyAsync(tmp.data(), src, bytes, hipMemcpyDeviceToHost, s->stream));
        TRY(prl_solver_sync(s));
        const size_t cb = bytes / (size_t)s->full_cols;
        for (int c = 0; c < s->full_cols; ++c) memcpy((char*)out + (size_t)s->col_dfs[c] * cb, tmp.data() + (size_t)c * cb, cb);
        return PRL_OK;
    }
    PRL_HIP_TRY(hipMemcpyAsync(out, src, bytes, hipMemcpyDeviceToHost, s->stream));
    return prl_solver_sync(s);
}

}

namespace {
PRL_GLOBAL void PRL_LAUNCH_BOUNDS(256) prl_k_table_fill(const void* cols, int elem, int R, int n_rows_here, int period, int cols_per_rep, const int32_t* col0,
                                                        const int32_t* nch, const int32_t* col_action, int n_actions, long long row0, float* probs, const int32_t* row_id) {
    const long long i = (long long)prl_bid() * prl_nthreads() + prl_tid();
    if (i >= (long long)n_rows_here * R) return;
    const int r = (int)(i / R), h = (int)(i - (long long)r * R);
    const int rep = r / period, t = r - rep * period;
    const long long row = row0 + (row_id ? row_id[r] : r);
    for (int j = 0; j < nch[t]; ++j) {
        const size_t at = ((size_t)rep * cols_per_rep + col0[t] + j) * R + h;
        const float v = elem == 8 ? (float)((const double*)cols)[at] : ((const float*)cols)[at];
        probs[((size_t)row * n_actions + col_action[col0[t] + j]) * R + h] = v;
    }
}

struct TableReplay {
    const PrlFlatTree& t;
    uint32_t seed;
    std::vector<LbrbHistKey> key_of;
    std::vector<int32_t> twin_of;
    std::vector<int32_t> rows;
    TableReplay(const PrlFlatTree& tree, uint32_t key_seed) : t(tree), seed(key_seed), key_of(tree.n_nodes), twin_of(tree.n_nodes, -1) {}
    void walk(int id, const PrlEnvState& st, const LbrbHistKey& parent_key) {
        const int8_t* row = t.board_id[id] >= 0 ? t.boards.data() + (size_t)t.board_id[id] * t.board_len : nullptr;
        int n_dealt = 0;
        for (int c = 0; row && c < t.board_len; ++c) n_dealt += row[c] >= 0;
        int8_t none[PRL_MAX_BOARD_CARDS] = {0, 0, 0, 0, 0};
        key_of[id] = lbrb_hist_step(parent_key, st, row ? row : none, n_dealt, t.rules.n_board_cards, t.rules.n_suits);
        if (t.n_children[id] == 0) return;
        rows.push_back(id);
        for (int i = 0; i < t.n_children[id]; ++i) {
            const int c = t.child_list[t.child_start[id] + i];
            PrlEnvState s2 = st;
            PrlStepInfo info;
            prl_env_step(t.game, s2, t.col_action[t.first_col[id] + i], &info);
            if (info.is_terminal) continue;
            if (t.kind[c] == PRL_NODE_CHANCE) {
                for (int k = 0; k < t.n_children[c]; ++k) walk(t.child_list[t.child_start[c] + k], s2, key_of[id]);
            } else walk(c, s2, key_of[id]);
        }
    }
};
}

namespace {
PRL_GLOBAL void PRL_LAUNCH_BOUNDS(256) prl_k_cols_from_node_probs(const float* probs, int R, int A, const int32_t* col_k, const int32_t* col_a, long long n_cols_here,
                                                                  float* dst32, double* dst64) {
    const long long i = (long long)prl_bid() * prl_nthreads() + prl_tid();
    if (i >= n_cols_here * R) return;
    const long long c = i / R;
    const int h = (int)(i - c * R);
    const float v = probs[((size_t)col_k[c] * R + h) * A + col_a[c]];
    if (dst32) dst32[(size_t)c * R + h] = v;
    if (dst64) dst64[(size_t)c * R + h] = (double)v;
}
}

extern "C" int32_t prl_solver_set_strategy_device(prl_solver_t* s, const prl_tree_t* tree, const float* d_probs, int32_t n_actions) {
    if (!s || !tree || !d_probs || n_actions < 2) { prl_set_error("bad argument"); return PRL_ERR_ARG; }
    const PrlFlatTree& full = *prl_tree_flat(tree);
    if (full.n_nodes != s->full_nodes || full.n_cols != s->full_cols || full.rules.range_size != s->R) { prl_set_error("prl_solver_set_strategy_device: not the tree this solver was created on"); return PRL_ERR_ARG; }
    std::vector<int32_t> ord(full.n_nodes, -1), maps((size_t)2 * s->full_cols);
    int n_dec = 0;
    for (int n = 0; n < full.n_nodes; ++n)
        if (full.kind[n] == PRL_NODE_DECISION) ord[n] = n_dec++;
    for (int ci = 0; ci < s->full_cols; ++ci) {
        const int c = s->col_dfs.empty() ? ci : s->col_dfs[ci];
        if (full.col_action[c] < 0 || full.col_action[c] >= n_actions) { prl_set_error("prl_solver_set_strategy_device: the tree has an action outside [0, n_actions)"); return PRL_ERR_ARG; }
        maps[ci] = ord[full.col_node[c]];
        maps[(size_t)s->full_cols + ci] = full.col_action[c];
    }
    int32_t* d_maps = nullptr;
    PRL_HIP_TRY(hipMalloc((void**)&d_maps, maps.size() * sizeof(int32_t)));
    auto fail = [&](int code) { (void)hipFree(d_maps); return code; };
#define SD_TRY(x) do { if ((x) != hipSuccess) { (void)hipGetLastError(); prl_set_error("HIP error in prl_solver_set_strategy_device"); return fail(PRL_ERR_HIP); } } while (0)
    SD_TRY(hipMemcpy(d_maps, maps.data(), maps.size() * sizeof(int32_t), hipMemcpyHostToDevice));
    const int32_t *d_k = d_maps, *d_a = d_maps + s->full_cols;
    const int R = s->R;
    auto launch = [&](long long c0, long long n, float* d32, double* d64) {
        if (n <= 0) return;
        PRL_LAUNCH(prl_k_cols_from_node_probs, (unsigned)((n * R + 255) / 256), 256, 0, s->stream, d_probs, R, (int)n_actions, d_k + c0, d_a + c0, n, d32, d64);
    };
    const long long tc = s->T.n_cols;
    launch(0, tc, nullptr, s->S.strategy);
    if (s->sorted) {
        const size_t ne = col_array_elems(s), nblk = (size_t)s->fp.n_boards * s->ncb * PRL_FHP_NBLOCKED;
        int rc = PRL_OK;
        if (!s->d_user_strategy32) rc = dev_alloc(s, &s->d_user_strategy32, ne);
        if (!rc && !s->d_user_blocked32) rc = dev_alloc(s, &s->d_user_blocked32, nblk);
        if (!rc) rc = stage_ready(s);
        if (rc) return fail(rc);
        launch(0, tc, s->d_user_strategy32, nullptr);
        for (int at = 0; at < s->fp.n_boards; at += s->stage_boards) {
            const int nb = s->fp.n_boards - at < s->stage_boards ? s->fp.n_boards - at : s->stage_boards;
            launch((long long)s->col_base + (long long)at * s->ncb, (long long)nb * s->ncb, (float*)s->d_stage, nullptr);
            prl_launch_fhp_compact(s->fp, s->d_stage, 4, at, nb, s->d_user_strategy32 + s->board_ofs, s->d_user_blocked32, s->stream);
            SD_TRY(hipGetLastError());
        }
        s->user_strategy_f64 = 0;
    } else if (s->fused) {
        if (!s->d_user_strategy32) { const int rc = dev_alloc(s, &s->d_user_strategy32, (size_t)s->full_cols * R); if (rc) return fail(rc); }
        launch(0, s->full_cols, s->d_user_strategy32, nullptr);
        s->user_strategy_f64 = 0;
    }
    SD_TRY(hipGetLastError());
    SD_TRY(hipMemsetAsync(s->S.strat_f64, 0, (size_t)s->T.n_nodes, s->stream));
    SD_TRY(hipStreamSynchronize(s->stream));
#undef SD_TRY
    (void)hipFree(d_maps);
    s->ev_valid = false;
    return do_update_reach(s, s->S);
}

extern "C" int32_t prl_policy_table_from_solver(prl_solver_t* s, const prl_tree_t* tree, uint32_t key_seed, prl_policy_table_t** out) {
    if (!s || !tree || !out) { prl_set_error("NULL argument"); return PRL_ERR_ARG; }
    *out = nullptr;
    const PrlFlatTree& full = *prl_tree_flat(tree);
    if (full.n_nodes != s->full_nodes || full.n_cols != s->full_cols || full.rules.range_size != s->R) { prl_set_error("prl_policy_table_from_solver: not the tree this solver was created on"); return PRL_ERR_ARG; }
    if (s->world > 1) { prl_set_error("prl_policy_table_from_solver: an unsharded solve (a rank of a sharded one holds its share of the boards only)"); return PRL_ERR_UNSUPPORTED; }
    if (s->fused && s->user_strategy_f64 >= 0) { prl_set_error("prl_policy_table_from_solver: an explicit strategy is loaded; the table is made of a CFR run's average"); return PRL_ERR_STATE; }
    if (s->iter < 1 || (s->variant == PRL_CFR_PLUS && s->iter <= s->delay)) { prl_set_error("prl_policy_table_from_solver: no average strategy yet (iterate first; CFR+ starts averaging after `delay` iterations)"); return PRL_ERR_STATE; }
    if (s->fused) {
        TRY(ensure_ev(s));
        if (s->avg_pending[0] >= 0 || s->avg_pending[1] >= 0) { prl_set_error("prl_policy_table_from_solver: iteration not closed"); return PRL_ERR_STATE; }
    }
    TRY(ensure_board_avg(s));
    TableReplay rp(full, key_seed);
// ... 149 lines not shown
```

Measured before the change: 202.3 million.

## Fuse seat-1 update and new-strategy evaluation into one tree walk; add steady specializations

For the UPDATE1_EVAL1 pass on shape 15, the regret-update walk now also carries a second value vector computed from the freshly updated strategy. This replaces the separate second tree walk that re-evaluated seat 1 with the new strategy, and avoids keeping the new regrets in registers. The UPDATE0 and EVAL0 passes also dispatch to steady-state template specializations when the CFR+ conditions hold. A counter of steady passes taken is exposed through a new solver field. The cost is an extra value vector per node during the combined walk, which raises register pressure, plus more template instantiations.

```diff
diff --git a/include/pokerrl_hip.h b/include/pokerrl_hip.h
--- a/include/pokerrl_hip.h
+++ b/include/pokerrl_hip.h
@@ -262,6 +262,7 @@
     PRL_SF_VMM_RANGES = 18,
     PRL_SF_AVG_PAIRS = 19,
     PRL_SF_AVG_SPLIT_PAIRS = 20,
+    PRL_SF_STEADY_ENDS = 21,
     PRL_SF_EXPLICIT_STRATEGY = 16
 };
 int32_t prl_solver_get(prl_solver_t* solver, int32_t field, void* out);
diff --git a/pokerrl_amd/_native.py b/pokerrl_amd/_native.py
--- a/pokerrl_amd/_native.py
+++ b/pokerrl_amd/_native.py
@@ -549,7 +549,7 @@
 OBS_VANILLA, OBS_HISTORY, OBS_FLAT_HU_LIMIT = 0, 1, 2
 
 SF = dict(reach=0, ev=1, ev_br=2, strategy=3, strat_f64=4, regret=5, avg=6, avg_f64=7, avg_sum=8, br_idx=9,
-          expl_history=10, iter=11, constants=12, bytes_allocated=13, engine=14, graph_replay=15, explicit_strategy=16, exchanges=17, vmm_ranges=18, avg_pairs=19, avg_split_pairs=20)
+          expl_history=10, iter=11, constants=12, bytes_allocated=13, engine=14, graph_replay=15, explicit_strategy=16, exchanges=17, vmm_ranges=18, avg_pairs=19, avg_split_pairs=20, steady_ends=21)
 VARIANTS = {"vanilla": 0, "plus": 1, "linear": 2}
 ENGINES = {"auto": 0, "levels": 1, "fused": 2}
 
@@ -806,7 +806,7 @@
             "avg": ((c, R), np.float64), "avg_f64": ((n,), np.uint8), "avg_sum": ((c, R), np.float32),
             "br_idx": ((n, R), np.int32), "constants": ((2,), np.float32), "bytes_allocated": ((1,), np.int64),
             "explicit_strategy": ((1,), np.int32), "exchanges": ((1,), np.int64), "vmm_ranges": ((2,), np.int64),
-            "avg_pairs": ((1,), np.int64), "avg_split_pairs": ((1,), np.int64),
+            "avg_pairs": ((1,), np.int64), "avg_split_pairs": ((1,), np.int64), "steady_ends": ((2,), np.int64),
         }.get(name, (None, None))
         if name == "expl_history":
             shape, dtype = (self.iter + 1, 2), np.float32
diff --git a/pokerrl_amd/csrc/prl_fhp.h b/pokerrl_amd/csrc/prl_fhp.h
--- a/pokerrl_amd/csrc/prl_fhp.h
+++ b/pokerrl_amd/csrc/prl_fhp.h
@@ -188,7 +188,7 @@
 
 int prl_fhp_match_shape(const PrlFlatTree& t, int* chance_node, int* first_board_node, int* col_base, float* pots );
 
-int prl_launch_fhp_pass(const PrlFhpParams& prm, int mode, int src0, int src1, void* stream);
+int prl_launch_fhp_pass(const PrlFhpParams& prm, int mode, int src0, int src1, void* stream, int* steady_taken = nullptr);
 bool prl_fhp_avg_split_supported(int shape_id);
 void prl_launch_fhp_strategy_from_regret(const PrlFhpParams& prm, double* out_region, void* stream);
 void prl_launch_fhp_avg_from_sum(const PrlFhpParams& prm, void* stream);
diff --git a/pokerrl_amd/csrc/prl_fhp_kernels.hip b/pokerrl_amd/csrc/prl_fhp_kernels.hip
--- a/pokerrl_amd/csrc/prl_fhp_kernels.hip
+++ b/pokerrl_amd/csrc/prl_fhp_kernels.hip
@@ -15,6 +15,8 @@
 #define FHP_SLOTS 2
 #define FHP_LAUNCH_BOUNDS FHP_LB(768, 3)
 #define FHP_AVG_SPLIT 1
+#define FHP_ONE_WALK 1
+#define FHP_STEADY_EVAL0 1
 #define FHP_SPEC PrlFhpSpec15
 namespace fhp_shape15 {
 #include "prl_fhp_pass.inc"
@@ -28,6 +30,10 @@
 #if !defined(PRL_FHP_NO_SHAPE21)
 #undef FHP_AVG_SPLIT
 #define FHP_AVG_SPLIT 0
+#undef FHP_ONE_WALK
+#define FHP_ONE_WALK 0
+#undef FHP_STEADY_EVAL0
+#define FHP_STEADY_EVAL0 0
 #define FHP_SPEC PrlFhpSpec21
 namespace fhp_shape21 {
 #include "prl_fhp_pass.inc"
@@ -38,6 +44,8 @@
 #undef FHP_SLOTS
 #undef FHP_LAUNCH_BOUNDS
 #undef FHP_AVG_SPLIT
+#undef FHP_ONE_WALK
+#undef FHP_STEADY_EVAL0
 
 bool prl_fhp_avg_split_supported(int shape_id) { return shape_id == PRL_FHP_SHAPE_15 || shape_id == PRL_FHP_SHAPE_9; }
 
@@ -72,12 +80,12 @@
     PRL_LAUNCH(prl_k_fhp_symmetrize, (n + 255) / 256, 256, 0, stream, in, n_vec, R, class_of, class_start, class_hands, out);
 }
 
-int prl_launch_fhp_pass(const PrlFhpParams& prm, int mode, int src0, int src1, void* stream) {
+int prl_launch_fhp_pass(const PrlFhpParams& prm, int mode, int src0, int src1, void* stream, int* steady_taken) {
     switch (prm.shape) {
-        case PRL_FHP_SHAPE_15: return fhp_shape15::launch_pass(prm, mode, src0, src1, stream);
-        case PRL_FHP_SHAPE_9: return fhp_shape9::launch_pass(prm, mode, src0, src1, stream);
+        case PRL_FHP_SHAPE_15: return fhp_shape15::launch_pass(prm, mode, src0, src1, stream, steady_taken);
+        case PRL_FHP_SHAPE_9: return fhp_shape9::launch_pass(prm, mode, src0, src1, stream, steady_taken);
 #if !defined(PRL_FHP_NO_SHAPE21)
-        case PRL_FHP_SHAPE_21: return fhp_shape21::launch_pass(prm, mode, src0, src1, stream);
+        case PRL_FHP_SHAPE_21: return fhp_shape21::launch_pass(prm, mode, src0, src1, stream, steady_taken);
 #endif
         default: return PRL_ERR_UNSUPPORTED;
     }
diff --git a/pokerrl_amd/csrc/prl_fhp_pass.inc b/pokerrl_amd/csrc/prl_fhp_pass.inc
--- a/pokerrl_amd/csrc/prl_fhp_pass.inc
+++ b/pokerrl_amd/csrc/prl_fhp_pass.inc
@@ -207,6 +207,12 @@
     if (steady == 0) return true;
     const int k = fhp_set_kind(steady, fhp_avg_set(n));
     return k == 1 || k == 4 || k == 6;
+}
+constexpr bool fhp_one_walk(int steady) { return FHP_ONE_WALK && (steady == 1 || steady == 5 || steady == 6 || steady >= FHP_STEADY_PAIR0); }
+constexpr bool fhp_own_below(int P, int n) {
+    for (int m = n; m < n + PrlFhpShape::subtree_size(n); ++m)
+        if (PrlFhpShape::kind(m) == PRL_NODE_DECISION && PrlFhpShape::actor(m) == P) return true;
+    return false;
 }
 template <int STEADY>
 struct FhpCtxT {
@@ -459,7 +465,7 @@
         }
         const float pj = carry + incl[LAST];
         if (show && lane < LAST_LANES) y[st * 64 * LAST] = pj;
-        if (lane == LAST_LANES - 1) L.Tt[v] = pj;
+        if (lane == LAST_LANES - 1) L.Tt[prl_opaque_lane(v)] = pj;
     };
     for (int v = wave; v < FHP_NVEC; v += n_waves) {
         if (v < 2 * FHP_NPAIRS) range_prefix(std::integral_constant<int, 2>(), v);
@@ -505,7 +511,9 @@
 template <int MODE, int P, int S0, int S1, int NODE, int TC = 0>
 struct FhpUp {
     template <class C>
-    static PRL_DEV PRL_INLINE void run(C& c, FhpRegs& R, FhpV& ev, FhpV& br) {
+    static PRL_DEV PRL_INLINE void run(C& c, FhpRegs& R, FhpV& ev, FhpV& en, FhpV& br) {
+        constexpr bool ONE = TC == 3;
+        static_assert(!ONE || (MODE == PRL_FHP_UPDATE1_EVAL1 && (P == 0 ? S0 : S1) == PRL_SRC_REGRET), "one walk: the update pass that also evaluates the new strategy");
         constexpr int kind = PrlFhpShape::kind(NODE);
         const FhpLds& L = c.L;
         if constexpr (kind != PRL_NODE_DECISION) {
@@ -556,6 +564,7 @@
                 ev.v[k] = ek;
                 br.v[k] = ek;
             }
+            if constexpr (ONE) en.v = ev.v;
             if constexpr (TC == 1) {
                 if constexpr (kind == PRL_NODE_TERM_SHOWDOWN) fhp_lds_store2(L.K + slot * FHP_NPAD, c.p0, ev.v);
                 else { L.y[yb + ys * c.p0] = ev.v[0]; L.y[yb + ys * (c.p0 + 1)] = ev.v[1]; }
@@ -568,10 +577,10 @@
             if constexpr (UPD) {
                 if (!FHP_AVG_PIPELINED(c)) fhp_request_old_average<NODE>(c);
             }
-            FhpV ce[3], cb[3];
-            FhpUp<MODE, P, S0, S1, PrlFhpShape::child(NODE, 0), TC>::run(c, R, ce[0], cb[0]);
-            FhpUp<MODE, P, S0, S1, PrlFhpShape::child(NODE, 1), TC>::run(c, R, ce[1], cb[1]);
-            if constexpr (A > 2) FhpUp<MODE, P, S0, S1, PrlFhpShape::child(NODE, 2), TC>::run(c, R, ce[2], cb[2]);
+            FhpV ce[3], cn[3], cb[3];
+            FhpUp<MODE, P, S0, S1, PrlFhpShape::child(NODE, 0), TC>::run(c, R, ce[0], cn[0], cb[0]);
+            FhpUp<MODE, P, S0, S1, PrlFhpShape::child(NODE, 1), TC>::run(c, R, ce[1], cn[1], cb[1]);
+            if constexpr (A > 2) FhpUp<MODE, P, S0, S1, PrlFhpShape::child(NODE, 2), TC>::run(c, R, ce[2], cn[2], cb[2]);
             if constexpr (a == P) {
                 constexpr int SRC = P == 0 ? S0 : S1;
                 typedef typename FhpScalar<SRC>::type S;
@@ -634,7 +643,7 @@
                             double an[FHP_SLOTS];
                             for (int k = 0; k < FHP_SLOTS; ++k) {
                                 const float sn = qn[i][k];
-                                if (KEEP) R.rg[col0 + i][k] = sn;
+                                if (KEEP && !ONE) R.rg[col0 + i][k] = sn;
                                 double ao = c.av_old[col0 + i][k];
                                 if constexpr (SRC == PRL_SRC_REGRET) {
                                     if (c.template avg_catch_up<NODE>()) ao = c.prm->m_old_prev * ao + c.prm->m_new_prev * (double)s[i][k];
@@ -649,6 +658,14 @@
                                 } else fhp_gstore_nt(c.prm->avg + c.cofs + (size_t)(col0 + i) * FHP_NP, an);
                             }
                         }
+                        if constexpr (ONE) {
+                            FhpF qv[3];
+                            for (int i = 0; i < A; ++i)
+                                for (int k = 0; k < FHP_SLOTS; ++k) qv[i][k] = qn[i][k];
+                            FhpF accn = qv[0] * cn[0].v;
+                            for (int i = 1; i < A; ++i) accn = accn + qv[i] * cn[i].v;
+                            en.v = accn;
+                        }
                     }
                     if constexpr (fhp_may_load_avg(C::steady, NODE)) {
                         if (FHP_AVG_PIPELINED(c)) fhp_request_old_average<fhp_node_of_rank(C::steady, P, fhp_completion_rank(C::steady, P, NODE) + 2)>(c);
@@ -659,6 +676,13 @@
                 for (int i = 1; i < A; ++i) { acc = acc + ce[i].v; accb = accb + cb[i].v; }
                 ev.v = acc;
                 br.v = accb;
+                if constexpr (ONE) {
+                    if constexpr (fhp_own_below(P, NODE)) {
+                        FhpF accn = cn[0].v;
+                        for (int i = 1; i < A; ++i) accn = accn + cn[i].v;
+                        en.v = accn;
+                    } else en.v = acc;
+                }
             }
         }
     }
@@ -707,7 +731,7 @@
 }
 
 template <int MODE, int P, int S0, int S1, bool FIRST, class C>
-PRL_DEV PRL_INLINE void fhp_seat(C& c, FhpRegs& R, const FhpV& r_opp, FhpV& ev, FhpV& br, int next_b) {
+PRL_DEV PRL_INLINE void fhp_seat(C& c, FhpRegs& R, const FhpV& r_opp, FhpV& ev, FhpV& en, FhpV& br, int next_b) {
     if (c.active) {
         FhpAvgPre AP;
         if ((P == 0 ? S1 : S0) == PRL_SRC_REGRET && (c.avgsum_mask() & (1 << (1 - P))) && c.prm->avgsum_iter[1 - P] > 0) {
@@ -750,11 +774,13 @@
                 fhp_request_old_average<fhp_node_of_rank(C::steady, P, 1)>(c);
             }
         }
-        if constexpr (MODE == PRL_FHP_UPDATE1_EVAL1) {
-            if (FHP_TERMINAL_CACHE(c)) FhpUp<MODE, P, S0, S1, 0, 1>::run(c, R, ev, br);
-            else FhpUp<MODE, P, S0, S1, 0>::run(c, R, ev, br);
+        if constexpr (MODE == PRL_FHP_UPDATE1_EVAL1 && fhp_one_walk(C::steady)) {
+            FhpUp<MODE, P, S0, S1, 0, 3>::run(c, R, ev, en, br);
+        } else if constexpr (MODE == PRL_FHP_UPDATE1_EVAL1) {
+            if (FHP_TERMINAL_CACHE(c)) FhpUp<MODE, P, S0, S1, 0, 1>::run(c, R, ev, en, br);
+            else FhpUp<MODE, P, S0, S1, 0>::run(c, R, ev, en, br);
         } else {
-            FhpUp<MODE, P, S0, S1, 0>::run(c, R, ev, br);
+            FhpUp<MODE, P, S0, S1, 0>::run(c, R, ev, en, br);
         }
     }
     FHP_TICK(c, 4);
@@ -791,9 +817,10 @@
     constexpr int NV = prl_fhp_out_width(MODE);
     auto flush_block = [&](int blk) __attribute__((always_inline)) {
         if (c.valid) {
-            float* o = (prm.board_out + (size_t)blk * NV * prm.R) + c.p0;
-#pragma unroll
-            for (int v = 0; v < NV; ++v) fhp_gstore(o + (size_t)v * prm.R, fhp_lds_load2(c.L.acc + v * FHP_R, c.p0));
+            const int p0 = prl_opaque_lane(c.p0);
+            float* o = (prm.board_out + (size_t)blk * NV * prm.R) + p0;
+#pragma unroll
+            for (int v = 0; v < NV; ++v) fhp_gstore(o + (size_t)v * prm.R, fhp_lds_load2(c.L.acc + v * FHP_R, p0));
         }
     };
 #ifdef PRL_FHP_TIMING
@@ -822,7 +849,7 @@
     }
     for (int b_iv = b; b_iv < b_end; b_iv += b_step) {
         const int b = prl_opaque_scalar(b_iv);
-        c.cofs = (size_t)b * (PrlFhpShape::N_COLS * FHP_NP) + (size_t)c.p0;
+        c.cofs = (size_t)b * (PrlFhpShape::N_COLS * FHP_NP) + (size_t)prl_opaque_lane(c.p0);
         FHP_SYNC(c, 0);
         if (prm.block_sum && b_iv > b_begin && b % PRL_CHANCE_BLOCK == 0) flush_block(b / PRL_CHANCE_BLOCK - 1);
         FhpRegs R;
@@ -912,18 +939,20 @@
         FhpV ev0, ev1, br0, br1;
         for (int k = 0; k < FHP_SLOTS; ++k) { ev0.v[k] = 0.f; ev1.v[k] = 0.f; br0.v[k] = 0.f; br1.v[k] = 0.f; }
         if constexpr (!prl_fhp_runs_seat(MODE, 0)) {
-            fhp_seat<MODE, 1, S0, S1, true>(c, R, r0, ev1, br1, next_b);
-            if constexpr (MODE == PRL_FHP_UPDATE1_EVAL1) {
+            fhp_seat<MODE, 1, S0, S1, true>(c, R, r0, ev1, br0, br1, next_b);
+            if constexpr (MODE == PRL_FHP_UPDATE1_EVAL1 && !fhp_one_walk(STEADY)) {
                 if (c.active) {
-                    if (FHP_TERMINAL_CACHE(c)) FhpUp<PRL_FHP_EVAL, 1, S0, PRL_SRC_STRAT32, 0, 2>::run(c, R, br0, br1);
-                    else FhpUp<PRL_FHP_EVAL, 1, S0, PRL_SRC_STRAT32, 0>::run(c, R, br0, br1);
+                    FhpV en_unused;
+                    if (FHP_TERMINAL_CACHE(c)) FhpUp<PRL_FHP_EVAL, 1, S0, PRL_SRC_STRAT32, 0, 2>::run(c, R, br0, en_unused, br1);
+                    else FhpUp<PRL_FHP_EVAL, 1, S0, PRL_SRC_STRAT32, 0>::run(c, R, br0, en_unused, br1);
                 }
             }
         } else {
-            fhp_seat<MODE, 0, S0, S1, true>(c, R, r1, ev0, br0, next_b);
+            FhpV en_unused;
+            fhp_seat<MODE, 0, S0, S1, true>(c, R, r1, ev0, en_unused, br0, next_b);
             if constexpr (prl_fhp_runs_seat(MODE, 1)) {
                 FHP_SYNC(c, 4);
-                fhp_seat<MODE, 1, S0, S1, false>(c, R, r0, ev1, br1, -1);
+                fhp_seat<MODE, 1, S0, S1, false>(c, R, r0, ev1, en_unused, br1, -1);
             }
         }
         if (c.valid) {
@@ -980,7 +1009,8 @@
     else fhp_launch_t<MODE, PRL_SRC_REGRET, PRL_SRC_REGRET>(prm, grid, stream);
 }
 
-int launch_pass(const PrlFhpParams& prm, int mode, int src0, int src1, void* stream) {
+int launch_pass(const PrlFhpParams& prm, int mode, int src0, int src1, void* stream, int* steady_taken) {
+    if (steady_taken) *steady_taken = 0;
     if (prm.n_boards <= 0) return PRL_OK;
     if (prm.R != FHP_R) return PRL_ERR_UNSUPPORTED;
     if (((prm.avgsum_mask & 1) && src0 != PRL_SRC_REGRET) || ((prm.avgsum_mask & 2) && src1 != PRL_SRC_REGRET)) return PRL_ERR_UNSUPPORTED;
@@ -993,10 +1023,18 @@
                            ? (prm.avg32 ? 4 : fhp_steady_pair(kind_of(prm.avg_pair), kind_of(prm.avg_pair_b)))
                        : (prm.variant == PRL_CFR_LINEAR && prm.avg_mode == 0) ? 2
                        : (prm.variant == PRL_CFR_VANILLA && prm.avg_mode == 0) ? 3 : 0;
+    const bool steady_eval = FHP_STEADY_EVAL0 && !prm.no_steady && prm.iter > 0 && prm.variant == PRL_CFR_PLUS && prm.avgsum_mask == 0;
+    int taken = 0;
     switch (key) {
         case PRL_FHP_UPDATE0 * 100 + PRL_SRC_UNIFORM64 * 10 + PRL_SRC_UNIFORM64: fhp_launch_t<PRL_FHP_UPDATE0, PRL_SRC_UNIFORM64, PRL_SRC_UNIFORM64>(prm, grid, stream); break;
         case PRL_FHP_UPDATE1 * 100 + PRL_SRC_REGRET * 10 + PRL_SRC_UNIFORM64: fhp_launch_t<PRL_FHP_UPDATE1, PRL_SRC_REGRET, PRL_SRC_UNIFORM64>(prm, grid, stream); break;
-        case PRL_FHP_UPDATE0 * 100 + PRL_SRC_REGRET * 10 + PRL_SRC_REGRET: fhp_launch_t<PRL_FHP_UPDATE0, PRL_SRC_REGRET, PRL_SRC_REGRET>(prm, grid, stream); break;
+        case PRL_FHP_UPDATE0 * 100 + PRL_SRC_REGRET * 10 + PRL_SRC_REGRET:
+            taken = steady;
+            if (steady == 1) fhp_launch_t<PRL_FHP_UPDATE0, PRL_SRC_REGRET, PRL_SRC_REGRET, 1>(prm, grid, stream);
+            else if (steady == 5) fhp_launch_t<PRL_FHP_UPDATE0, PRL_SRC_REGRET, PRL_SRC_REGRET, 5>(prm, grid, stream);
+            else if (steady == fhp_steady_pair(5, 1) && FHP_AVG_SPLIT) fhp_launch_split_t<PRL_FHP_UPDATE0, fhp_steady_pair(5, 1)>(prm, grid, stream);
+            else { taken = 0; fhp_launch_t<PRL_FHP_UPDATE0, PRL_SRC_REGRET, PRL_SRC_REGRET>(prm, grid, stream); }
+            break;
         case PRL_FHP_UPDATE1 * 100 + PRL_SRC_REGRET * 10 + PRL_SRC_REGRET: fhp_launch_t<PRL_FHP_UPDATE1, PRL_SRC_REGRET, PRL_SRC_REGRET>(prm, grid, stream); break;
         case PRL_FHP_UPDATE0_EVAL * 100 + PRL_SRC_REGRET * 10 + PRL_SRC_REGRET: fhp_launch_t<PRL_FHP_UPDATE0_EVAL, PRL_SRC_REGRET, PRL_SRC_REGRET>(prm, grid, stream); break;
         case PRL_FHP_UPDATE0_BR * 100 + PRL_SRC_REGRET * 10 + PRL_SRC_REGRET:
@@ -1027,7 +1065,10 @@
             else if (steady == 3) fhp_launch_t<PRL_FHP_UPDATE1_EVAL1, PRL_SRC_REGRET, PRL_SRC_REGRET, 3>(prm, grid, stream);
             else fhp_launch_t<PRL_FHP_UPDATE1_EVAL1, PRL_SRC_REGRET, PRL_SRC_REGRET>(prm, grid, stream);
             break;
-        case PRL_FHP_EVAL0 * 100 + PRL_SRC_REGRET * 10 + PRL_SRC_REGRET: fhp_launch_t<PRL_FHP_EVAL0, PRL_SRC_REGRET, PRL_SRC_REGRET>(prm, grid, stream); break;
+        case PRL_FHP_EVAL0 * 100 + PRL_SRC_REGRET * 10 + PRL_SRC_REGRET:
+            if (steady_eval) { taken = 1; fhp_launch_t<PRL_FHP_EVAL0, PRL_SRC_REGRET, PRL_SRC_REGRET, 1>(prm, grid, stream); }
+            else fhp_launch_t<PRL_FHP_EVAL0, PRL_SRC_REGRET, PRL_SRC_REGRET>(prm, grid, stream);
+            break;
         case PRL_FHP_EVAL * 100 + PRL_SRC_UNIFORM64 * 10 + PRL_SRC_UNIFORM64: fhp_launch_t<PRL_FHP_EVAL, PRL_SRC_UNIFORM64, PRL_SRC_UNIFORM64>(prm, grid, stream); break;
         case PRL_FHP_EVAL * 100 + PRL_SRC_REGRET * 10 + PRL_SRC_REGRET: fhp_launch_t<PRL_FHP_EVAL, PRL_SRC_REGRET, PRL_SRC_REGRET>(prm, grid, stream); break;
         case PRL_FHP_EVAL * 100 + PRL_SRC_ARR64 * 10 + PRL_SRC_ARR64: fhp_launch_t<PRL_FHP_EVAL, PRL_SRC_ARR64, PRL_SRC_ARR64>(prm, grid, stream); break;
@@ -1036,5 +1077,6 @@
         case PRL_FHP_EVAL * 100 + PRL_SRC_ARR32 * 10 + PRL_SRC_ARR32: fhp_launch_t<PRL_FHP_EVAL, PRL_SRC_ARR32, PRL_SRC_ARR32>(prm, grid, stream); break;
         default: return PRL_ERR_UNSUPPORTED;
     }
+    if (steady_taken) *steady_taken = taken;
     return PRL_OK;
 }
diff --git a/pokerrl_amd/csrc/prl_solver.hip b/pokerrl_amd/csrc/prl_solver.hip
--- a/pokerrl_amd/csrc/prl_solver.hip
+++ b/pokerrl_amd/csrc/prl_solver.hip
@@ -88,6 +88,7 @@
     long long n_exchanges = 0;
     long long n_avg_pairs = 0;
     long long n_avg_split_pairs = 0;
+    long long n_steady_ends[2] = {0, 0};
     void* rccl_comm = nullptr;
     bool streets = false;
     PrlStPlanHost st;
@@ -580,8 +581,11 @@
         PRL_HIP_TRY(hipEventCreate(&ev1));
         PRL_HIP_TRY(hipEventRecord(ev0, s->stream));
     }
-    int e = prl_launch_fhp_pass(p, mode, src0, src1, s->stream);
+    int steady_taken = 0;
+    int e = prl_launch_fhp_pass(p, mode, src0, src1, s->stream, &steady_taken);
     if (e) { prl_set_error("fused engine: unsupported strategy-source combination"); return e; }
+    if (steady_taken && mode == PRL_FHP_UPDATE0) ++s->n_steady_ends[0];
+    if (steady_taken && mode == PRL_FHP_EVAL0) ++s->n_steady_ends[1];
     if (s->time_passes) {
         PRL_HIP_TRY(hipEventRecord(ev1, s->stream));
         s->pass_events.push_back(ev0);
@@ -2353,6 +2357,7 @@
         case PRL_SF_EXCHANGES: *(int64_t*)out = (int64_t)s->n_exchanges; return PRL_OK;
         case PRL_SF_AVG_PAIRS: *(int64_t*)out = (int64_t)s->n_avg_pairs; return PRL_OK;
         case PRL_SF_AVG_SPLIT_PAIRS: *(int64_t*)out = (int64_t)s->n_avg_split_pairs; return PRL_OK;
+        case PRL_SF_STEADY_ENDS: ((int64_t*)out)[0] = (int64_t)s->n_steady_ends[0]; ((int64_t*)out)[1] = (int64_t)s->n_steady_ends[1]; return PRL_OK;
         case PRL_SF_VMM_RANGES: {
             int64_t bytes = 0;
 #if !defined(PRL_EMU)
```

Result: no change. 204.2 million, median of 6 (+0.9%).
